# bdaiinstitute/judo

Hardware: AMD Instinct MI355X
Metric: rollouts/sec + plan-step ms, leap_cube MPPI 65536xH64 (higher is better)
Workload: dtype f32

## Files before the change

### include/judo_amd.h

```cpp
#ifndef JUDO_AMD_H
#define JUDO_AMD_H

#include <stddef.h>
#include <stdint.h>

#ifdef __cplusplus
extern "C" {
#endif

typedef struct jh_model jh_model;

enum jh_status {
  JH_OK = 0,
  JH_ERR_INVALID = -1,
  JH_ERR_HIP = -2,
  JH_ERR_UNSUPPORTED = -3,
  JH_ERR_BLOB = -4
};

enum jh_task_kind { JH_TASK_CARTPOLE = 0, JH_TASK_CYLINDER_PUSH = 1, JH_TASK_LEAP_CUBE = 2, JH_TASK_FR3_PICK = 3 };
enum jh_spline_kind { JH_SPLINE_ZERO = 0, JH_SPLINE_LINEAR = 1, JH_SPLINE_CUBIC = 3 };

#define JH_MAX_TASK_PARAMS 32
#define JH_MAX_KNOT_DIM 512
// ... 1 lines not shown

const char* jh_last_error(void);
int jh_version(void);

int jh_model_create(const void* blob, size_t nbytes, int device, jh_model** out);
void jh_model_destroy(jh_model* m);
int jh_model_dims(const jh_model* m, int* dims );

int jh_model_stats(jh_model* m, int* out , int reset);


int jh_model_set_self_collision(jh_model* m, int on);

int jh_model_set_contact_capacity(jh_model* m, int contacts);

int jh_model_build(const jh_model* m, int* out );

int jh_model_fr3_build(const jh_model* m, int* out );

int jh_model_trace_layout(const jh_model* m, int* out );
int jh_trace_gather(const float* rec_in , int k, int stride_in, int n_offset, int n_local, const float* trace , int row_floats,
                    int colmajor, float* rec_out , void* stream);

int jh_model_limits(const jh_model* m, int* out );
int jh_model_max_fused_knots(const jh_model* m, int H);
int jh_model_one_launch_max_knots(const jh_model* m, int H);
int jh_model_set_plan_step_launches(jh_model* m, int launches);
int jh_model_set_rollout_schedule(jh_model* m, int mode);

int jh_upload_async(void* dst_device, const void* src_host, size_t nbytes, void* stream);
int jh_download_wait(void* dst_host, const void* src_device, size_t nbytes, void* stream);
int jh_download_begin(void* dst_host, const void* src_device, size_t nbytes, void* stream);
int jh_download_end(void);

int jh_rollout_cost(const jh_model* m, const float* x0, const float* nominal, const float* noise, int ldn, const float* sigma,
                    const float* W, const float* ctrl_lo_hi, const float* task_params, int phase, int N, int n_offset, int H, int K,
                    float* costs, float* knots_out, void* stream);
int jh_rollout_cost_traced(const jh_model* m, const float* x0, const float* nominal, const float* noise, int ldn, const float* sigma,
                    const float* W, const float* ctrl_lo_hi, const float* task_params, int phase, int N, int n_offset, int H, int K,
                    float* costs, float* knots_out, float* trace , void* stream);

int jh_rollout_materialize(const jh_model* m, const float* x0, int x0_batched, const float* controls, int N, int H, float* states,
                           float* sensors, void* stream);

int jh_task_reward(const jh_model* m, const float* states, const float* sensors, const float* controls, const float* task_params,
                   int phase, int N, int H, float* rewards, void* stream);

int jh_noise_normal(unsigned long long seed, unsigned int draw, int rows, int n_offset, int n_local, float* out, int ldn, void* stream);

int jh_sample_knots(const float* nominal, const float* noise, int ldn, const float* sigma, const float* ctrl_lo_hi ,
                    int N, int n_offset, int K, int nu, float* knots_nku, void* stream);

int jh_spline_controls(const float* W, const float* knots_nku, const float* nominal, const float* noise, int ldn, const float* sigma,
                       const float* ctrl_lo_hi, int N, int n_offset, int H, int K, int nu, float* controls, void* stream);

int jh_knot_moments(const float* knots_nku, const float* nominal, const float* noise, int ldn, const float* sigma, const float* ctrl_lo_hi,
                    const float* center, int N, int n_offset, int K, int nu, float* out, void* stream);

size_t jh_update_scratch_floats(int N, int K, int nu);
int jh_mppi_partial(const float* costs, const float* knots_nku, const float* nominal, const float* noise, int ldn, const float* sigma,
                    const float* ctrl_lo_hi, int N, int n_offset, int K, int nu, float lambda, float* scratch, float* rec, void* stream);
int jh_mppi_merge(const float* recs, int G, int K, int nu, float lambda, float* nominal_out, void* stream);

int jh_topk_partial(const float* costs, const float* knots_nku, const float* nominal, const float* noise, int ldn, const float* sigma,
                    const float* ctrl_lo_hi, int N, int n_offset, int K, int nu, int k, int tie_high, float* scratch, float* rec,
                    void* stream);
size_t jh_update_fused_scratch_floats(int N, int K, int nu);
int jh_update_fused(const float* costs, const float* knots_nku, const float* nominal, const float* noise, int ldn, const float* sigma, const float* ctrl_lo_hi, int N,
                    int n_offset, int K, int nu, int mode, float lambda, int k, int tie_high, int E, const float* trace, int row_floats, int colmajor, float* scratch,
                    float* nominal_out, float* sigma_out, float* trace_out, void* stream);
int jh_plan_step(const jh_model* m, void* blk_dev, const void* blk_host, size_t blk_bytes, int o_nominal, int o_sigma, int o_tp, int o_lohi, const float* noise, int ldn,
                 const float* W, int phase, int N, int n_offset, int H, int K, float* costs, float* knots_out, float* trace, int mode, float lambda, int k, int tie_high, int E,
                 int row_floats, int colmajor, float* scratch, float* out, void* out_host_mark, void* const* timing, void* stream);
size_t jh_plan_batch_scratch_floats(int B, int N, int K, int nu);
int jh_plan_step_batch(const jh_model* m, int B, void* blk_dev, const void* blk_host, size_t blk_bytes, size_t blk_stride_bytes, int o_nominal, int o_sigma, int o_tp, int o_lohi,
                       const float* noise, int ldn, size_t noise_stride_floats, const float* W, int N, int H, int K, float* costs, float* trace, int mode, float lambda, int k,
                       int tie_high, int E, int row_floats, int colmajor, float* scratch, float* out, size_t out_stride_floats, void* out_host_mark, void* const* timing,
                       void* stream);
typedef struct jh_model_set jh_model_set;
int jh_model_set_create(const jh_model* const* models , int B, jh_model_set** out);
int jh_model_set_update(jh_model_set* set, int b, const jh_model* model);
int jh_model_set_info(const jh_model_set* set, int* out );
void jh_model_set_destroy(jh_model_set* set);
int jh_plan_step_batch_models(const jh_model_set* set, void* blk_dev, const void* blk_host, size_t blk_bytes, size_t blk_stride_bytes, int o_nominal, int o_sigma, int o_tp, int o_lohi,
                              const float* noise, int ldn, size_t noise_stride_floats, const float* W, int N, int H, int K, float* costs, float* trace, int mode, float lambda, int k,
                              int tie_high, int E, int row_floats, int colmajor, float* scratch, float* out, size_t out_stride_floats, void* out_host_mark, void* const* timing,
                              void* stream);
int jh_noise_normal_batch(int B, const unsigned long long* seeds , const unsigned int* draws , int rows, int n_local, float* out, int ldn, void* stream);
int jh_spline_controls_batch(const float* W, int B, const float* blk, size_t blk_stride_floats, int o_nominal, int o_sigma, int o_lohi, const float* noise, int ldn,
                             size_t noise_stride_floats, int N, int H, int K, int nu, float* controls, void* stream);
int jh_update_fused_batch(int B, const float* costs, const float* blk, size_t blk_stride_floats, int o_nominal, int o_sigma, int o_lohi, const float* noise, int ldn,
                          size_t noise_stride_floats, int N, int K, int nu, int mode, float lambda, int k, int tie_high, int E, const float* trace, int row_floats, int colmajor,
                          float* scratch, float* out, size_t out_stride_floats, void* out_host_mark, void* stream);
size_t jh_shard_record_floats(int K, int nu, int mode, int k, int E, int row_floats);
int jh_update_shard(const float* costs, const float* knots_nku, const float* nominal, const float* noise, int ldn, const float* sigma, const float* ctrl_lo_hi, int N,
                    int n_offset, int K, int nu, int mode, float lambda, int k, int tie_high, int E, const float* trace, int row_floats, int colmajor, float* scratch,
                    float* rec_out, void* stream);
int jh_shard_merge(const float* recs, int G, int K, int nu, int mode, float lambda, int k, int tie_high, int E, int row_floats, float* nominal_out, float* sigma_out,
                   float* trace_out, void* stream);
int jh_plan_step_shard(const jh_model* m, void* blk_dev, const void* blk_host, size_t blk_bytes, int o_nominal, int o_sigma, int o_tp, int o_lohi, const float* noise, int ldn,
                       const float* W, int phase, int N, int n_offset, int H, int K, float* costs, float* knots_out, float* trace, int mode, float lambda, int k, int tie_high,
                       int E, int row_floats, int colmajor, float* scratch, float* rec_out, void* const* timing, void* stream);
int jh_plan_merge(const float* recs, int G, int K, int nu, int mode, float lambda, int k, int tie_high, int E, int row_floats, float* out, void* out_host_mark,
                  void* timing_done, void* stream);
int jh_event_create(void** out);
void jh_event_destroy(void* ev);
int jh_event_record(void* ev, void* stream);
int jh_stream_wait_event(void* stream, void* ev);
int jh_event_elapsed_ms(void* a, void* b, float* ms);
int jh_elite_merge(const float* recs, int G, int k, int K, int nu, int tie_high, float sigma_min, float sigma_max, float* nominal_out,
                   float* sigma_out, void* stream);

typedef struct jh_policy jh_policy;
int jh_policy_create(const float* const* weights, const float* const* biases, jh_policy** out);
void jh_policy_destroy(jh_policy* p);
size_t jh_policy_scratch_floats(int N);
int jh_policy_step(const jh_policy* p, const float* states, int ld, int nq, int base_qpos, int base_qvel, int leg_qpos, int leg_qvel,
                   const float* command, float* policy_out, float* control, float* scratch, int N, void* stream);

typedef struct jh_tree jh_tree;
int jh_tree_create(const void* blob, size_t nbytes, jh_tree** out);
void jh_tree_destroy(jh_tree* t);
int jh_tree_stats(jh_tree* t, int* out4, int reset);
int jh_tree_set_self_collision(jh_tree* t, int on);
int jh_tree_dims(const jh_tree* t, int* out4 );
int jh_tree_substeps(const jh_tree* t, const float* state_in, const float* ctrl, float* warmstart, int N, int substeps, float* state_out, float* sensors_out,
                     void* stream);

size_t jh_policy_rollout_scratch_floats(int N);
int jh_policy_rollout(const jh_policy* p, jh_tree* t, const float* x0, int x0_batched, const float* commands, float* policy_out, float* warmstart, int reset_warmstart,
                      int N, int T, int substeps, double cutoff_seconds, float* states, float* sensors, float* scratch, int* steps_done, void* stream);
int jh_policy_rollout_batch(const jh_policy* p, jh_tree* t, int B, const float* x0, size_t x0_stride_floats, const float* commands, float* policy_out, float* warmstart,
                            int reset_warmstart, int n, int T, int substeps, double cutoff_seconds, float* states, float* sensors, float* scratch, int* steps_done, void* stream);

#ifdef __cplusplus
}
#endif
#endif
```

### judo_amd/_lib.py

```python

from __future__ import annotations

import ctypes as C
import os

_HERE = os.path.dirname(os.path.abspath(__file__))
LIB_PATH = os.environ.get("JUDO_AMD_LIB") or os.path.join(_HERE, "libjudo_amd.so")

_lib: C.CDLL | None = None

f32p = C.c_void_p

_SIGNATURES = {
    "jh_last_error": (C.c_char_p, []),
    "jh_version": (C.c_int, []),
    "jh_model_create": (C.c_int, [C.c_void_p, C.c_size_t, C.c_int, C.POINTER(C.c_void_p)]),
    "jh_model_destroy": (None, [C.c_void_p]),
    "jh_model_dims": (C.c_int, [C.c_void_p, C.POINTER(C.c_int)]),
    "jh_model_stats": (C.c_int, [C.c_void_p, C.POINTER(C.c_int), C.c_int]),
    "jh_model_set_kernel": (C.c_int, [C.c_void_p, C.c_int]),
    "jh_model_limits": (C.c_int, [C.c_void_p, C.POINTER(C.c_int)]),
    "jh_register_xcheck": (C.c_int, [C.c_void_p]),
    "jh_model_max_fused_knots": (C.c_int, [C.c_void_p, C.c_int]),
    "jh_model_one_launch_max_knots": (C.c_int, [C.c_void_p, C.c_int]),
    "jh_model_set_plan_step_launches": (C.c_int, [C.c_void_p, C.c_int]),
    "jh_model_set_rollout_schedule": (C.c_int, [C.c_void_p, C.c_int]),
    "jh_model_set_self_collision": (C.c_int, [C.c_void_p, C.c_int]),
    "jh_model_set_contact_capacity": (C.c_int, [C.c_void_p, C.c_int]),
    "jh_model_build": (C.c_int, [C.c_void_p, C.POINTER(C.c_int)]),
    "jh_model_fr3_build": (C.c_int, [C.c_void_p, C.POINTER(C.c_int)]),
    "jh_model_trace_layout": (C.c_int, [C.c_void_p, C.POINTER(C.c_int)]),
    "jh_trace_gather": (C.c_int, [C.c_void_p, C.c_int, C.c_int, C.c_int, C.c_int, C.c_void_p, C.c_int, C.c_int, C.c_void_p, C.c_void_p]),
    "jh_upload_async": (C.c_int, [C.c_void_p, C.c_void_p, C.c_size_t, C.c_void_p]),
    "jh_download_wait": (C.c_int, [C.c_void_p, C.c_void_p, C.c_size_t, C.c_void_p]),
    "jh_download_begin": (C.c_int, [C.c_void_p, C.c_void_p, C.c_size_t, C.c_void_p]),
    "jh_download_end": (C.c_int, []),
    "jh_rollout_cost": (C.c_int, [C.c_void_p, f32p, f32p, f32p, C.c_int, f32p, f32p, f32p, f32p, C.c_int, C.c_int, C.c_int, C.c_int, C.c_int, f32p, f32p, C.c_void_p]),
    "jh_rollout_cost_traced": (C.c_int, [C.c_void_p, f32p, f32p, f32p, C.c_int, f32p, f32p, f32p, f32p, C.c_int, C.c_int, C.c_int, C.c_int, C.c_int, f32p, f32p, f32p, C.c_void_p]),
    "jh_rollout_materialize": (C.c_int, [C.c_void_p, f32p, C.c_int, f32p, C.c_int, C.c_int, f32p, f32p, C.c_void_p]),
    "jh_task_reward": (C.c_int, [C.c_void_p, f32p, f32p, f32p, f32p, C.c_int, C.c_int, C.c_int, f32p, C.c_void_p]),
    "jh_noise_normal": (C.c_int, [C.c_ulonglong, C.c_uint, C.c_int, C.c_int, C.c_int, f32p, C.c_int, C.c_void_p]),
    "jh_sample_knots": (C.c_int, [f32p, f32p, C.c_int, f32p, f32p, C.c_int, C.c_int, C.c_int, C.c_int, f32p, C.c_void_p]),
    "jh_spline_controls": (C.c_int, [f32p, f32p, f32p, f32p, C.c_int, f32p, f32p, C.c_int, C.c_int, C.c_int, C.c_int, C.c_int, f32p, C.c_void_p]),
    "jh_spline_controls_batch": (C.c_int, [f32p, C.c_int, f32p, C.c_size_t, C.c_int, C.c_int, C.c_int, f32p, C.c_int, C.c_size_t, C.c_int, C.c_int, C.c_int, C.c_int, f32p, C.c_void_p]),
    "jh_knot_moments": (C.c_int, [f32p, f32p, f32p, C.c_int, f32p, f32p, f32p, C.c_int, C.c_int, C.c_int, C.c_int, f32p, C.c_void_p]),
    "jh_policy_create": (C.c_int, [C.POINTER(C.c_void_p), C.POINTER(C.c_void_p), C.POINTER(C.c_void_p)]),
    "jh_policy_destroy": (None, [C.c_void_p]),
    "jh_policy_scratch_floats": (C.c_size_t, [C.c_int]),
    "jh_policy_step": (C.c_int, [C.c_void_p, f32p, C.c_int, C.c_int, C.c_int, C.c_int, C.c_int, C.c_int, f32p, f32p, f32p, f32p, C.c_int, C.c_void_p]),
    "jh_tree_create": (C.c_int, [C.c_void_p, C.c_size_t, C.POINTER(C.c_void_p)]),
    "jh_tree_destroy": (None, [C.c_void_p]),
    "jh_tree_stats": (C.c_int, [C.c_void_p, C.POINTER(C.c_int), C.c_int]),
    "jh_tree_dims": (C.c_int, [C.c_void_p, C.POINTER(C.c_int)]),
    "jh_tree_set_self_collision": (C.c_int, [C.c_void_p, C.c_int]),
    "jh_tree_substeps": (C.c_int, [C.c_void_p, f32p, f32p, f32p, C.c_int, C.c_int, f32p, f32p, C.c_void_p]),
    "jh_policy_rollout_scratch_floats": (C.c_size_t, [C.c_int]),
    "jh_policy_rollout": (C.c_int, [C.c_void_p, C.c_void_p, f32p, C.c_int, f32p, f32p, f32p, C.c_int, C.c_int, C.c_int, C.c_int, C.c_double, f32p, f32p, f32p, C.POINTER(C.c_int), C.c_void_p]),
    "jh_policy_rollout_batch": (C.c_int, [C.c_void_p, C.c_void_p, C.c_int, f32p, C.c_size_t, f32p, f32p, f32p, C.c_int, C.c_int, C.c_int, C.c_int, C.c_double, f32p, f32p, f32p, C.POINTER(C.c_int),
                                          C.c_void_p]),
    "jh_update_scratch_floats": (C.c_size_t, [C.c_int, C.c_int, C.c_int]),
    "jh_mppi_partial": (C.c_int, [f32p, f32p, f32p, f32p, C.c_int, f32p, f32p, C.c_int, C.c_int, C.c_int, C.c_int, C.c_float, f32p, f32p, C.c_void_p]),
    "jh_mppi_merge": (C.c_int, [f32p, C.c_int, C.c_int, C.c_int, C.c_float, f32p, C.c_void_p]),
    "jh_topk_partial": (C.c_int, [f32p, f32p, f32p, f32p, C.c_int, f32p, f32p, C.c_int, C.c_int, C.c_int, C.c_int, C.c_int, C.c_int, f32p, f32p, C.c_void_p]),
    "jh_update_fused_scratch_floats": (C.c_size_t, [C.c_int, C.c_int, C.c_int]),
    "jh_update_fused": (C.c_int, [f32p, f32p, f32p, f32p, C.c_int, f32p, f32p, C.c_int, C.c_int, C.c_int, C.c_int, C.c_int, C.c_float, C.c_int, C.c_int, C.c_int, f32p, C.c_int, C.c_int,
                                  f32p, f32p, f32p, f32p, C.c_void_p]),
    "jh_plan_step": (C.c_int, [C.c_void_p, C.c_void_p, C.c_void_p, C.c_size_t, C.c_int, C.c_int, C.c_int, C.c_int, f32p, C.c_int, f32p, C.c_int, C.c_int, C.c_int, C.c_int, C.c_int, f32p, f32p, f32p,
                               C.c_int, C.c_float, C.c_int, C.c_int, C.c_int, C.c_int, C.c_int, f32p, f32p, C.c_void_p, C.c_void_p, C.c_void_p]),
    "jh_plan_batch_scratch_floats": (C.c_size_t, [C.c_int, C.c_int, C.c_int, C.c_int]),
    "jh_plan_step_batch": (C.c_int, [C.c_void_p, C.c_int, C.c_void_p, C.c_void_p, C.c_size_t, C.c_size_t, C.c_int, C.c_int, C.c_int, C.c_int, f32p, C.c_int, C.c_size_t, f32p, C.c_int, C.c_int, C.c_int,
                                     f32p, f32p, C.c_int, C.c_float, C.c_int, C.c_int, C.c_int, C.c_int, C.c_int, f32p, f32p, C.c_size_t, C.c_void_p, C.c_void_p, C.c_void_p]),
    "jh_model_set_create": (C.c_int, [C.POINTER(C.c_void_p), C.c_int, C.POINTER(C.c_void_p)]),
    "jh_model_set_update": (C.c_int, [C.c_void_p, C.c_int, C.c_void_p]),
    "jh_model_set_info": (C.c_int, [C.c_void_p, C.POINTER(C.c_int)]),
    "jh_model_set_destroy": (None, [C.c_void_p]),
    "jh_plan_step_batch_models": (C.c_int, [C.c_void_p, C.c_void_p, C.c_void_p, C.c_size_t, C.c_size_t, C.c_int, C.c_int, C.c_int, C.c_int, f32p, C.c_int, C.c_size_t, f32p, C.c_int, C.c_int, C.c_int,
                                            f32p, f32p, C.c_int, C.c_float, C.c_int, C.c_int, C.c_int, C.c_int, C.c_int, f32p, f32p, C.c_size_t, C.c_void_p, C.c_void_p, C.c_void_p]),
    "jh_update_fused_batch": (C.c_int, [C.c_int, f32p, f32p, C.c_size_t, C.c_int, C.c_int, C.c_int, f32p, C.c_int, C.c_size_t, C.c_int, C.c_int, C.c_int, C.c_int, C.c_float, C.c_int, C.c_int, C.c_int,
                                        f32p, C.c_int, C.c_int, f32p, f32p, C.c_size_t, C.c_void_p, C.c_void_p]),
    "jh_noise_normal_batch": (C.c_int, [C.c_int, C.POINTER(C.c_ulonglong), C.POINTER(C.c_uint), C.c_int, C.c_int, f32p, C.c_int, C.c_void_p]),
    "jh_shard_record_floats": (C.c_size_t, [C.c_int, C.c_int, C.c_int, C.c_int, C.c_int, C.c_int]),
    "jh_update_shard": (C.c_int, [f32p, f32p, f32p, f32p, C.c_int, f32p, f32p, C.c_int, C.c_int, C.c_int, C.c_int, C.c_int, C.c_float, C.c_int, C.c_int, C.c_int, f32p, C.c_int, C.c_int,
                                  f32p, f32p, C.c_void_p]),
    "jh_shard_merge": (C.c_int, [f32p, C.c_int, C.c_int, C.c_int, C.c_int, C.c_float, C.c_int, C.c_int, C.c_int, C.c_int, f32p, f32p, f32p, C.c_void_p]),
    "jh_plan_step_shard": (C.c_int, [C.c_void_p, C.c_void_p, C.c_void_p, C.c_size_t, C.c_int, C.c_int, C.c_int, C.c_int, f32p, C.c_int, f32p, C.c_int, C.c_int, C.c_int, C.c_int, C.c_int, f32p, f32p, f32p,
                                     C.c_int, C.c_float, C.c_int, C.c_int, C.c_int, C.c_int, C.c_int, f32p, f32p, C.c_void_p, C.c_void_p]),
    "jh_plan_merge": (C.c_int, [f32p, C.c_int, C.c_int, C.c_int, C.c_int, C.c_float, C.c_int, C.c_int, C.c_int, C.c_int, f32p, C.c_void_p, C.c_void_p, C.c_void_p]),
    "jh_event_create": (C.c_int, [C.POINTER(C.c_void_p)]),
    "jh_event_destroy": (None, [C.c_void_p]),
    "jh_event_record": (C.c_int, [C.c_void_p, C.c_void_p]),
    "jh_stream_wait_event": (C.c_int, [C.c_void_p, C.c_void_p]),
    "jh_event_elapsed_ms": (C.c_int, [C.c_void_p, C.c_void_p, C.POINTER(C.c_float)]),
    "jh_elite_merge": (C.c_int, [f32p, C.c_int, C.c_int, C.c_int, C.c_int, C.c_int, C.c_float, C.c_float, f32p, f32p, C.c_void_p]),
}

EXPORTED_SYMBOLS = tuple(_SIGNATURES)

MAX_KNOT_DIM = 512
MAX_ELITES = 32
MAX_TASK_PARAMS = 32


class JudoAmdError(RuntimeError):
    """A HIP/runtime failure reported by libjudo_amd.so."""


def lib() -> C.CDLL:
    global _lib
    if _lib is None:
        if not os.path.exists(LIB_PATH):
            raise ImportError(
                f"{LIB_PATH} is missing: the MI355X engine has no CPU fallback. "
                "Build it with `python -c 'import __graft_entry__ as g; g.build()'` (needs hipcc)."
            )
        L = C.CDLL(LIB_PATH)
        for name, (res, args) in _SIGNATURES.items():
            fn = getattr(L, name)
            fn.restype = res
            fn.argtypes = args
        _lib = L
    return _lib


def check(status: int, what: str) -> None:
    if status == 0:
        return
    msg = lib().jh_last_error().decode("utf-8", "replace")
    if status == -1:
        raise ValueError(f"{what}: {msg}")
    raise JudoAmdError(f"{what} failed (status {status}): {msg}")


def ptr(t) -> int | None:
    if t is None or isinstance(t, int):
        return t
    return t.data_ptr()
```

### judo_amd/csrc/jh_api.hip

```cpp
#include <algorithm>
#include <cmath>
#include <cstdlib>
#include <cstring>

#include "jh_internal.h"
#include "jh_update_dev.h"

static thread_local char g_err[512] = "";

void jh_set_error(const char* fmt, ...) {
  va_list ap;
  va_start(ap, fmt);
  vsnprintf(g_err, sizeof(g_err), fmt, ap);
  va_end(ap);
}

extern "C" const char* jh_last_error(void) { return g_err; }
extern "C" int jh_version(void) { return 100; }

static int image_cylinders(const jh_blob_header& h, const float* F, const int* I) {
  constexpr int HEADER = 24, BODY_I = 6, BODY_F = 32, BLOCK_I = 4, DOF_F = 20, ACT_I = 2, ACT_F = 8, GEOM_I = 2, GEOM_F = 20, GF_RBOUND = 15;
  if (h.nint < (uint32_t)HEADER || h.nfloat < (uint32_t)HEADER) return 0;
  const long NM = I[0], NBLK = I[1], nv = I[2], nu = I[4], NG = I[5];
  if (NM < 0 || NBLK < 0 || nv < 0 || nu < 0 || NG < 0) return 0;
  const long oI = HEADER + NM * BODY_I + NBLK * BLOCK_I + nu * ACT_I, oF = HEADER + NM * BODY_F + nv * DOF_F + nu * ACT_F;
  if (oI + NG * GEOM_I > (long)h.nint || oF + NG * GEOM_F > (long)h.nfloat) return 0;
  int n = 0;
  for (long g = 0; g < NG; g++) {
    if (I[oI + g * GEOM_I + 1] != 5) continue;
    const float* f = F + oF + g * GEOM_F;
    const float r = f[0], L = f[1], rb = f[GF_RBOUND], want = sqrtf(r * r + L * L);
    if (!(r > 0.f) || !(L > 0.f) || f[2] != 0.f) { jh_set_error("model_create: cylinder geom %ld: sizes must be (radius > 0, half length > 0, 0), got (%g, %g, %g)", g, r, L, f[2]); return -1; }
    if (!(fabsf(rb - want) <= 1e-5f * want)) { jh_set_error("model_create: cylinder geom %ld: bounding radius %g is not sqrt(r^2 + L^2) = %g", g, rb, want); return -1; }
    n++;
  }
  return n;
}

static int image_arm_pairs(const jh_blob_header& h, const int* I) {
  constexpr int HEADER = 24, GEOM_I = 2, GBOX = 6, GCAPSULE = 3, LF = 8, RF = 9;
  if (h.nint < (uint32_t)HEADER) return 0;
  const long gi = I[13];
  if (gi < HEADER || gi + 8 > (long)h.nint) return 0;
  const long nag = I[gi], npair = I[gi + 1];
  if (nag < 0 || npair < 0 || gi + 8 + nag * GEOM_I + npair * 2 > (long)h.nint) return 0;
  int n = 0;
  for (long p = 0; p < npair; p++) {
    const long g1 = I[gi + 8 + nag * GEOM_I + 2 * p], g2 = I[gi + 8 + nag * GEOM_I + 2 * p + 1];
    if (g1 < 0 || g1 >= nag || g2 < 0 || g2 >= nag || g1 == g2) { jh_set_error("model_create: candidate pair %ld names geoms (%ld, %ld) of %ld", p, g1, g2, nag); return -1; }
    const int b1 = I[gi + 8 + g1 * GEOM_I], t1 = I[gi + 8 + g1 * GEOM_I + 1], b2 = I[gi + 8 + g2 * GEOM_I], t2 = I[gi + 8 + g2 * GEOM_I + 1];
    const bool arm_arm = b1 >= 1 && b2 >= 1 && !((b1 == LF && b2 == RF) || (b1 == RF && b2 == LF));
    const bool arm_capsule = t1 == GCAPSULE || (t1 == GBOX && t2 == GCAPSULE && b1 >= 1);
    if (!arm_arm && !arm_capsule) continue;
    if (b1 == b2) { jh_set_error("model_create: candidate pair %ld collides two geoms of arm body %d with each other", p, b1); return -1; }
    if (t1 == GCAPSULE && t2 != GCAPSULE) { jh_set_error("model_create: candidate pair %ld between arm bodies has its capsule first; the kernel takes (box, capsule)", p); return -1; }
    n++;
  }
  return n;
}

extern "C" int jh_model_create(const void* blob, size_t nbytes, int device, jh_model** out) {
  JH_REQUIRE(blob && out, "model_create: null pointer");
  if (nbytes < sizeof(jh_blob_header)) { jh_set_error("model_create: blob too small (%zu bytes)", nbytes); return JH_ERR_BLOB; }
  jh_blob_header h;
  memcpy(&h, blob, sizeof(h));
  if (h.magic != JH_BLOB_MAGIC || h.version != JH_BLOB_VERSION) { jh_set_error("model_create: bad magic/version (%08x, %u)", h.magic, h.version); return JH_ERR_BLOB; }
  size_t need = sizeof(h) + 4 * ((size_t)h.nfloat + h.nint);
  if (nbytes != need) { jh_set_error("model_create: blob size %zu != expected %zu", nbytes, need); return JH_ERR_BLOB; }
  if (h.kind > JH_TASK_FR3_PICK) { jh_set_error("model_create: unknown task kind %u", h.kind); return JH_ERR_BLOB; }
  if (h.kind == JH_TASK_CARTPOLE && h.nfloat < CP_NPARAM) { jh_set_error("model_create: cartpole blob has %u floats, need %d", h.nfloat, CP_NPARAM); return JH_ERR_BLOB; }
  if (h.kind == JH_TASK_CYLINDER_PUSH && h.nfloat < CY_NPARAM) { jh_set_error("model_create: cylinder blob has %u floats, need %d", h.nfloat, CY_NPARAM); return JH_ERR_BLOB; }
  if (h.ntaskparam > JH_MAX_TASK_PARAMS) { jh_set_error("model_create: too many task params"); return JH_ERR_BLOB; }
  int cylinders = 0, arm_pairs = 0;
  if (h.kind == JH_TASK_LEAP_CUBE || h.kind == JH_TASK_FR3_PICK) {
    const char* q = (const char*)blob + sizeof(h);
    std::vector<float> F((const float*)q, (const float*)q + h.nfloat);
    std::vector<int> I((const int*)(q + 4 * (size_t)h.nfloat), (const int*)(q + 4 * (size_t)h.nfloat) + h.nint);
    cylinders = image_cylinders(h, F.data(), I.data());
    if (cylinders < 0) return JH_ERR_BLOB;
    if (cylinders > 0 && h.kind != JH_TASK_LEAP_CUBE) { jh_set_error("model_create: %d cylinder geoms, and only the leap kernel has a cylinder build", cylinders); return JH_ERR_BLOB; }
    if (h.kind == JH_TASK_FR3_PICK) {
      arm_pairs = image_arm_pairs(h, I.data());
      if (arm_pairs < 0) return JH_ERR_BLOB;
    }
  }
  JH_HIP(hipSetDevice(device));
  jh_model* m = new jh_model();
  m->device = device; m->kind = (int)h.kind; m->nq = h.nq; m->nv = h.nv; m->nu = h.nu; m->ns = h.ns; m->ntaskparam = h.ntaskparam;
  m->nf = h.nfloat; m->ni = h.nint; m->d_f = nullptr; m->d_i = nullptr; m->d_stats = nullptr; m->kernel_gen = (h.kind == JH_TASK_LEAP_CUBE || h.kind == JH_TASK_FR3_PICK) ? 3 : 2; m->self_collision = 1; m->contact_capacity = cylinders > 0 ? 64 : 48; m->cylinders = cylinders; m->arm_pairs = arm_pairs;
  { const char* e = getenv("JUDO_AMD_ROLLOUT_SCHEDULE"); m->rollout_schedule = (e && (e[0] == '1' || e[0] == '2')) ? e[0] - '0' : 0; }
  { const char* e = getenv("JUDO_AMD_PLAN_STEP_LAUNCHES"); m->plan_step_launches = (e && e[0] == '2') ? 2 : 0; }
  const char* p = (const char*)blob + sizeof(h);
  m->h_f.assign((const float*)p, (const float*)p + h.nfloat);
  m->h_i.assign((const int*)(p + 4 * (size_t)h.nfloat), (const int*)(p + 4 * (size_t)h.nfloat) + h.nint);
  {
    hipMemPool_t pool = nullptr; int dev = 0;
    if (hipGetDevice(&dev) == hipSuccess && hipDeviceGetDefaultMemPool(&pool, dev) == hipSuccess && pool) {
      unsigned long long keep = ~0ull;
      (void)hipMemPoolSetAttribute(pool, hipMemPoolAttrReleaseThreshold, &keep);
    }
  }
  hipError_t e = hipMalloc(&m->d_f, 4 * (m->nf ? m->nf : 1));
  if (e == hipSuccess) e = hipMalloc(&m->d_i, 4 * (m->ni ? m->ni : 1));
  if (e == hipSuccess) e = hipMalloc(&m->d_stats, JH_NSTATS * sizeof(int));
  if (e == hipSuccess) e = hipMemset(m->d_stats, 0, JH_NSTATS * sizeof(int));
  if (e == hipSuccess && m->nf) e = hipMemcpy(m->d_f, m->h_f.data(), 4 * m->nf, hipMemcpyHostToDevice);
  if (e == hipSuccess && m->ni) e = hipMemcpy(m->d_i, m->h_i.data(), 4 * m->ni, hipMemcpyHostToDevice);
  if (e != hipSuccess) {
    jh_set_error("model_create: device upload failed: %s", hipGetErrorString(e));
    if (m->d_f) (void)hipFree(m->d_f);
    if (m->d_i) (void)hipFree(m->d_i);
    if (m->d_stats) (void)hipFree(m->d_stats);
    delete m;
    return JH_ERR_HIP;
  }
  *out = m;
  return JH_OK;
}

extern "C" void jh_model_destroy(jh_model* m) {
  if (!m) return;
  if (m->d_f) (void)hipFree(m->d_f);
  if (m->d_i) (void)hipFree(m->d_i);
  if (m->d_stats) (void)hipFree(m->d_stats);
  delete m;
}

extern "C" int jh_model_dims(const jh_model* m, int* dims) {
  JH_REQUIRE(m && dims, "model_dims: null pointer");
  dims[0] = m->nq; dims[1] = m->nv; dims[2] = m->nu; dims[3] = m->ns; dims[4] = m->kind; dims[5] = m->ntaskparam;
  return JH_OK;
}

extern "C" int jh_model_stats(jh_model* m, int* out, int reset) {
  JH_REQUIRE(m && out, "model_stats: null pointer");
  JH_HIP(hipMemcpy(out, m->d_stats, 4 * sizeof(int), hipMemcpyDeviceToHost));
  JH_HIP(hipMemcpy(out + 4, m->d_stats + 20, 2 * sizeof(int), hipMemcpyDeviceToHost));
  out[6] = reset ? __atomic_exchange_n(&m->ovf_fallbacks, 0, __ATOMIC_RELAXED) : __atomic_load_n(&m->ovf_fallbacks, __ATOMIC_RELAXED);
  out[7] = reset ? __atomic_exchange_n(&m->one_launch_steps, 0, __ATOMIC_RELAXED) : __atomic_load_n(&m->one_launch_steps, __ATOMIC_RELAXED);
  if (reset) JH_HIP(hipMemset(m->d_stats, 0, JH_NSTATS * sizeof(int)));
  return JH_OK;
}

extern "C" int jh_model_hist(jh_model* m, int* out ) {
  JH_REQUIRE(m && out, "model_hist: null pointer");
  JH_HIP(hipMemcpy(out, m->d_stats + 24, 40 * sizeof(int), hipMemcpyDeviceToHost));
  return JH_OK;
}

extern "C" int jh_model_counters(jh_model* m, int* out, int first, int count) {
  JH_REQUIRE(m && out && first >= 0 && count >= 0 && first + count <= JH_NSTATS, "model_counters: bad range");
  JH_HIP(hipMemcpy(out, m->d_stats + first, count * sizeof(int), hipMemcpyDeviceToHost));
  return JH_OK;
}

static jh_xcheck_launchers g_xcheck = {nullptr, nullptr, nullptr};

extern "C" int jh_register_xcheck(const jh_xcheck_launchers* launchers) {
  JH_REQUIRE(launchers && launchers->rollout_cost && launchers->rollout_materialize && launchers->max_knots, "register_xcheck: incomplete launcher table");
  g_xcheck = *launchers;
  return JH_OK;
}
// ... 185 lines not shown
  JH_HIP(hipMemcpy(out, m->d_stats + 4, 10 * sizeof(long long), hipMemcpyDeviceToHost));
  return JH_OK;
}

extern "C" int jh_rollout_cost(const jh_model* m, const float* x0, const float* nominal, const float* noise, int ldn, const float* sigma,
                               const float* W, const float* lohi, const float* tp, int phase, int N, int n_offset, int H, int K, float* costs,
                               float* knots_out, void* stream) {
  return jh_rollout_cost_traced(m, x0, nominal, noise, ldn, sigma, W, lohi, tp, phase, N, n_offset, H, K, costs, knots_out, nullptr, stream);
}

extern "C" int jh_rollout_cost_traced(const jh_model* m, const float* x0, const float* nominal, const float* noise, int ldn, const float* sigma,
                                      const float* W, const float* lohi, const float* tp, int phase, int N, int n_offset, int H, int K, float* costs,
                                      float* knots_out, float* trace, void* stream) {
  JH_REQUIRE(m && x0 && nominal && noise && sigma && W && lohi && tp && costs, "rollout_cost: null pointer");
  if (trace) { int adr, nfl, cm; trace_layout(m, &adr, &nfl, &cm); JH_REQUIRE(nfl > 0, "rollout_cost_traced: this model's fused kernel writes no trace sensors (jh_model_trace_layout)"); }
  JH_REQUIRE(N > 0 && H > 0 && K >= 1, "rollout_cost: N, H, K must be positive (N=%d H=%d K=%d)", N, H, K);
  JH_REQUIRE(ldn >= N, "rollout_cost: ldn (%d) < N (%d)", ldn, N);
  JH_REQUIRE(K * m->nu <= JH_MAX_KNOT_DIM, "rollout_cost: K*nu = %d exceeds %d", K * m->nu, JH_MAX_KNOT_DIM);
  JH_REQUIRE(n_offset >= 0, "rollout_cost: negative n_offset");
  hipStream_t st = (hipStream_t)stream;
  if (m->kind == JH_TASK_CARTPOLE || m->kind == JH_TASK_CYLINDER_PUSH)
    return jh_simple_rollout_cost(m, x0, nominal, noise, ldn, sigma, W, lohi, tp, N, n_offset, H, K, costs, knots_out, trace, st);
  if (m->kind == JH_TASK_LEAP_CUBE && m->kernel_gen == 3)
    return m->cylinders > 0         ? jh_engine5_rollout_cost_cyl(m, x0, nominal, noise, ldn, sigma, W, lohi, tp, N, n_offset, H, K, costs, knots_out, trace, st)
           : m->contact_capacity > 48 ? jh_engine5_rollout_cost_cap64(m, x0, nominal, noise, ldn, sigma, W, lohi, tp, N, n_offset, H, K, costs, knots_out, trace, st)
                                    : jh_engine5_rollout_cost(m, x0, nominal, noise, ldn, sigma, W, lohi, tp, N, n_offset, H, K, costs, knots_out, trace, st);
  if (m->kind == JH_TASK_FR3_PICK && m->kernel_gen == 3)
    return m->arm_pairs > 0 ? jh_engine6_rollout_cost_self(m, x0, nominal, noise, ldn, sigma, W, lohi, tp, phase, N, n_offset, H, K, costs, knots_out, trace, st)
                            : jh_engine6_rollout_cost(m, x0, nominal, noise, ldn, sigma, W, lohi, tp, phase, N, n_offset, H, K, costs, knots_out, trace, st);
  JH_REQUIRE(trace == nullptr, "rollout_cost_traced: only the product kernels (generation 3, cartpole, cylinder_push) write trace sensors");
  if (!g_xcheck.rollout_cost) { jh_set_error("rollout_cost: no kernel for this model / generation in this library"); return JH_ERR_UNSUPPORTED; }
  return g_xcheck.rollout_cost(m, m->kernel_gen, x0, nominal, noise, ldn, sigma, W, lohi, tp, phase, N, n_offset, H, K, costs, knots_out, stream);
}

static int plan_step_launches(const jh_model* m, int N, int H, int K, const float* costs, const float* knots_out, const float* W, const float* noise, int ldn, bool* one) {
  *one = false;
  if (m->plan_step_launches == 2 || !(m->kind == JH_TASK_CARTPOLE || m->kind == JH_TASK_CYLINDER_PUSH)) return JH_OK;
  const bool fits = costs && W && noise && N > 0 && H > 0 && K >= 1 && ldn >= N && K * m->nu <= JH_MAX_KNOT_DIM && jh_simple_plan_step_fits(m, H, K);
  if (m->plan_step_launches == 1) {
    JH_REQUIRE(!knots_out, "plan_step: the one-launch plan step writes no candidate knots (knots_out), and one launch is forced (jh_model_set_plan_step_launches)");
    JH_REQUIRE(fits, "plan_step: one launch is forced but K = %d exceeds its LDS staging at H = %d (jh_model_one_launch_max_knots)", K, H);
  }
  *one = fits && !knots_out;
  if (*one) __atomic_fetch_add(&m->one_launch_steps, 1, __ATOMIC_RELAXED);
  return JH_OK;
}

static int plan_step(const char* who, const jh_model* m, void* blk_dev, const void* blk_host, size_t blk_bytes, int o_nominal, int o_sigma, int o_tp, int o_lohi,
                     const float* noise, int ldn, const float* W, int phase, int N, int n_offset, int H, int K, float* costs, float* knots_out, float* trace, int mode,
                     float lambda, int k, int tie_high, int E, int row_floats, int colmajor, float* scratch, float* out, unsigned* flag, float* rec_out,
                     void* const* timing, void* stream) {
  JH_REQUIRE(m && blk_dev && blk_host && (out || rec_out) && scratch, "%s: null pointer", who);
  const float* b = (const float*)blk_dev;
  hipStream_t st = (hipStream_t)stream;
  int rc = blk_dev == blk_host ? JH_OK : jh_upload_async(blk_dev, blk_host, blk_bytes, stream);
  if (rc == JH_OK && timing) JH_HIP(hipEventRecord((hipEvent_t)timing[0], st));
  const int KU = K * m->nu;
  const unsigned expect = flag ? __atomic_load_n(flag, __ATOMIC_RELAXED) + 1u : 0u;
  bool one = false;
  if (rc == JH_OK) rc = plan_step_launches(m, N, H, K, costs, knots_out, W, noise, ldn, &one);
  if (rc == JH_OK && !one) rc = jh_rollout_cost_traced(m, b, b + o_nominal, noise, ldn, b + o_sigma, W, b + o_lohi, b + o_tp, phase, N, n_offset, H, K, costs, knots_out, trace, stream);
  if (rc == JH_OK && !one && timing) JH_HIP(hipEventRecord((hipEvent_t)timing[1], st));
  jh_upd::TailArgs a;
  if (rc == JH_OK)
    rc = jh_update_tail_args(who, costs, nullptr, b + o_nominal, noise, ldn, b + o_sigma, b + o_lohi, N, n_offset, K, m->nu, mode, lambda, k, tie_high, trace ? E : 0, trace, row_floats,
                             colmajor, scratch, out, out ? out + KU : nullptr, (out && trace && E > 0) ? out + 2 * KU : nullptr, rec_out, &a);
  a.done_flag = flag; a.done_value = expect;
  if (rc == JH_OK) rc = one ? jh_simple_plan_step(m, b, W, b + o_tp, H, K, a, st) : jh_update_tail_launch(a, st);
  if (rc == JH_OK && one && timing) JH_HIP(hipEventRecord((hipEvent_t)timing[1], st));
  if (rc == JH_OK && timing) JH_HIP(hipEventRecord((hipEvent_t)timing[2], st));
  if (rc == JH_OK && out) rc = download_begin(out, out, 0, stream, flag, expect);
  return rc;
}

extern "C" int jh_plan_step(const jh_model* m, void* blk_dev, const void* blk_host, size_t blk_bytes, int o_nominal, int o_sigma, int o_tp, int o_lohi, const float* noise, int ldn,
                            const float* W, int phase, int N, int n_offset, int H, int K, float* costs, float* knots_out, float* trace, int mode, float lambda, int k, int tie_high, int E,
                            int row_floats, int colmajor, float* scratch, float* out, void* out_host_mark, void* const* timing , void* stream) {
  JH_REQUIRE(out, "plan_step: null pointer");
  unsigned* flag = (out_host_mark && out_host_mark != (void*)out) ? (unsigned*)out_host_mark : nullptr;
  return plan_step("plan_step", m, blk_dev, blk_host, blk_bytes, o_nominal, o_sigma, o_tp, o_lohi, noise, ldn, W, phase, N, n_offset, H, K, costs, knots_out, trace, mode, lambda, k,
                   tie_high, E, row_floats, colmajor, scratch, out, flag, nullptr, timing, stream);
}

static int plan_step_batch(const char* who, const jh_model* m, const float* images, long long image_stride, int B, void* blk_dev, const void* blk_host, size_t blk_bytes, size_t blk_stride_bytes,
                           int o_nominal, int o_sigma, int o_tp, int o_lohi, const float* noise, int ldn, size_t noise_stride_floats, const float* W, int N, int H, int K, float* costs,
                           float* trace, int mode, float lambda, int k, int tie_high, int E, int row_floats, int colmajor, float* scratch, float* out, size_t out_stride_floats,
                           void* out_host_mark, void* const* timing, void* stream) {
  JH_REQUIRE(m && blk_dev && blk_host && out && scratch && noise && W && costs, "%s: null pointer", who);
  if (m->kind == JH_TASK_FR3_PICK) { jh_set_error("%s: fr3_pick has no batched plan step (its phase is chosen per problem on the host)", who); return JH_ERR_UNSUPPORTED; }
  if (m->kind == JH_TASK_LEAP_CUBE && m->kernel_gen != 3) { jh_set_error("%s: only kernel generation 3 of the leap family has a batched launch (this model runs %d)", who, m->kernel_gen); return JH_ERR_UNSUPPORTED; }
  JH_REQUIRE(B >= 1, "%s: B must be at least 1 (B=%d)", who, B);
  JH_REQUIRE(B <= 65535, "%s: B = %d exceeds the 65535 problems of a launch (the grid's second dimension)", who, B);
  JH_REQUIRE(N > 0 && H > 0 && K >= 1, "%s: N, H, K must be positive (N=%d H=%d K=%d)", who, N, H, K);
  JH_REQUIRE(ldn >= N, "%s: ldn (%d) < N (%d)", who, ldn, N);
  const int KU = K * m->nu;
  JH_REQUIRE(KU <= JH_MAX_KNOT_DIM, "%s: K*nu = %d exceeds %d", who, KU, JH_MAX_KNOT_DIM);
  const int nx = m->nq + m->nv;
  JH_REQUIRE(o_nominal >= 0 && o_sigma >= 0 && o_tp >= 0 && o_lohi >= 0, "%s: negative block offset", who);
  const size_t need = sizeof(float) * (size_t)std::max(std::max(nx, o_nominal + KU), std::max(std::max(o_sigma + KU, o_tp + m->ntaskparam), o_lohi + 2 * m->nu));
  JH_REQUIRE(blk_bytes >= need, "%s: a block of %zu bytes does not hold x0 | nominal | sigma | task params | bounds at the given offsets (%zu bytes)", who, blk_bytes, need);
  JH_REQUIRE(blk_stride_bytes >= blk_bytes && blk_stride_bytes % sizeof(float) == 0, "%s: blk_stride_bytes = %zu is smaller than a block (%zu bytes) or no multiple of 4", who, blk_stride_bytes, blk_bytes);
  JH_REQUIRE(noise_stride_floats >= (size_t)KU * (size_t)ldn, "%s: noise_stride_floats = %zu is smaller than a problem's noise (K*nu*ldn = %zu)", who, noise_stride_floats, (size_t)KU * (size_t)ldn);
  int t_adr = 0, t_nfl = 0, t_cm = 0;
  if (trace) { trace_layout(m, &t_adr, &t_nfl, &t_cm); JH_REQUIRE(t_nfl > 0 && row_floats == H * t_nfl, "%s: row_floats = %d is not H x the model's %d trace floats per step (jh_model_trace_layout)", who, row_floats, t_nfl); }
  const int E_t = trace ? E : 0;
  JH_REQUIRE(E_t >= 0 && E_t <= JH_MAX_ELITES, "%s: bad trace arguments (E=%d)", who, E);
  const size_t rec = 2 * (size_t)KU + (size_t)E_t * (2 + (size_t)(E_t > 0 ? row_floats : 0));
  JH_REQUIRE(out_stride_floats >= rec, "%s: out_stride_floats = %zu is smaller than an output record (nominal | sigma | E trace records = %zu floats)", who, out_stride_floats, rec);
  const bool closed = m->kind == JH_TASK_CARTPOLE || m->kind == JH_TASK_CYLINDER_PUSH;
  if (!closed && m->kind != JH_TASK_LEAP_CUBE) { jh_set_error("%s: no batched kernel for this model", who); return JH_ERR_UNSUPPORTED; }
  hipStream_t st = (hipStream_t)stream;
  const float* b = (const float*)blk_dev;
  if (blk_dev != blk_host) { const int rc = jh_upload_async(blk_dev, blk_host, (size_t)(B - 1) * blk_stride_bytes + blk_bytes, stream); if (rc != JH_OK) return rc; }
  if (timing) JH_HIP(hipEventRecord((hipEvent_t)timing[0], st));
  unsigned* flag = (out_host_mark && out_host_mark != (void*)out) ? (unsigned*)out_host_mark : nullptr;
  const unsigned expect = flag ? __atomic_load_n(flag, __ATOMIC_RELAXED) + 1u : 0u;
  bool one = false;
  if (int rc = plan_step_launches(m, N, H, K, costs, nullptr, W, noise, ldn, &one)) return rc;
  jh_upd::TailArgs a;
  if (int rc = jh_update_tail_args(who, costs, nullptr, b + o_nominal, noise, ldn, b + o_sigma, b + o_lohi, N, 0, K, m->nu, mode, lambda, k, tie_high, E_t, trace, row_floats, colmajor,
                                   scratch, out, out + KU, E_t > 0 ? out + 2 * KU : nullptr, nullptr, &a)) return rc;
  jh_upd::BatchArgs s;
  s.B = B; s.blk = (long long)(blk_stride_bytes / sizeof(float)); s.noise = (long long)noise_stride_floats; s.costs = N; s.trace = (long long)N * row_floats;
  s.scratch = (long long)jh_update_fused_scratch_floats(N, K, m->nu); s.out = (long long)out_stride_floats;
  s.counter = reinterpret_cast<unsigned*>(scratch) + 1; s.done_flag = flag; s.done_value = expect; s.image = image_stride;
  int rc = JH_OK;
  if (one) rc = jh_simple_plan_step_batch(m, images, b, W, b + o_tp, H, K, a, s, st);
  else {
    if (closed) rc = jh_simple_rollout_cost_batch(m, images, b, b + o_tp, W, H, K, a, s, st);
    else
      rc = m->cylinders > 0           ? jh_engine5_rollout_cost_batch_cyl(m, images, image_stride, B, b, b + o_nominal, b + o_sigma, b + o_lohi, b + o_tp, s.blk, noise, ldn, s.noise, W, N, H, K, costs, trace, st)
           : m->contact_capacity > 48 ? jh_engine5_rollout_cost_batch_cap64(m, images, image_stride, B, b, b + o_nominal, b + o_sigma, b + o_lohi, b + o_tp, s.blk, noise, ldn, s.noise, W, N, H, K, costs, trace, st)
                                      : jh_engine5_rollout_cost_batch(m, images, image_stride, B, b, b + o_nominal, b + o_sigma, b + o_lohi, b + o_tp, s.blk, noise, ldn, s.noise, W, N, H, K, costs, trace, st);
    if (rc == JH_OK && timing) JH_HIP(hipEventRecord((hipEvent_t)timing[1], st));
    if (rc == JH_OK) rc = jh_update_tail_batch_launch(a, s, st);
  }
  if (rc == JH_OK && one && timing) JH_HIP(hipEventRecord((hipEvent_t)timing[1], st));
  if (rc == JH_OK && timing) JH_HIP(hipEventRecord((hipEvent_t)timing[2], st));
  if (rc == JH_OK) rc = download_begin(out, out, 0, stream, flag, expect);
  return rc;
}

extern "C" int jh_plan_step_batch(const jh_model* m, int B, void* blk_dev, const void* blk_host, size_t blk_bytes, size_t blk_stride_bytes, int o_nominal, int o_sigma, int o_tp, int o_lohi,
                                  const float* noise, int ldn, size_t noise_stride_floats, const float* W, int N, int H, int K, float* costs, float* trace, int mode, float lambda, int k,
                                  int tie_high, int E, int row_floats, int colmajor, float* scratch, float* out, size_t out_stride_floats, void* out_host_mark, void* const* timing,
                                  void* stream) {
  JH_REQUIRE(m != nullptr, "plan_step_batch: null pointer");
  return plan_step_batch("plan_step_batch", m, m->d_f, 0, B, blk_dev, blk_host, blk_bytes, blk_stride_bytes, o_nominal, o_sigma, o_tp, o_lohi, noise, ldn, noise_stride_floats, W, N, H, K, costs, trace,
                         mode, lambda, k, tie_high, E, row_floats, colmajor, scratch, out, out_stride_floats, out_host_mark, timing, stream);
}

struct jh_model_set {
  int B;
  size_t nf, stride;
  float* d_images;
  const jh_model* m0;
  std::vector<std::vector<float>> hf;
};

static int model_set_member(const char* who, const jh_model* m0, const jh_model* m, int b) {
  JH_REQUIRE(m != nullptr, "%s: member %d is a null pointer", who, b);
  if (m->kind == JH_TASK_FR3_PICK) { jh_set_error("%s: member %d is an fr3_pick model, which has no batched plan step (its phase is chosen per problem on the host)", who, b); return JH_ERR_UNSUPPORTED; }
  if (m->kind == JH_TASK_LEAP_CUBE && m->kernel_gen != 3) { jh_set_error("%s: member %d runs kernel_gen %d: only kernel generation 3 of the leap family has a batched launch", who, b, m->kernel_gen); return JH_ERR_UNSUPPORTED; }
  if (m->kind != JH_TASK_CARTPOLE && m->kind != JH_TASK_CYLINDER_PUSH && m->kind != JH_TASK_LEAP_CUBE) { jh_set_error("%s: member %d: no batched kernel for this model (kind %d)", who, b, m->kind); return JH_ERR_UNSUPPORTED; }
  if (m != m0) {
#define JH_SET_SAME(field, fmt)                                                                                                                                    \
  JH_REQUIRE(m->field == m0->field, "%s: member %d differs from the set's member 0 in " #field " (" fmt " against " fmt ")", who, b, m->field, m0->field)
    JH_SET_SAME(device, "%d"); JH_SET_SAME(kind, "%d"); JH_SET_SAME(nq, "%d"); JH_SET_SAME(nv, "%d"); JH_SET_SAME(nu, "%d"); JH_SET_SAME(ns, "%d"); JH_SET_SAME(ntaskparam, "%d");
    JH_SET_SAME(nf, "%zu"); JH_SET_SAME(ni, "%zu");
    if (m->h_i != m0->h_i) {
      size_t w = 0;
      while (w < m->h_i.size() && m->h_i[w] == m0->h_i[w]) w++;
      jh_set_error("%s: member %d differs from the set's member 0 in the int section h_i (word %zu: %d against %d): topology, pair lists and lane lists are one for the launch", who, b, w, m->h_i[w], m0->h_i[w]);
      return JH_ERR_INVALID;
    }
    JH_SET_SAME(kernel_gen, "%d"); JH_SET_SAME(contact_capacity, "%d"); JH_SET_SAME(cylinders, "%d"); JH_SET_SAME(self_collision, "%d"); JH_SET_SAME(rollout_schedule, "%d");
    JH_SET_SAME(plan_step_launches, "%d");
#undef JH_SET_SAME
  }
  JH_REQUIRE(m->h_f.size() == m->nf && m->d_f, "%s: member %d has no float section of nf = %zu floats", who, b, m->nf);
  if (m->kind == JH_TASK_LEAP_CUBE) {
    const bool ok = m->cylinders > 0 ? jh_engine5_accepts_cyl(m) : m->contact_capacity > 48 ? jh_engine5_accepts_cap64(m) : jh_engine5_accepts(m);
    if (!ok) {
      jh_set_error("%s: member %d: the leap kernel does not accept this image (dimensions, table sizes, or h_f: the cube's inertia must be isotropic)", who, b);
      return JH_ERR_UNSUPPORTED;
    }
  }
  return JH_OK;
}

static int model_set_upload(jh_model_set* s, int b, const jh_model* m) {
  if (s->nf) JH_HIP(hipMemcpy(s->d_images + (size_t)b * s->stride, m->d_f, 4 * s->nf, hipMemcpyDeviceToDevice));
  s->hf[b] = m->h_f;
  return JH_OK;
}

extern "C" int jh_model_set_create(const jh_model* const* models, int B, jh_model_set** out) {
  JH_REQUIRE(models && out, "model_set_create: null pointer");
  JH_REQUIRE(B >= 1, "model_set_create: B must be at least 1 (B=%d)", B);
  JH_REQUIRE(B <= 65535, "model_set_create: B = %d exceeds the 65535 problems of a launch (the grid's second dimension)", B);
  for (int b = 0; b < B; b++) if (int rc = model_set_member("model_set_create", models[0], models[b], b)) return rc;
  const jh_model* m0 = models[0];
  JH_HIP(hipSetDevice(m0->device));
  jh_model_set* s = new jh_model_set();
  s->B = B; s->nf = m0->nf; s->stride = (m0->nf + 63) / 64 * 64; s->d_images = nullptr; s->m0 = m0; s->hf.resize(B);
  if (s->stride == 0) s->stride = 64;
  hipError_t e = hipMalloc(&s->d_images, 4 * s->stride * (size_t)B);
  if (e == hipSuccess) e = hipMemset(s->d_images, 0, 4 * s->stride * (size_t)B);
  int rc = JH_OK;
  if (e != hipSuccess) { jh_set_error("model_set_create: device allocation failed: %s", hipGetErrorString(e)); rc = JH_ERR_HIP; }
  for (int b = 0; b < B && rc == JH_OK; b++) rc = model_set_upload(s, b, models[b]);
  if (rc != JH_OK) { if (s->d_images) (void)hipFree(s->d_images); delete s; return rc; }
  *out = s;
  return JH_OK;
}

extern "C" int jh_model_set_update(jh_model_set* s, int b, const jh_model* model) {
  JH_REQUIRE(s && model, "model_set_update: null pointer");
  JH_REQUIRE(b >= 0 && b < s->B, "model_set_update: member %d of a set of %d", b, s->B);
  if (int rc = model_set_member("model_set_update", s->m0, model, b)) return rc;
  JH_HIP(hipSetDevice(s->m0->device));
  if (int rc = model_set_upload(s, b, model)) return rc;
  if (b == 0) s->m0 = model;
  return JH_OK;
}

extern "C" int jh_model_set_info(const jh_model_set* s, int* out) {
  JH_REQUIRE(s && out, "model_set_info: null pointer");
  int differ = 0;
  for (int b = 1; b < s->B; b++) differ += s->hf[b].size() != s->hf[0].size() || memcmp(s->hf[b].data(), s->hf[0].data(), 4 * s->hf[0].size()) != 0;
  out[0] = s->B; out[1] = (int)s->nf; out[2] = (int)s->stride; out[3] = differ;
  return JH_OK;
}

extern "C" void jh_model_set_destroy(jh_model_set* s) {
  if (!s) return;
  if (s->d_images) (void)hipFree(s->d_images);
  delete s;
}

extern "C" int jh_plan_step_batch_models(const jh_model_set* set, void* blk_dev, const void* blk_host, size_t blk_bytes, size_t blk_stride_bytes, int o_nominal, int o_sigma, int o_tp, int o_lohi,
                                         const float* noise, int ldn, size_t noise_stride_floats, const float* W, int N, int H, int K, float* costs, float* trace, int mode, float lambda,
                                         int k, int tie_high, int E, int row_floats, int colmajor, float* scratch, float* out, size_t out_stride_floats, void* out_host_mark,
                                         void* const* timing, void* stream) {
  JH_REQUIRE(set != nullptr, "plan_step_batch_models: null pointer");
  return plan_step_batch("plan_step_batch_models", set->m0, set->d_images, (long long)set->stride, set->B, blk_dev, blk_host, blk_bytes, blk_stride_bytes, o_nominal, o_sigma, o_tp, o_lohi, noise, ldn,
                         noise_stride_floats, W, N, H, K, costs, trace, mode, lambda, k, tie_high, E, row_floats, colmajor, scratch, out, out_stride_floats, out_host_mark, timing, stream);
}

extern "C" int jh_update_fused_batch(int B, const float* costs, const float* blk, size_t blk_stride_floats, int o_nominal, int o_sigma, int o_lohi, const float* noise, int ldn,
                                     size_t noise_stride_floats, int N, int K, int nu, int mode, float lambda, int k, int tie_high, int E, const float* trace, int row_floats,
                                     int colmajor, float* scratch, float* out, size_t out_stride_floats, void* out_host_mark, void* stream) {
  JH_REQUIRE(costs && blk && noise && scratch && out, "update_fused_batch: null pointer");
  JH_REQUIRE(B >= 1, "update_fused_batch: B must be at least 1 (B=%d)", B);
  JH_REQUIRE(B <= 65535, "update_fused_batch: B = %d exceeds the 65535 problems of a launch (the grid's second dimension)", B);
  JH_REQUIRE(N > 0 && K > 0 && nu > 0 && K * nu <= JH_MAX_KNOT_DIM, "update_fused_batch: N, K, nu must be positive and K*nu <= %d (N=%d K=%d nu=%d)", JH_MAX_KNOT_DIM, N, K, nu);
  JH_REQUIRE(o_nominal >= 0 && o_sigma >= 0 && o_lohi >= 0, "update_fused_batch: negative block offset");
  const int KU = K * nu;
  const size_t need = (size_t)std::max(std::max(o_nominal + KU, o_sigma + KU), o_lohi + 2 * nu);
  JH_REQUIRE(blk_stride_floats >= need, "update_fused_batch: blk_stride_floats = %zu is smaller than a block (nominal | sigma | bounds at the given offsets end at %zu floats)", blk_stride_floats, need);
  JH_REQUIRE(ldn >= N && noise_stride_floats >= (size_t)KU * (size_t)ldn, "update_fused_batch: ldn (%d) < N (%d), or noise_stride_floats = %zu is smaller than a problem's noise (K*nu*ldn = %zu)", ldn, N,
             noise_stride_floats, (size_t)KU * (size_t)ldn);
  const int E_t = trace ? E : 0;
  JH_REQUIRE(E_t >= 0 && E_t <= JH_MAX_ELITES && (E_t == 0 || row_floats >= 1), "update_fused_batch: bad trace arguments (E=%d row_floats=%d)", E, row_floats);
  const size_t rec = 2 * (size_t)KU + (size_t)E_t * (2 + (size_t)(E_t > 0 ? row_floats : 0));
  JH_REQUIRE(out_stride_floats >= rec, "update_fused_batch: out_stride_floats = %zu is smaller than an output record (nominal | sigma | E trace records = %zu floats)", out_stride_floats, rec);
  unsigned* flag = (out_host_mark && out_host_mark != (void*)out) ? (unsigned*)out_host_mark : nullptr;
  const unsigned expect = flag ? __atomic_load_n(flag, __ATOMIC_RELAXED) + 1u : 0u;
  jh_upd::TailArgs a;
  if (int rc = jh_update_tail_args("update_fused_batch", costs, nullptr, blk + o_nominal, noise, ldn, blk + o_sigma, blk + o_lohi, N, 0, K, nu, mode, lambda, k, tie_high, E_t, trace, row_floats,
                                   colmajor, scratch, out, out + KU, E_t > 0 ? out + 2 * KU : nullptr, nullptr, &a)) return rc;
  jh_upd::BatchArgs s;
  s.B = B; s.blk = (long long)blk_stride_floats; s.noise = (long long)noise_stride_floats; s.costs = N; s.trace = (long long)N * row_floats;
  s.scratch = (long long)jh_update_fused_scratch_floats(N, K, nu); s.out = (long long)out_stride_floats;
  s.counter = reinterpret_cast<unsigned*>(scratch) + 1; s.done_flag = flag; s.done_value = expect;
  if (int rc = jh_update_tail_batch_launch(a, s, (hipStream_t)stream)) return rc;
  return download_begin(out, out, 0, stream, flag, expect);
}

extern "C" int jh_plan_step_shard(const jh_model* m, void* blk_dev, const void* blk_host, size_t blk_bytes, int o_nominal, int o_sigma, int o_tp, int o_lohi, const float* noise,
                                  int ldn, const float* W, int phase, int N, int n_offset, int H, int K, float* costs, float* knots_out, float* trace, int mode, float lambda, int k,
                                  int tie_high, int E, int row_floats, int colmajor, float* scratch, float* rec_out, void* const* timing , void* stream) {
  JH_REQUIRE(rec_out, "plan_step_shard: null pointer");
  return plan_step("plan_step_shard", m, blk_dev, blk_host, blk_bytes, o_nominal, o_sigma, o_tp, o_lohi, noise, ldn, W, phase, N, n_offset, H, K, costs, knots_out, trace, mode,
                   lambda, k, tie_high, E, row_floats, colmajor, scratch, nullptr, nullptr, rec_out, timing, stream);
}

extern "C" int jh_plan_merge(const float* recs, int G, int K, int nu, int mode, float lambda, int k, int tie_high, int E, int row_floats, float* out, void* out_host_mark,
                             void* timing_done , void* stream) {
  JH_REQUIRE(recs && out, "plan_merge: null pointer");
  const int KU = K * nu;
  int rc = jh_shard_merge(recs, G, K, nu, mode, lambda, k, tie_high, E, row_floats, out, out + KU, E > 0 ? out + 2 * KU : nullptr, stream);
  if (rc == JH_OK && timing_done) JH_HIP(hipEventRecord((hipEvent_t)timing_done, (hipStream_t)stream));
  if (rc == JH_OK) rc = jh_download_begin(out_host_mark, out, 0, stream);
  return rc;
}

extern "C" int jh_event_create(void** out) { JH_REQUIRE(out, "event_create: null pointer"); hipEvent_t e; JH_HIP(hipEventCreate(&e)); *out = e; return JH_OK; }
extern "C" void jh_event_destroy(void* ev) { if (ev) (void)hipEventDestroy((hipEvent_t)ev); }
extern "C" int jh_event_record(void* ev, void* stream) { JH_REQUIRE(ev, "event_record: null pointer"); JH_HIP(hipEventRecord((hipEvent_t)ev, (hipStream_t)stream)); return JH_OK; }
extern "C" int jh_stream_wait_event(void* stream, void* ev) {
  JH_REQUIRE(ev, "stream_wait_event: null pointer");
  JH_HIP(hipStreamWaitEvent((hipStream_t)stream, (hipEvent_t)ev, 0));
  return JH_OK;
}
extern "C" int jh_event_elapsed_ms(void* a, void* b, float* ms) {
  JH_REQUIRE(a && b && ms, "event_elapsed_ms: null pointer");
  JH_HIP(hipEventSynchronize((hipEvent_t)b));
  JH_HIP(hipEventElapsedTime(ms, (hipEvent_t)a, (hipEvent_t)b));
  return JH_OK;
}

extern "C" int jh_rollout_materialize(const jh_model* m, const float* x0, int x0_batched, const float* controls, int N, int H, float* states,
                                      float* sensors, void* stream) {
  JH_REQUIRE(m && x0 && controls, "rollout_materialize: null pointer");
  JH_REQUIRE(states || sensors, "rollout_materialize: both outputs are null");
  JH_REQUIRE(N > 0 && H > 0, "rollout_materialize: N and H must be positive (N=%d H=%d)", N, H);
  hipStream_t st = (hipStream_t)stream;
  if (m->kind == JH_TASK_CARTPOLE || m->kind == JH_TASK_CYLINDER_PUSH) return jh_simple_materialize(m, x0, x0_batched, controls, N, H, states, sensors, st);
  if (m->kind == JH_TASK_LEAP_CUBE && m->kernel_gen == 3)
    return m->cylinders > 0 ? jh_engine5_materialize_cyl(m, x0, x0_batched, controls, N, H, states, sensors, st) : m->contact_capacity > 48 ? jh_engine5_materialize_cap64(m, x0, x0_batched, controls, N, H, states, sensors, st) : jh_engine5_materialize(m, x0, x0_batched, controls, N, H, states, sensors, st);
  if (m->kind == JH_TASK_FR3_PICK && m->kernel_gen == 3)
    return m->arm_pairs > 0 ? jh_engine6_materialize_self(m, x0, x0_batched, controls, N, H, states, sensors, st) : jh_engine6_materialize(m, x0, x0_batched, controls, N, H, states, sensors, st);
  if (!g_xcheck.rollout_materialize) { jh_set_error("rollout_materialize: no kernel for this model / generation in this library"); return JH_ERR_UNSUPPORTED; }
  return g_xcheck.rollout_materialize(m, m->kernel_gen, x0, x0_batched, controls, N, H, states, sensors, stream);
}

extern "C" int jh_task_reward(const jh_model* m, const float* states, const float* sensors, const float* controls, const float* tp, int phase, int N,
                              int H, float* rewards, void* stream) {
// ... 10 lines not shown
```

### judo_amd/csrc/jh_engine_v5.hip

```cpp
#include <cstddef>
#include <type_traits>

#include "jh_coop.h"

using namespace jh_eng;
using namespace jh_coop;

namespace {

#ifdef JH_V5_WAVESTAMP
__device__ unsigned long long* g_wavestamp = nullptr;
__device__ int g_wavestamp_cap = 0;
#endif

constexpr int G = 16, RPW = 4, WAVE = 64;
constexpr int NCH = 4, NLK = 4;

constexpr int LSMAX = 16;
constexpr int WAVES_PER_EU = 2;
constexpr int WAVES_PER_BLOCK = 4;
constexpr int BFS = 33;
constexpr int PAS = 9;
constexpr int RSPAD = 4;
constexpr int C3PAD = 278;
constexpr int NSLDS = 3;
constexpr double BIGPROB = 0.999999;
constexpr int CVX_STOP_NM = 1000;
#define OPAQUE(x) asm volatile("" : "+v"(x))
#define WSYNC() do { __builtin_amdgcn_fence(__ATOMIC_RELEASE, "wavefront"); __builtin_amdgcn_wave_barrier(); __builtin_amdgcn_fence(__ATOMIC_ACQUIRE, "wavefront"); } while (0)
#ifndef JH_V5_NSLOT
#define JH_V5_NSLOT 2
#endif
#ifndef JH_V5_NSBIG
#define JH_V5_NSBIG 3
#endif
#ifndef JH_V5_CYL
#define JH_V5_CYL 0
#endif
constexpr int GCYL = 5;
constexpr int NSLOT = JH_V5_NSLOT;
constexpr int NSBIG = JH_V5_NSBIG;
constexpr int NCP = 16 * (NSBIG < NSLDS ? NSBIG : NSLDS);
constexpr int NCAP = 16 * NSBIG;
constexpr int NOVF = NCAP - NCP;
constexpr int MAXHIT = 64;
constexpr int POOL_F = 10;
constexpr int MAXG = 80, MAXLG = 8;
constexpr int CUBE = 17;
constexpr int HITPAIR = 1 << 15;
static_assert(MAXG <= 128, "hand geom pairs are packed into 14 bits");
constexpr int MAXBP = 128;
constexpr int MAXBPL = 96;
constexpr int NDH = 22 * 23 / 2;
constexpr int NV = 22, NQ = 23, NU = 16, NS = 31, NS_CALTECH = 23, NX = 45, NMB = 17;
constexpr int NBC = 20;
__device__ __forceinline__ bool static_code(int b) { return b == 0 || b >= NMB; }

enum { LC_DAMP = 0, LC_KVD, LC_KP, LC_KV, LC_CLO, LC_CHI, LC_CLIM, LC_FL, LC_FB, LC_FD, LC_INVW, LC_LIMITED, LC_LO, LC_HI, LC_LK, LC_LB, LC_SI, LC_IMCK = LC_SI + 5, LC_N = 25 };

struct __attribute__((aligned(16))) RS {
  float pa[NMB][PAS];
  float xR[NMB][9];
  float qv[NV], g[NV], p[NV], ws[NV];
  float acn[6];
  float Mbb[NCH][10];
  float rhs6[6];
  float cmd[4];
  union {
    struct {
      float bs[NBC][4];
      unsigned short hits[MAXHIT];
      unsigned char bpl[MAXBPL];
    };
    struct { float pk_q[G], pk_fs[G], pk_cq[4], pk_acc; };
  };
  union {
    float pool[NCP][POOL_F];
    struct { float Hcc[21], Hbb[NCH][10], Hcb[NCH][24], Hx[6][16]; };
    struct { float Hd[NDH], dinv[NV]; };
    struct { float c3pad_[C3PAD]; float c3s[G][12]; };
  };
  int ncon, nhit;
  float pad_[RSPAD];
};

static_assert(offsetof(RS, c3s) % 16 == 0 && C3PAD >= NDH + NV && sizeof(((RS*)nullptr)->c3pad_) + sizeof(((RS*)nullptr)->c3s) <= sizeof(((RS*)nullptr)->pool), "c3 cache: aligned rows behind the Newton matrices, inside the pool's storage");
struct PoolCtx { RS* S; int* overflow; float* ovf; };

__device__ __forceinline__ void push_contact(const PoolCtx& pc, const float* pos, const float* n, float dist, int body, float mu, float tran) {
  int i = atomicAdd(&pc.S->ncon, 1);
  float* e;
  if (i < NCP) e = pc.S->pool[i];
  else if (NOVF > 0 && pc.ovf && i < NCAP) e = pc.ovf + (i - NCP) * POOL_F;
  else { if (pc.overflow) atomicAdd(pc.overflow, 1); return; }
  e[0] = pos[0]; e[1] = pos[1]; e[2] = pos[2]; e[3] = n[0]; e[4] = n[1]; e[5] = n[2]; e[6] = dist; e[7] = mu; e[8] = __int_as_float(body); e[9] = tran;
}

struct LeapSink {
  PoolCtx pc; int sides; float mu, tran; bool flip;
  __device__ __forceinline__ void push(const float* pos, const float* n, float dist) {
    const float nn[3] = {flip ? -n[0] : n[0], flip ? -n[1] : n[1], flip ? -n[2] : n[2]};
    push_contact(pc, pos, nn, dist, sides, mu, tran);
  }
};

#if JH_V5_CYL
struct CvxOne {
  float pos[3], n[3], dist; bool hit;
  __device__ __forceinline__ void push(const float* p, const float* nn, float d) { for (int k = 0; k < 3; k++) { pos[k] = p[k]; n[k] = nn[k]; } dist = d; hit = true; }
};
#endif

struct Slot {
  int la, lb;
  float fr[9];
  float rc[3];
  float aref[3], D0, D1, Dm, mu, fri;
  float jar[3], jp[3];
};

__device__ __forceinline__ bool obb_face_overlap(const float* ca, const float* Ra, const float* ha, const float* cb, const float* Rb, const float* hb) {
  const float d[3] = {cb[0] - ca[0], cb[1] - ca[1], cb[2] - ca[2]};
  float C[9];
#pragma unroll
  for (int i = 0; i < 3; i++)
#pragma unroll
    for (int j = 0; j < 3; j++) C[3 * i + j] = fabsf(Ra[i] * Rb[j] + Ra[3 + i] * Rb[3 + j] + Ra[6 + i] * Rb[6 + j]);
  bool ok = true;
#pragma unroll
  for (int i = 0; i < 3; i++) {
    const float da = fabsf(d[0] * Ra[i] + d[1] * Ra[3 + i] + d[2] * Ra[6 + i]);
    ok = ok && da <= ha[i] + hb[0] * C[3 * i] + hb[1] * C[3 * i + 1] + hb[2] * C[3 * i + 2];
    const float db = fabsf(d[0] * Rb[i] + d[1] * Rb[3 + i] + d[2] * Rb[6 + i]);
    ok = ok && db <= hb[i] + ha[0] * C[i] + ha[1] * C[3 + i] + ha[2] * C[6 + i];
// ... 225 lines not shown
#ifdef JH_V5_WAVESTAMP
  const unsigned long long ws_entry = wall_clock64(); unsigned long long ws_staged = ws_entry;
#endif
  const int tid = threadIdx.x, wv = tid >> 6, lane = tid & 63, r = lane >> 4;
  int l = lane & 15, c = l >> 2, s = l & 3;
  RS& S = sRS[wv * RPW + r];
  const int nmI = gI[0], nblkI = gI[1], nuI = gI[4], ngI = gI[5], nsiteI = gI[6], nsI = gI[7], oRef = gI[18];
  const int oBodyF = HEADER_F, oDofF = oBodyF + nmI * BODY_F, oActF = oDofF + gI[2] * DOF_F, oGeomF = oActF + nuI * ACT_F, oSiteF = oGeomF + ngI * GEOM_F;
  const int oGeomI = HEADER_I + nmI * BODY_I + nblkI * BLOCK_I + nuI * ACT_I, oSiteI = oGeomI + ngI * GEOM_I;
  const int oLane = gI[11], lgm = gI[12];
  const int oBP = gI[15], oBS = gI[16], nBP = gI[17], oBG = oBP + 2 * nBP;
  for (int i = tid; i < 16 * BODY_F; i += WAVE * WPB) sBody[(i / BODY_F) * BFS + i % BODY_F] = gF[oBodyF + BODY_F + i];
  for (int i = tid; i < ngI * GEOM_F; i += WAVE * WPB) sGeomF[i] = gF[oGeomF + i];
  for (int i = tid; i < ngI * GEOM_I; i += WAVE * WPB) sGeomI[i] = gI[oGeomI + i];
  for (int i = tid; i < 16 * lgm; i += WAVE * WPB) sLaneG[i] = gI[oLane + i];
  if (!MATERIALIZE && tid < 9) sTp[tid] = tp[tid];
  if constexpr (SELF) {
    for (int i = tid; i < 2 * nBP && i < 2 * MAXBP; i += WAVE * WPB) sBP[i] = gI[oBP + i];
    for (int i = tid; i < 2 * NBC; i += WAVE * WPB) sBG[i] = gI[oBG + i];
    for (int i = tid; i < NBC * 8; i += WAVE * WPB) sBB[i] = gF[oBS + i];
  }
  if (tid < 16) {
    const float* df = gF + oDofF + (6 + l) * DOF_F; const float* af = gF + oActF + l * ACT_F;
    float* lc = sLane + l * LC_N;
    lc[LC_DAMP] = df[DF_DAMP]; lc[LC_KVD] = df[DF_KV]; lc[LC_FL] = df[DF_FL]; lc[LC_FB] = df[DF_FB]; lc[LC_FD] = df[DF_FD]; lc[LC_INVW] = df[DF_INVW];
    lc[LC_LIMITED] = df[DF_LIMITED]; lc[LC_LO] = df[DF_LO]; lc[LC_HI] = df[DF_HI]; lc[LC_LK] = df[DF_LK]; lc[LC_LB] = df[DF_LB];
    for (int k = 0; k < 5; k++) lc[LC_SI + k] = df[DF_SOLIMP + k];
    lc[LC_KP] = af[AF_KP]; lc[LC_KV] = af[AF_KV]; lc[LC_CLIM] = af[AF_CLIM]; lc[LC_CLO] = af[AF_CLO]; lc[LC_CHI] = af[AF_CHI];
    lc[LC_IMCK] = l < 6 ? 1.f / (l < 3 ? gF[HF_CMASS] : gF[HF_CINERTIA + (l < 3 ? 0 : l - 3)]) : 0.f;
  }
  const float* lc = sLane + l * LC_N;
  int grp = blockIdx.x * WPB + wv;
  const int ngroups = (N + RPW - 1) / RPW;
  if constexpr (PERSIST) {
    __syncthreads();
#ifdef JH_V5_WAVESTAMP
    ws_staged = wall_clock64();
#endif
  }
  for (; !PERSIST || grp < ngroups;) {
  if constexpr (PERSIST) { if (lane == 0) sGrp[wv] = grp; }
#ifdef JH_V5_WAVESTAMP
  const unsigned long long ws_start = wall_clock64();
#endif
  const int n = (grp << (2 - dshift)) + (r >> dshift);
  const bool live = n < N && (r & ((1 << dshift) - 1)) == 0;
  const int nc = n < N ? n : N - 1;
  const float h = gF[HF_DT], impratio = gF[HF_IMPRATIO], tol = gF[HF_TOL], lstol = gF[HF_LSTOL]; const int cap = (int)gF[HF_MAXITER];
  const float grav[3] = {gF[HF_GRAV], gF[HF_GRAV + 1], gF[HF_GRAV + 2]};
  const float cmass = gF[HF_CMASS], cI[3] = {gF[HF_CINERTIA], gF[HF_CINERTIA + 1], gF[HF_CINERTIA + 2]};
  const float chs[3] = {gF[HF_CSIZE], gF[HF_CSIZE + 1], gF[HF_CSIZE + 2]}, crb = gF[HF_CRBOUND], ctran = gF[HF_CTRAN];
  const float cK = gF[HF_CK], cB = gF[HF_CB];
  float csi[5]; for (int k = 0; k < 5; k++) csi[k] = gF[HF_SOLIMP + k];
  const float mck = (l < 3 ? cmass : (l == 3 ? cI[0] : (l == 4 ? cI[1] : (l == 5 ? cI[2] : 0.f))));
  float q, qd, qc[7], vc[6];
  {
    const float* xi = x0 + ((MATERIALIZE && x0_batched) ? (size_t)nc * NX : 0);
    for (int k = 0; k < 7; k++) qc[k] = xi[k];
    for (int k = 0; k < 6; k++) vc[k] = xi[NQ + k];
    q = xi[7 + l]; qd = xi[NQ + 6 + l];
  }
  auto knot_at = [&](int k, int ll, int ncc) -> float {
    const int i = k * NU + ll;
    float v = nominal[i];
    if (n_offset + ncc != 0) v = fmaf(sigma[i], noise[(size_t)i * ldn + ncc], v);
    return jh_clampf(v, lohi[ll], lohi[NU + ll]);
  };
  if (!MATERIALIZE) {
    if (knots_out && live) for (int k = 0; k < K; k++) knots_out[(size_t)(k * NU + l) * ldn + n] = knot_at(k, l, nc);
  }
  S.ws[6 + l] = 0.f; if (l < 6) S.ws[l] = 0.f;
  if (l < 4) S.cmd[l] = l == 0 ? cmass : (l == 1 ? cI[0] : (l == 2 ? cI[1] : cI[2]));
  int n_iters = 0, n_maxed = 0, n_wave_iters = 0;
  float acc = 0.f;
#ifdef JH_V5_TICKS
  long long cyc[16] = {0, 0, 0, 0, 0, 0, 0, 0, 0, 0, 0, 0, 0, 0, 0, 0}, t0 = clock64();
#define V5_TICK(slot) { long long t__ = clock64(); cyc[slot] += t__ - t0; t0 = t__; }
#else
#define V5_TICK(slot)
#endif
#ifdef JH_V5_COUNT
  int cnt_dense = 0, cnt_it = 0, cnt_l2 = 0, cnt_bp = 0, cnt_hh = 0, cnt_cls[4] = {0, 0, 0, 0};
  enum { CB_SPH = 34, CB_SPHMAX, CB_BOXMAX, CB_L1PAIRPASS, CB_L1LISTPASS, CB_TRIPS, CB_BPAIRS, CB_T, CB_COMBOPASS, CB_CUBEBOX, CB_CUBEBOXLANES, CB_MSPH, CB_MBOX, CB_MT, CB_NOSPH, CB_ONEA, CB_ONEB,
         CB_OWNTRIPS, CB_SPHOVER, CB_FEWSPH };
#define V5_CADD(k, v) do { if (stats) atomicAdd(stats + (k), (int)(v)); } while (0)
#define V5_CMAX(k, v) do { if (stats) atomicMax(stats + (k), (int)(v)); } while (0)
#endif
  if constexpr (PERSIST) WSYNC();
  else {
    __syncthreads();
#ifdef JH_V5_WAVESTAMP
    ws_staged = wall_clock64();
#endif
  }

  for (int hh = 0; hh < H; hh++) {
    OPAQUE(l); c = l >> 2; s = l & 3;
    const float* lc = sLane + l * LC_N;
    float u;
    if (MATERIALIZE) u = controls[((size_t)nc * H + hh) * NU + l];
    else {
      u = 0.f;
      {
        int lo_ = lane; OPAQUE(lo_);
        const int g_ = PERSIST ? sGrp[wv] : (int)(blockIdx.x * WPB + wv);
        const int n_ = (g_ << (2 - dshift)) + ((lo_ >> 4) >> dshift), nc_ = n_ < N ? n_ : N - 1;
        for (int k = 0; k < K; k++) u = fmaf(W[hh * K + k], knot_at(k, l, nc_), u);
      }
    }
    float Mrow[NLK], fs_own, a0_own;
    {
      float ax[NLK][3], og[NLK][3], Rown[9], pown[3];
      {
        float nn = rsqrtf(qc[3] * qc[3] + qc[4] * qc[4] + qc[5] * qc[5] + qc[6] * qc[6]);
        qc[3] *= nn; qc[4] *= nn; qc[5] *= nn; qc[6] *= nn;
        float Rc[9]; quat2mat(Rc, qc + 3);
        float P[3] = {0, 0, 0}, R[9] = {1, 0, 0, 0, 1, 0, 0, 0, 1};
        float sn_own, cs_own; sincosf(q, &sn_own, &cs_own);
#pragma unroll
        for (int j = 0; j < NLK; j++) {
          const float* bf = sBody + (4 * c + j) * BFS;
          float P2[3], R0[9];
          if (j == 0) { for (int k = 0; k < 3; k++) P2[k] = bf[BF_LPOS + k]; for (int k = 0; k < 9; k++) R0[k] = bf[BF_LR + k]; }
          else { mulMV(P2, R, bf + BF_LPOS); for (int k = 0; k < 3; k++) P2[k] += P[k]; mulMM(R0, R, bf + BF_LR); }
          const float* al = bf + BF_AXIS;
          mulMV(ax[j], R0, al);
          for (int k = 0; k < 3; k++) { og[j][k] = P2[k]; P[k] = P2[k]; }
          const float sn = quad_get(sn_own, j), cs = quad_get(cs_own, j), t = 1.f - cs, x = al[0], y = al[1], z = al[2];
          float Rq[9] = {t * x * x + cs, t * x * y - sn * z, t * x * z + sn * y, t * x * y + sn * z, t * y * y + cs, t * y * z - sn * x, t * x * z - sn * y, t * y * z + sn * x, t * z * z + cs};
          mulMM(R, R0, Rq);
          if (j == s) { for (int k = 0; k < 3; k++) pown[k] = P2[k]; for (int k = 0; k < 9; k++) Rown[k] = R[k]; }
        }
        for (int k = 0; k < 3; k++) { S.pa[1 + l][k] = pown[k]; S.pa[1 + l][4 + k] = s == 0 ? ax[0][k] : (s == 1 ? ax[1][k] : (s == 2 ? ax[2][k] : ax[3][k])); }
        for (int k = 0; k < 9; k++) S.xR[1 + l][k] = Rown[k];
        if (l == 0) { for (int k = 0; k < 3; k++) S.pa[0][k] = qc[k]; for (int k = 0; k < 9; k++) S.xR[0][k] = Rc[k]; S.ncon = 0; S.nhit = 0; }
        S.qv[6 + l] = qd;
        if (l < 6) S.qv[l] = vc[l];
      }
      if (!MATERIALIZE && trace && nsI == NS) {
        WSYNC();
        if (live && l < nsiteI && l < 5) {
          int b = gI[oSiteI + l]; float p3[3]; mulMV(p3, S.xR[b], gF + oSiteF + l * SITE_F);
          float* tr = trace + ((size_t)n * H + hh) * 15 + 3 * l;
          for (int k = 0; k < 3; k++) tr[k] = p3[k] + S.pa[b][k];
        }
      }
      if (MATERIALIZE && sensors) {
        float* y = sensors + ((size_t)nc * H + hh) * nsI;
        if (live) y[l] = q;
        WSYNC();
        if (nsI == NS) {
          if (live && l < nsiteI && l < 5) {
            int b = gI[oSiteI + l]; float p3[3]; mulMV(p3, S.xR[b], gF + oSiteF + l * SITE_F);
            for (int k = 0; k < 3; k++) y[16 + 3 * l + k] = p3[k] + S.pa[b][k];
          }
        } else if (live && l < 7) {
          const float* rf = gF + oRef;
          if (l < 3) y[16 + l] = rf[3 + l] * (qc[0] - rf[0]) + rf[6 + l] * (qc[1] - rf[1]) + rf[9 + l] * (qc[2] - rf[2]);
          else {
            const float a0 = rf[12], a1 = -rf[13], a2 = -rf[14], a3 = -rf[15], b0 = qc[3], b1 = qc[4], b2 = qc[5], b3 = qc[6];
            const float qo[4] = {a0 * b0 - a1 * b1 - a2 * b2 - a3 * b3, a0 * b1 + a1 * b0 + a2 * b3 - a3 * b2, a0 * b2 - a1 * b3 + a2 * b0 + a3 * b1, a0 * b3 + a1 * b2 - a2 * b1 + a3 * b0};
            y[16 + l] = l == 3 ? qo[0] : (l == 4 ? qo[1] : (l == 5 ? qo[2] : qo[3]));
          }
        }
      }
      {
        const float* bf = sBody + (4 * c + s) * BFS;
// ... 61 lines not shown
      float Icw[3] = {cI[0] * vc[3], cI[1] * vc[4], cI[2] * vc[5]}, gc[3]; cross3(gc, vc + 3, Icw);
      (void)gc;
      a0c_own = l < 3 ? (l == 0 ? grav[0] : (l == 1 ? grav[1] : grav[2])) : 0.f;
    }
    WSYNC();
    V5_TICK(0)
    bool hand_hits = false;
    {
      int nh = 0;
      float Rc[9]; for (int k = 0; k < 9; k++) Rc[k] = S.xR[0][k];
      const float* pw = S.pa[1 + l]; const float* Rw = S.xR[1 + l];
      if constexpr (SELF) {
        const float* b8 = sBB + 8 * (1 + l); float cw[3]; mulMV(cw, Rw, b8);
        S.bs[1 + l][0] = cw[0] + pw[0]; S.bs[1 + l][1] = cw[1] + pw[1]; S.bs[1 + l][2] = cw[2] + pw[2]; S.bs[1 + l][3] = b8[3];
        if (l < 4) { S.bs[0][l] = sBB[l]; for (int b = NMB; b < NBC; b++) S.bs[b][l] = sBB[8 * b + l]; }
      }
      float pwr[3], Rwr[9];
      for (int k = 0; k < 3; k++) pwr[k] = pw[k];
      for (int k = 0; k < 9; k++) Rwr[k] = Rw[k];
      int gids[MAXLG];
#pragma unroll
      for (int i = 0; i < MAXLG; i++) gids[i] = i < lgm ? sLaneG[l * lgm + i] : -1;
#pragma unroll
      for (int i = 0; i < MAXLG; i++) {
        if (i >= lgm) break;
        const int gid = gids[i], g0 = gid < 0 ? 0 : gid;
        const float* gf = sGeomF + g0 * GEOM_F;
        const int gbody = sGeomI[g0 * GEOM_I], gtype = sGeomI[g0 * GEOM_I + 1];
        const float lp[3] = {gf[GF_POS], gf[GF_POS + 1], gf[GF_POS + 2]}, rb = gf[GF_RBOUND];
        float gp[3]; mulMV(gp, Rwr, lp); gp[0] += pwr[0]; gp[1] += pwr[1]; gp[2] += pwr[2];
        if (gbody < 0) { gp[0] = lp[0]; gp[1] = lp[1]; gp[2] = lp[2]; }
        const float dc[3] = {gp[0] - qc[0], gp[1] - qc[1], gp[2] - qc[2]}, rs = rb + crb;
        float cl[3]; mulMTV(cl, Rc, dc);
        bool hit = (gid >= 0) & (dot3(dc, dc) <= rs * rs) & (fabsf(cl[0]) <= chs[0] + rb) & (fabsf(cl[1]) <= chs[1] + rb) & (fabsf(cl[2]) <= chs[2] + rb);
#if JH_V5_CYL
        if (hit && gtype != GSPHERE) {
          const bool cyl = gtype == GCYL;
          const float gh[3] = {gf[GF_SIZE], cyl ? gf[GF_SIZE] : gf[GF_SIZE + 1], cyl ? gf[GF_SIZE + 1] : gf[GF_SIZE + 2]};
          float gR[9], gl[3];
          if (gbody < 0) { for (int k = 0; k < 9; k++) gR[k] = gf[GF_R + k]; } else mulMM(gR, Rwr, gf + GF_R);
          mulMTV(gl, gR, dc);
          hit = fabsf(gl[0]) <= gh[0] + crb && fabsf(gl[1]) <= gh[1] + crb && fabsf(gl[2]) <= gh[2] + crb;
        }
#else
#ifdef JH_V5_COUNT
        if constexpr (SELF) { const unsigned long long bx = __ballot(hit && gtype == GBOX); if (lane == 0 && bx != 0) { V5_CADD(CB_CUBEBOX, 1); V5_CADD(CB_CUBEBOXLANES, __popcll(bx)); } }
#endif
        if (hit && gtype == GBOX) {
          float gR[9], gl[3];
          if (gbody < 0) { for (int k = 0; k < 9; k++) gR[k] = gf[GF_R + k]; } else mulMM(gR, Rwr, gf + GF_R);
          mulMTV(gl, gR, dc);
          hit = fabsf(gl[0]) <= gf[GF_SIZE] + crb && fabsf(gl[1]) <= gf[GF_SIZE + 1] + crb && fabsf(gl[2]) <= gf[GF_SIZE + 2] + crb;
        }
#endif
        unsigned m16 = (unsigned)((__ballot(hit) >> (16 * r)) & 0xFFFFull);
        int pos = nh + __popc(m16 & ((1u << l) - 1u));
        if (hit && pos < MAXHIT) S.hits[pos] = (unsigned short)gid;
        nh += __popc(m16);
      }
      WSYNC();
      V5_TICK(13)
      if constexpr (SELF) {
      int nbl = 0;
      {
        constexpr int NPASS = MAXBP / G;
        int pab[NPASS]; unsigned sph = 0;
#pragma unroll
        for (int i = 0; i < NPASS; i++) { const int pi = i * G + l, pj = pi < nBP ? pi : 0; pab[i] = sBP[2 * pj] | sBP[2 * pj + 1] << 8; }
#pragma unroll
        for (int i = 0; i < NPASS; i++) {
          const float* sa = S.bs[pab[i] & 0xFF]; const float* sb = S.bs[pab[i] >> 8];
          const float d[3] = {sa[0] - sb[0], sa[1] - sb[1], sa[2] - sb[2]}, rs = sa[3] + sb[3];
          sph |= ((i * G + l < nBP) & (dot3(d, d) <= rs * rs)) ? 1u << i : 0u;
        }
#ifdef JH_V5_COUNT
        {
          int ns = 0, npass = 0;
          for (int i = 0; i < NPASS; i++) { const unsigned long long b = __ballot((sph >> i) & 1u); ns += __popc((unsigned)((b >> (16 * r)) & 0xFFFFull)); npass += b != 0; }
          const int nsm = wave_rowmax(ns);
          if (l == 0 && live) { V5_CADD(CB_SPH, ns); V5_CMAX(CB_MSPH, ns); V5_CADD(CB_NOSPH, ns == 0); V5_CADD(CB_SPHOVER, ns > MAXBPL); V5_CMAX(CB_FEWSPH, MAXBP - ns); }
          if (lane == 0) { V5_CADD(CB_SPHMAX, nsm); V5_CADD(CB_L1PAIRPASS, npass); V5_CADD(CB_L1LISTPASS, (nsm + G - 1) / G); }
        }
#endif
        unsigned char* const tail = reinterpret_cast<unsigned char*>(&S.pool[0][0]);
        static_assert(sizeof(((RS*)nullptr)->pool) >= MAXBP - MAXBPL, "the tail of the sphere survivors fits the contact pool's storage");
        int nsl = 0;
#pragma unroll
        for (int i = 0; i < NPASS; i++) {
          if (i * G >= nBP) break;
          const bool hit = (sph >> i) & 1u;
          const unsigned m16 = (unsigned)((__ballot(hit) >> (16 * r)) & 0xFFFFull);
          const int pos = nsl + __popc(m16 & ((1u << l) - 1u));
          if (hit) { if (pos < MAXBPL) S.bpl[pos] = (unsigned char)(i * G + l); else tail[pos - MAXBPL] = (unsigned char)(i * G + l); }
          nsl += __popc(m16);
        }
        WSYNC();
        for (int base = 0; __any(base < nsl); base += G) {
          const int idx = base + l;
          bool hit = idx < nsl; int pi = 0;
          if (hit) {
            pi = idx < MAXBPL ? S.bpl[idx] : tail[idx - MAXBPL];
            const int ba = sBP[2 * pi], bb = sBP[2 * pi + 1];
            const float* sa = S.bs[ba]; const float* sb = S.bs[bb];
            const float I9[9] = {1, 0, 0, 0, 1, 0, 0, 0, 1};
            float Ra[9]; for (int k = 0; k < 9; k++) Ra[k] = static_code(ba) ? I9[k] : S.xR[ba][k];
            hit = obb_face_overlap(sa, Ra, sBB + 8 * ba + 4, sb, S.xR[bb], sBB + 8 * bb + 4);
          }
          unsigned m16 = (unsigned)((__ballot(hit) >> (16 * r)) & 0xFFFFull);
          int pos = nbl + __popc(m16 & ((1u << l) - 1u));
          if (hit && pos < MAXBPL) S.bpl[pos] = (unsigned char)pi;
          nbl += __popc(m16);
          WSYNC();
        }
      }
#ifdef JH_V5_COUNT
      { const int nbm = wave_rowmax(nbl); if (lane == 0) V5_CADD(CB_BOXMAX, nbm); if (l == 0 && live) V5_CMAX(CB_MBOX, nbl); }
#endif
      if (nbl > MAXBPL) { if (l == 0 && live && stats) atomicAdd(stats, nbl - MAXBPL); nbl = MAXBPL; }
#ifdef JH_V5_COUNT
      if (l == 0 && live) cnt_bp += nbl;
#endif
      const int nh_cube = nh;
      WSYNC();
      V5_TICK(14)
      for (int i = 0; __any(i < nbl); i++) {
#ifdef JH_V5_COUNT
        if (lane == 0) cnt_l2++;
#endif
        int ba = 0, bb = 0, ga0 = 0, na = 0, gb0 = 0, nb = 0;
        if (i < nbl) { const int pi = S.bpl[i]; ba = sBP[2 * pi]; bb = sBP[2 * pi + 1]; ga0 = sBG[2 * ba]; na = sBG[2 * ba + 1]; gb0 = sBG[2 * bb]; nb = sBG[2 * bb + 1]; }
        bool near = false;
        if (l < na + nb) {
          const bool isA = l < na;
          const int g = isA ? ga0 + l : gb0 + (l - na), own = isA ? ba : bb, oth = isA ? bb : ba;
          const float* gf = sGeomF + g * GEOM_F;
          float cw[3];
          if (static_code(own)) { cw[0] = gf[GF_POS]; cw[1] = gf[GF_POS + 1]; cw[2] = gf[GF_POS + 2]; }
          else { mulMV(cw, S.xR[own], gf + GF_POS); cw[0] += S.pa[own][0]; cw[1] += S.pa[own][1]; cw[2] += S.pa[own][2]; }
          const float dw[3] = {cw[0] - S.bs[oth][0], cw[1] - S.bs[oth][1], cw[2] - S.bs[oth][2]};
          float dl[3];
          if (static_code(oth)) { dl[0] = dw[0]; dl[1] = dw[1]; dl[2] = dw[2]; } else mulMTV(dl, S.xR[oth], dw);
          const float* hb = sBB + 8 * oth + 4;
          const float ex = fmaxf(fabsf(dl[0]) - hb[0], 0.f), ey = fmaxf(fabsf(dl[1]) - hb[1], 0.f), ez = fmaxf(fabsf(dl[2]) - hb[2], 0.f);
          near = ex * ex + ey * ey + ez * ez <= gf[GF_RBOUND] * gf[GF_RBOUND];
        }
        const unsigned m16 = (unsigned)((__ballot(near) >> (16 * r)) & 0xFFFFull);
        const unsigned mB = (m16 >> na) & ((1u << nb) - 1u);
        const unsigned mA = mB != 0 ? (m16 & ((1u << na) - 1u)) : 0u;
        const int nB = __popc(mB), T = __popc(mA) * nB;
#ifdef JH_V5_COUNT
        {
          const int tm = wave_rowmax((T + G - 1) / G);
          if (lane == 0) V5_CADD(CB_COMBOPASS, tm);
          if (l == 0 && live && T != 0) { V5_CADD(CB_BPAIRS, 1); V5_CADD(CB_T, T); V5_CMAX(CB_MT, T); V5_CADD(CB_ONEA, __popc(mA) == 1); V5_CADD(CB_ONEB, nB == 1); V5_CADD(CB_OWNTRIPS, __popc(mA)); }
        }
#endif
        const float rnB = __builtin_amdgcn_rcpf((float)nB);
        for (int t = l; __any(t - l < T); t += G) {
          bool hit = false;
          int ga = 0, gb = 0;
          if (t < T) {
            const int ra = (int)(((float)t + 0.5f) * rnB), rb = t - ra * nB;
            ga = ga0 + nth_bit16(mA, ra); gb = gb0 + nth_bit16(mB, rb);
            const float* fa = sGeomF + ga * GEOM_F; const float* fb = sGeomF + gb * GEOM_F;
            float ca[3], cb[3];
            if (static_code(ba)) { ca[0] = fa[GF_POS]; ca[1] = fa[GF_POS + 1]; ca[2] = fa[GF_POS + 2]; }
// ... 780 lines not shown
  if (stats && lane == 0 && live) { atomicAdd(stats + 20, n_wave_iters); atomicAdd(stats + 21, H); }
#ifdef JH_V5_WAVESTAMP
  if (lane == 0 && g_wavestamp && grp < g_wavestamp_cap) {
    unsigned long long* w = g_wavestamp + (size_t)grp * 6;
    w[0] = ((unsigned long long)blockIdx.x << 32) | ((unsigned long long)wv << 8) | (__smid() & 0xff); w[1] = ws_entry; w[2] = ws_staged; w[3] = ws_start; w[4] = wall_clock64(); w[5] = 1;
  }
#endif
  if constexpr (!PERSIST) break;
  else {
    int t = 0;
    if (lane == 0) t = (int)atomicAdd(head, 1u);
    grp = (int)(gridDim.x * WPB) + __builtin_amdgcn_readfirstlane(t);
  }
  }
}

bool model_is_leap(const jh_model* m) {
  return m->kind == JH_TASK_LEAP_CUBE && m->nq == 23 && m->nv == 22 && m->nu == 16 && (m->ns == NS || (m->ns == NS_CALTECH && m->h_i.size() > 18 && m->h_i[18] > 0)) && m->h_i.size() > 17 &&
         m->h_i[0] == 17 && m->h_i[1] == 4 && m->h_i[11] > 0 && m->h_i[5] <= MAXG && m->h_i[12] <= MAXLG && m->h_i[17] <= MAXBP
         && m->h_f.size() > (size_t)HF_CINERTIA + 2 && m->h_f[HF_CINERTIA] == m->h_f[HF_CINERTIA + 1] && m->h_f[HF_CINERTIA] == m->h_f[HF_CINERTIA + 2]
         ;
}

int device_cus(const jh_model* m) {
  int v = 0;
  return (hipDeviceGetAttribute(&v, hipDeviceAttributeMultiprocessorCount, m->device) == hipSuccess && v > 0) ? v : 256;
}

}

#ifndef JH_V5_NAME
#define JH_V5_NAME(f) f
#endif
#ifdef JH_V5_WAVESTAMP
extern "C" int JH_V5_NAME(jh_v5_wavestamp_buffer)(unsigned long long* buf, int groups) {
  JH_HIP(hipMemcpyToSymbol(HIP_SYMBOL(g_wavestamp), &buf, sizeof(buf)));
  JH_HIP(hipMemcpyToSymbol(HIP_SYMBOL(g_wavestamp_cap), &groups, sizeof(groups)));
  return JH_OK;
}
#endif
int JH_V5_NAME(jh_engine5_rollout_cost)(const jh_model* m, const float* x0, const float* nominal, const float* noise, int ldn, const float* sigma, const float* W,
                            const float* lohi, const float* tp, int N, int n_offset, int H, int K, float* costs, float* knots_out, float* trace, hipStream_t st) {
  if (!model_is_leap(m)) { jh_set_error("rollout_cost: the cooperative engine kernel is instantiated for leap_cube only"); return JH_ERR_UNSUPPORTED; }
  if ((m->cylinders > 0) != (JH_V5_CYL != 0)) { jh_set_error("rollout_cost: an image with cylinder geoms runs on the cylinder build of the leap kernel and no other image does (%d cylinders)", m->cylinders); return JH_ERR_UNSUPPORTED; }
  const int dshift = jh_latency_shift(N, RPW); const int per_block = (RPW >> dshift) * WAVES_PER_BLOCK;
  int grid = (N + per_block - 1) / per_block;
  bool persist = dshift == 0 && m->rollout_schedule != 1; int slots = 0;
  if (persist) { slots = 2 * device_cus(m); persist = m->rollout_schedule == 2 || grid > slots; }
  const size_t ovf_bytes = NOVF > 0 ? (size_t)N * NOVF * POOL_F * sizeof(float) : 0;
  float* scratch = nullptr; float* ovf = nullptr; unsigned* head = nullptr;
  if (ovf_bytes > 0 || persist) scratch = jh_launch_scratch(m, ovf_bytes + (persist ? 16 : 0), st, ovf_bytes > 0);
  if (scratch && persist && hipMemsetAsync(scratch, 0, 16, st) != hipSuccess) { (void)hipGetLastError(); persist = false; }
  if (!scratch) persist = false;
  if (persist) { head = (unsigned*)scratch; if (grid > slots) grid = slots; }
  if (scratch && ovf_bytes > 0) ovf = scratch + (head ? 4 : 0);
#define JH_V5_LAUNCH_COST(SELF_, PERSIST_)                                                                                                                                        \
  hipLaunchKernelGGL((k_leap_v5<false, WAVES_PER_BLOCK, SELF_, PERSIST_>), dim3(grid), dim3(WAVE * WAVES_PER_BLOCK), 0, st, m->d_f, m->d_i, x0, 0, nominal, noise, ldn, sigma, W, \
                     lohi, tp, N, n_offset, H, K, costs, knots_out, (const float*)nullptr, (float*)nullptr, (float*)nullptr, m->d_stats, dshift, trace, ovf, head, 0ll, 0ll, 0ll)
  if (m->self_collision && m->h_i[17] > 0) { if (persist) JH_V5_LAUNCH_COST(true, true); else JH_V5_LAUNCH_COST(true, false); }
  else { if (persist) JH_V5_LAUNCH_COST(false, true); else JH_V5_LAUNCH_COST(false, false); }
#undef JH_V5_LAUNCH_COST
  return jh_launch_done(scratch, st);
}

int JH_V5_NAME(jh_engine5_materialize)(const jh_model* m, const float* x0, int x0_batched, const float* controls, int N, int H, float* states, float* sensors,
                           hipStream_t st) {
  if (!model_is_leap(m)) { jh_set_error("rollout_materialize: the cooperative engine kernel is instantiated for leap_cube only"); return JH_ERR_UNSUPPORTED; }
  if ((m->cylinders > 0) != (JH_V5_CYL != 0)) { jh_set_error("rollout_materialize: an image with cylinder geoms runs on the cylinder build of the leap kernel and no other image does (%d cylinders)", m->cylinders); return JH_ERR_UNSUPPORTED; }
  const int dshift = jh_latency_shift(N, RPW); const int per_block = (RPW >> dshift) * WAVES_PER_BLOCK;
  int grid = (N + per_block - 1) / per_block;
  float* ovf = nullptr;
  if (NOVF > 0) ovf = jh_launch_scratch(m, (size_t)N * NOVF * POOL_F * sizeof(float), st);
  if (m->self_collision && m->h_i[17] > 0)
    hipLaunchKernelGGL((k_leap_v5<true, WAVES_PER_BLOCK, true>), dim3(grid), dim3(WAVE * WAVES_PER_BLOCK), 0, st, m->d_f, m->d_i, x0, x0_batched, (const float*)nullptr, (const float*)nullptr, 0,
                       (const float*)nullptr, (const float*)nullptr, (const float*)nullptr, (const float*)nullptr, N, 0, H, 0, (float*)nullptr, (float*)nullptr,
                       controls, states, sensors, m->d_stats, dshift, (float*)nullptr, ovf, (unsigned*)nullptr, 0ll, 0ll, 0ll);
  else
    hipLaunchKernelGGL((k_leap_v5<true, WAVES_PER_BLOCK, false>), dim3(grid), dim3(WAVE * WAVES_PER_BLOCK), 0, st, m->d_f, m->d_i, x0, x0_batched, (const float*)nullptr, (const float*)nullptr, 0,
                       (const float*)nullptr, (const float*)nullptr, (const float*)nullptr, (const float*)nullptr, N, 0, H, 0, (float*)nullptr, (float*)nullptr,
                       controls, states, sensors, m->d_stats, dshift, (float*)nullptr, ovf, (unsigned*)nullptr, 0ll, 0ll, 0ll);
  return jh_launch_done(ovf, st);
}

int JH_V5_NAME(jh_engine5_rollout_cost_batch)(const jh_model* m, const float* images, long long image_stride, int B, const float* x0, const float* nominal, const float* sigma, const float* lohi, const float* tp, long long blk_stride,
                                  const float* noise, int ldn, long long noise_stride, const float* W, int N, int H, int K, float* costs, float* trace, hipStream_t st) {
  if (!model_is_leap(m)) { jh_set_error("plan_step_batch: the cooperative engine kernel is instantiated for leap_cube only"); return JH_ERR_UNSUPPORTED; }
  if ((m->cylinders > 0) != (JH_V5_CYL != 0)) { jh_set_error("plan_step_batch: an image with cylinder geoms runs on the cylinder build of the leap kernel and no other image does (%d cylinders)", m->cylinders); return JH_ERR_UNSUPPORTED; }
  JH_REQUIRE((long long)B * N <= 0x7fffffffll, "plan_step_batch: B * N = %lld rollouts exceed one launch", (long long)B * N);
  const int dshift = jh_latency_shift(B * N, RPW); const int per_block = (RPW >> dshift) * WAVES_PER_BLOCK;
  const int grid = (N + per_block - 1) / per_block;
  const size_t ovf_bytes = NOVF > 0 ? (size_t)B * N * NOVF * POOL_F * sizeof(float) : 0;
  float* ovf = ovf_bytes > 0 ? jh_launch_scratch(m, ovf_bytes, st) : nullptr;
#define JH_V5_LAUNCH_BATCH(SELF_)                                                                                                                                                  \
  hipLaunchKernelGGL((k_leap_v5<false, WAVES_PER_BLOCK, SELF_, false, true>), dim3(grid, B), dim3(WAVE * WAVES_PER_BLOCK), 0, st, images, m->d_i, x0, 0, nominal, noise, ldn, sigma, W, \
                     lohi, tp, N, 0, H, K, costs, (float*)nullptr, (const float*)nullptr, (float*)nullptr, (float*)nullptr, m->d_stats, dshift, trace, ovf, (unsigned*)nullptr, blk_stride, noise_stride, image_stride)
  if (m->self_collision && m->h_i[17] > 0) JH_V5_LAUNCH_BATCH(true); else JH_V5_LAUNCH_BATCH(false);
#undef JH_V5_LAUNCH_BATCH
  return jh_launch_done(ovf, st);
}

bool JH_V5_NAME(jh_engine5_accepts)(const jh_model* m) { return model_is_leap(m) && (m->cylinders > 0) == (JH_V5_CYL != 0); }
```

### judo_amd/csrc/jh_internal.h

```cpp
#pragma once

#include <hip/hip_runtime.h>

#include <cstdarg>
#include <cstdint>
#include <cstdio>
#include <vector>

#include "judo_amd.h"
#include "judo_amd_xcheck.h"

#define JH_BLOB_MAGIC 0x314D484Au
#define JH_BLOB_VERSION 1u
#define JH_NSTATS 512

struct jh_blob_header {
  uint32_t magic, version, kind, nq, nv, nu, ns, ntaskparam, nfloat, nint;
  uint32_t reserved[6];
};

struct jh_model {
  int device, kind, nq, nv, nu, ns, ntaskparam;
  size_t nf, ni;
  float* d_f;
  int* d_i;
  int kernel_gen;
  int contact_capacity;
  int cylinders;
  int arm_pairs;
  int self_collision;
  int rollout_schedule;
  int plan_step_launches;
  mutable int one_launch_steps = 0;
  mutable int ovf_fallbacks = 0;
  int* d_stats;
  std::vector<float> h_f;
  std::vector<int> h_i;
};

void jh_set_error(const char* fmt, ...);

inline float* jh_launch_scratch(const jh_model* m, size_t bytes, hipStream_t st, bool overflow_rows = true) {
  hipMemPool_t pool = nullptr; void* p = nullptr;
  if (hipDeviceGetDefaultMemPool(&pool, m->device) == hipSuccess && pool && hipMallocFromPoolAsync(&p, bytes, pool, st) == hipSuccess) return (float*)p;
  (void)hipGetLastError();
  if (!overflow_rows) return nullptr;
  if (__atomic_fetch_add(&m->ovf_fallbacks, 1, __ATOMIC_RELAXED) == 0)
    fprintf(stderr, "judo_amd: no stream-ordered scratch for the contacts above the LDS pool (%zu bytes): this launch runs with the LDS capacity alone; see jh_model_stats out[6]\n", bytes);
  return nullptr;
}

#define JH_HIP(call)                                                                      \
  do {                                                                                    \
    hipError_t e__ = (call);                                                              \
    if (e__ != hipSuccess) {                                                              \
      jh_set_error("%s failed: %s (%s:%d)", #call, hipGetErrorString(e__), __FILE__, __LINE__); \
      return JH_ERR_HIP;                                                                  \
    }                                                                                     \
  } while (0)

inline int jh_launch_done(float* ovf, hipStream_t st) {
  const hipError_t e = hipGetLastError();
  const hipError_t f = ovf ? hipFreeAsync(ovf, st) : hipSuccess;
  if (e != hipSuccess) { jh_set_error("kernel launch failed: %s", hipGetErrorString(e)); return JH_ERR_HIP; }
  if (f != hipSuccess) { jh_set_error("hipFreeAsync failed: %s", hipGetErrorString(f)); return JH_ERR_HIP; }
  return JH_OK;
}

#define JH_REQUIRE(cond, ...)    \
  do {                           \
    if (!(cond)) {               \
      jh_set_error(__VA_ARGS__); \
      return JH_ERR_INVALID;     \
    }                            \
  } while (0)

enum {
  CP_DT = 0, CP_G, CP_MCART, CP_MPOLE, CP_L, CP_IPOLE, CP_DAMP_X, CP_DAMP_TH, CP_KP, CP_KV, CP_CTRL_LO, CP_CTRL_HI, CP_CTRL_LIMITED,
  CP_FRC_LO, CP_FRC_HI, CP_FRC_LIMITED, CP_X_LO, CP_X_HI, CP_X_LIMITED, CP_LIM_K, CP_LIM_B, CP_SOLIMP0, CP_SOLIMP1, CP_SOLIMP2,
  CP_SOLIMP3, CP_SOLIMP4, CP_INVW_X, CP_TIP, CP_NPARAM
};
enum {
  CY_DT = 0, CY_MP, CY_MC, CY_DAMP_P, CY_DAMP_C, CY_KP, CY_KV, CY_CTRL_LO, CY_CTRL_HI, CY_CTRL_LIMITED, CY_FRC_LO, CY_FRC_HI,
  CY_FRC_LIMITED, CY_RSUM, CY_CON_K, CY_CON_B, CY_SOLIMP0, CY_SOLIMP1, CY_SOLIMP2, CY_SOLIMP3, CY_SOLIMP4, CY_TRAN, CY_MU, CY_SITE_Z,
  CY_MARGIN, CY_NPARAM
};

int jh_simple_rollout_cost(const jh_model* m, const float* x0, const float* nominal, const float* noise, int ldn, const float* sigma,
                           const float* W, const float* lohi, const float* tp, int N, int n_offset, int H, int K, float* costs,
                           float* knots_out, float* trace, hipStream_t st);
int jh_latency_shift(int N, int rpw);
int jh_simple_max_knots(const jh_model* m, int H);
int jh_simple_one_launch_max_knots(const jh_model* m, int H);
int jh_engine_max_knots(const jh_model* m, int H);
int jh_simple_materialize(const jh_model* m, const float* x0, int x0_batched, const float* controls, int N, int H, float* states,
                          float* sensors, hipStream_t st);
int jh_simple_reward(const jh_model* m, const float* states, const float* controls, const float* tp, int N, int H, float* rewards, hipStream_t st);

int jh_engine_rollout_cost(const jh_model* m, const float* x0, const float* nominal, const float* noise, int ldn, const float* sigma,
                           const float* W, const float* lohi, const float* tp, int phase, int N, int n_offset, int H, int K, float* costs,
                           float* knots_out, hipStream_t st);
int jh_engine_materialize(const jh_model* m, const float* x0, int x0_batched, const float* controls, int N, int H, float* states,
                          float* sensors, hipStream_t st);
int jh_engine_reward(const jh_model* m, const float* states, const float* sensors, const float* controls, const float* tp, int phase, int N,
                     int H, float* rewards, hipStream_t st);

int jh_engine2_rollout_cost(const jh_model* m, const float* x0, const float* nominal, const float* noise, int ldn, const float* sigma,
                            const float* W, const float* lohi, const float* tp, int N, int n_offset, int H, int K, float* costs, float* knots_out,
                            hipStream_t st);
int jh_engine2_materialize(const jh_model* m, const float* x0, int x0_batched, const float* controls, int N, int H, float* states, float* sensors,
                           hipStream_t st);

int jh_engine5_rollout_cost(const jh_model* m, const float* x0, const float* nominal, const float* noise, int ldn, const float* sigma, const float* W,
                            const float* lohi, const float* tp, int N, int n_offset, int H, int K, float* costs, float* knots_out, float* trace, hipStream_t st);
int jh_engine5_materialize(const jh_model* m, const float* x0, int x0_batched, const float* controls, int N, int H, float* states, float* sensors,
                           hipStream_t st);
int jh_engine5_rollout_cost_cap64(const jh_model* m, const float* x0, const float* nominal, const float* noise, int ldn, const float* sigma, const float* W,
                                  const float* lohi, const float* tp, int N, int n_offset, int H, int K, float* costs, float* knots_out, float* trace, hipStream_t st);
int jh_engine5_materialize_cap64(const jh_model* m, const float* x0, int x0_batched, const float* controls, int N, int H, float* states, float* sensors,
                                 hipStream_t st);
int jh_engine5_rollout_cost_cyl(const jh_model* m, const float* x0, const float* nominal, const float* noise, int ldn, const float* sigma, const float* W,
                                const float* lohi, const float* tp, int N, int n_offset, int H, int K, float* costs, float* knots_out, float* trace, hipStream_t st);
int jh_engine5_materialize_cyl(const jh_model* m, const float* x0, int x0_batched, const float* controls, int N, int H, float* states, float* sensors,
                               hipStream_t st);

int jh_engine5_rollout_cost_batch(const jh_model* m, const float* images, long long image_stride, int B, const float* x0, const float* nominal, const float* sigma, const float* lohi, const float* tp, long long blk_stride,
                                  const float* noise, int ldn, long long noise_stride, const float* W, int N, int H, int K, float* costs, float* trace, hipStream_t st);
int jh_engine5_rollout_cost_batch_cap64(const jh_model* m, const float* images, long long image_stride, int B, const float* x0, const float* nominal, const float* sigma, const float* lohi, const float* tp, long long blk_stride,
                                        const float* noise, int ldn, long long noise_stride, const float* W, int N, int H, int K, float* costs, float* trace, hipStream_t st);
int jh_engine5_rollout_cost_batch_cyl(const jh_model* m, const float* images, long long image_stride, int B, const float* x0, const float* nominal, const float* sigma, const float* lohi, const float* tp, long long blk_stride,
                                      const float* noise, int ldn, long long noise_stride, const float* W, int N, int H, int K, float* costs, float* trace, hipStream_t st);

bool jh_engine5_accepts(const jh_model* m);
bool jh_engine5_accepts_cap64(const jh_model* m);
bool jh_engine5_accepts_cyl(const jh_model* m);

bool jh_model_is_fr3(const jh_model* m);
int jh_engine3_rollout_cost(const jh_model* m, const float* x0, const float* nominal, const float* noise, int ldn, const float* sigma, const float* W,
                            const float* lohi, const float* tp, int phase, int N, int n_offset, int H, int K, float* costs, float* knots_out, hipStream_t st);
int jh_engine3_materialize(const jh_model* m, const float* x0, int x0_batched, const float* controls, int N, int H, float* states, float* sensors,
                           hipStream_t st);

int jh_engine6_rollout_cost(const jh_model* m, const float* x0, const float* nominal, const float* noise, int ldn, const float* sigma, const float* W,
                            const float* lohi, const float* tp, int phase, int N, int n_offset, int H, int K, float* costs, float* knots_out, float* trace, hipStream_t st);
int jh_engine6_materialize(const jh_model* m, const float* x0, int x0_batched, const float* controls, int N, int H, float* states, float* sensors,
                           hipStream_t st);
bool jh_model_is_fr3_self(const jh_model* m);
int jh_engine6_rollout_cost_self(const jh_model* m, const float* x0, const float* nominal, const float* noise, int ldn, const float* sigma, const float* W,
                                 const float* lohi, const float* tp, int phase, int N, int n_offset, int H, int K, float* costs, float* knots_out, float* trace, hipStream_t st);
int jh_engine6_materialize_self(const jh_model* m, const float* x0, int x0_batched, const float* controls, int N, int H, float* states, float* sensors,
                                hipStream_t st);

__device__ __forceinline__ float jh_impedance(float s0, float s1, float s2, float s3, float s4, float dist) {
  if (s0 == s1 || s2 <= 1e-15f) return 0.5f * (s0 + s1);
  float x = fabsf(dist / s2);
  if (x >= 1.f) return s1;
  if (x <= 0.f) return s0;
  float y;
  if (s4 == 1.f) y = x;
  else if (x <= s3) y = __powf(x, s4) / __powf(s3, s4 - 1.f);
  else y = 1.f - __powf(1.f - x, s4) / __powf(1.f - s3, s4 - 1.f);
  return s0 + y * (s1 - s0);
}

__device__ __forceinline__ float jh_clampf(float v, float lo, float hi) { return fminf(hi, fmaxf(lo, v)); }

struct jh_policy;
int jh_policy_step_strided(const jh_policy* p, const float* states, int ld, int nq, int base_qpos, int base_qvel, int leg_qpos, int leg_qvel, const float* command, int ldc,
                           float* policy_out, float* control, float* scratch, int N, hipStream_t st);
```

### judo_amd/device.py

```python

from __future__ import annotations

import ctypes as C
import os

import numpy as np
import torch

from judo_amd import _lib
from judo_amd.models import layout, load_description, pack_model


def require_gpu() -> torch.device:
    if not torch.cuda.is_available():
        raise RuntimeError("judo_amd needs an MI355X (HIP device): torch.cuda.is_available() is False and there is no CPU fallback")
    return torch.device("cuda", torch.cuda.current_device())


_raw_stream = getattr(torch._C, "_cuda_getCurrentRawStream", None)


def current_stream_ptr() -> int:
    if _raw_stream is not None:
        return int(_raw_stream(torch.cuda.current_device()))
# ... 79 lines not shown

    def set_contact_capacity(self, contacts: int) -> None:
        _lib.check(_lib.lib().jh_model_set_contact_capacity(self.handle, int(contacts)), "jh_model_set_contact_capacity")
        self._max_knots_cache.clear()
        self.contact_capacity = int(contacts)

    def set_self_collision(self, on: bool) -> None:
        _lib.check(_lib.lib().jh_model_set_self_collision(self.handle, int(bool(on))), "jh_model_set_self_collision")
        self._self_collision_requested = bool(on)
        self.self_collision = bool(on) and self.kernel_generation == 3 and self.desc.get("family", self.task) == "leap_cube"

    def trace_layout(self) -> tuple[int, int, bool]:
        out = (C.c_int * 3)()
        _lib.check(_lib.lib().jh_model_trace_layout(self.handle, out), "jh_model_trace_layout")
        return int(out[0]), int(out[1]), bool(out[2])

    def limits(self) -> tuple[int, int, int, int]:
        out = (C.c_int * 4)()
        _lib.check(_lib.lib().jh_model_limits(self.handle, out), "jh_model_limits")
        return tuple(int(v) for v in out)

    @property
    def max_fused_knots(self) -> int:
        out = (C.c_int * 4)()
        _lib.check(_lib.lib().jh_model_limits(self.handle, out), "jh_model_limits")
        return int(out[0])

    def max_fused_knots_at(self, H: int) -> int:
        H = int(H)
        k = self._max_knots_cache.get(H)
        if k is None:
            k = int(_lib.lib().jh_model_max_fused_knots(self.handle, H))
            if k < 0:
                _lib.check(k, "jh_model_max_fused_knots")
            self._max_knots_cache[H] = k
        return k

    def one_launch_max_knots_at(self, H: int) -> int:
        k = int(_lib.lib().jh_model_one_launch_max_knots(self.handle, int(H)))
        if k < 0:
            _lib.check(k, "jh_model_one_launch_max_knots")
        return k

    def set_plan_step_launches(self, launches: int) -> None:
        _lib.check(_lib.lib().jh_model_set_plan_step_launches(self.handle, int(launches)), "jh_model_set_plan_step_launches")

    def set_rollout_schedule(self, mode: int) -> None:
        _lib.check(_lib.lib().jh_model_set_rollout_schedule(self.handle, int(mode)), "jh_model_set_rollout_schedule")

    def stats(self, reset: bool = True) -> dict:
        out = (C.c_int * 8)()
        _lib.check(_lib.lib().jh_model_stats(self.handle, out, int(reset)), "jh_model_stats")
        u = [v & 0xFFFFFFFF for v in out]
        return {"contact_overflow": u[0], "newton_cap_hits": u[1], "newton_iters": u[2], "steps": u[3], "wave_newton_iters": u[4], "wave_steps": u[5], "overflow_pool_fallbacks": u[6], "one_launch_plan_steps": u[7]}

    def __del__(self) -> None:
        try:
            if getattr(self, "handle", None):
                _lib.lib().jh_model_destroy(self.handle)
                self.handle = None
        except Exception:
            pass


class GpuModelSet:

    def __init__(self, models) -> None:
        self.models = list(models)
        if not self.models:
            raise ValueError("a model set needs at least one model")
        handles = (C.c_void_p * len(self.models))(*[m.handle.value for m in self.models])
        handle = C.c_void_p()
        _lib.check(_lib.lib().jh_model_set_create(handles, len(self.models), C.byref(handle)), "jh_model_set_create")
        self.handle = handle

    def __len__(self) -> int:
        return len(self.models)

    def info(self) -> dict:
        out = (C.c_int * 4)()
        _lib.check(_lib.lib().jh_model_set_info(self.handle, out), "jh_model_set_info")
        return {"B": int(out[0]), "image_floats": int(out[1]), "stride_floats": int(out[2]), "distinct_from_first": int(out[3])}

    def update(self, b: int, model: GpuModel) -> None:
        _lib.check(_lib.lib().jh_model_set_update(self.handle, int(b), model.handle), "jh_model_set_update")
        self.models[int(b)] = model

    def close(self) -> None:
        if getattr(self, "handle", None):
            _lib.lib().jh_model_set_destroy(self.handle)
            self.handle = None

    def __del__(self) -> None:
        try:
            self.close()
        except Exception:
            pass
```

### judo_amd/engine_model.py

```python

from __future__ import annotations

import numpy as np

from judo_amd.models import (
    MINMU,
    MINVAL,
    TASK_KIND,
    _pack,
    clamp_solimp,
    inverse_weights,
    layout,
    quat_mul,
    quat_to_mat,
    solref_to_kb,
)

JFREE, JSLIDE, JHINGE = 0, 2, 3
GBOX, GSPHERE, GCAPSULE, GCYLINDER = 6, 2, 3, 5
GTYPE = {"box": GBOX, "sphere": GSPHERE, "capsule": GCAPSULE, "cylinder": GCYLINDER}
MAX_MOVING, MAX_DOF, MAX_BLOCKS, MAX_BLOCK_DOF, MAX_GEOM, MAX_SITE = 20, 24, 4, 9, 80, 8

BODY_I, GEOM_I, ACT_I, BLOCK_I = 6, 2, 2, 4
BODY_F, DOF_F, ACT_F, GEOM_F, SITE_F = 32, 20, 8, 20, 3
HEADER_I, HEADER_F = 24, 24
SOLVER_TOL, SOLVER_MAX_ITER, SOLVER_LS_TOL = 1e-5, 50, 1e-2
ABLATE = (0, 1)


def _static_world_pose(desc: dict, b: int) -> tuple[np.ndarray, np.ndarray]:
    chain = []
    while b > 0:
        chain.append(b)
        b = desc["bodies"][b]["parent"]
    pos, quat = np.zeros(3), np.array([1.0, 0, 0, 0])
    for bb in reversed(chain):
        body = desc["bodies"][bb]
        pos = pos + quat_to_mat(quat) @ np.array(body["pos"])
        quat = quat_mul(quat, body["quat"])
    return pos, quat / np.linalg.norm(quat)


def engine_structure(desc: dict) -> dict:
    lay = layout(desc)
    nb = len(desc["bodies"])
    joints_of = lay.body_joints
    is_static = [False] * nb
    is_static[0] = True
    for b in range(1, nb):
        is_static[b] = (len(joints_of[b]) == 0) and is_static[desc["bodies"][b]["parent"]]
    moving = [b for b in range(1, nb) if not is_static[b]]
    for b in moving:
        if len(joints_of[b]) != 1:
            raise NotImplementedError(f"body {desc['bodies'][b]['name']}: the engine needs exactly one joint per moving body")
    free = [b for b in moving if desc["joints"][joints_of[b][0]]["type"] == "free"]
    if len(free) != 1 or moving[0] != free[0]:
        raise NotImplementedError("the engine needs exactly one free body, listed before the articulated bodies")
    fb = desc["bodies"][free[0]]
    if desc["bodies"][fb["parent"]]["parent"] != -1 and fb["parent"] != 0:
        raise NotImplementedError("free body must hang off the world")
    if np.abs(fb["ipos"]).max() > 0 or abs(abs(fb["iquat"][0]) - 1) > 1e-12:
        raise NotImplementedError("free body: centre of mass must be the body origin and the inertia axis-aligned")
    midx = {b: i for i, b in enumerate(moving)}
    block_of, blocks = {}, []
    for b in moving[1:]:
        p = desc["bodies"][b]["parent"]
        if is_static[p]:
            block_of[b] = len(blocks)
            blocks.append([b])
        else:
            if p not in block_of:
                raise NotImplementedError("articulated body attached to the free body is not supported")
            block_of[b] = block_of[p]
            blocks[block_of[b]].append(b)
    for blk in blocks:
        if blk != list(range(blk[0], blk[0] + len(blk))):
            raise NotImplementedError("bodies of a block must be contiguous (depth-first MJCF order)")
    return dict(layout=lay, is_static=is_static, moving=moving, midx=midx, blocks=blocks, block_of=block_of, free=free[0])


def _mat_to_quat(R: np.ndarray) -> np.ndarray:
    t = np.trace(R)
    if t > 0:
        s = np.sqrt(t + 1.0) * 2
# ... 83 lines not shown
                raise NotImplementedError("framepos relative to a moving site")
            bp, bq = _static_world_pose(desc, site["body"])
            p_ref = bp + quat_to_mat(bq) @ np.array(site["pos"])
            R_ref = quat_to_mat(quat_mul(bq, site.get("quat", [1, 0, 0, 0])))
            found = True
        elif sn["type"] == "framequat":
            if sn.get("reftype") == "body":
                if not weld(sn["ref"]):
                    raise NotImplementedError("framequat relative to a moving body")
                q_ref = np.array(_static_world_pose(desc, sn["ref"])[1], dtype=np.float64)
            found = True
    return [*p_ref, *R_ref.reshape(-1), *q_ref] if found else None


def generic_pairs(desc: dict, fused: dict, st: dict, cube_only: bool | None = None) -> list[tuple[int, int]]:
    arm_pairs = bool(desc.get("self_collision", False))
    bodies = desc["bodies"]
    njnt = [0] * len(bodies)
    for j in desc["joints"]:
        njnt[j["body"]] += 1

    def weld(b):
        while b > 0 and njnt[b] == 0:
            b = bodies[b]["parent"]
        return b

    def weld_parent(b):
        w = weld(b)
        return weld(bodies[w]["parent"]) if w > 0 else 0

    excl = {tuple(sorted(e)) for e in desc["excludes"]}
    geoms = fused["geoms"]
    free_fused = st["free"]
    out, extra = [], []
    for a in range(len(geoms)):
        for b in range(a + 1, len(geoms)):
            ia, ib = a, b
            if geoms[a]["type"] == "capsule" and geoms[b]["type"] == "box":
                ia, ib = b, a
            ga, gb = geoms[ia], geoms[ib]
            ta, tb = ga["type"], gb["type"]
            round_ = ("sphere", "cylinder")
            if not ((ta == "box" and tb in ("box", "sphere", "capsule", "cylinder")) or (ta in round_ and tb == "box") or (ta in round_ and tb in round_ and cube_only is False)
                    or (arm_pairs and ta == tb == "capsule")):
                continue
            ba, bb = ga["orig_body"], gb["orig_body"]
            wa, wb = weld(ba), weld(bb)
            new = ta == "capsule" or (tb == "capsule" and not (wa == 0 or ga["body"] == free_fused))
            if new and not arm_pairs:
                continue
            if wa == wb or tuple(sorted((ba, bb))) in excl:
                continue
            if (weld_parent(ba) == wb and wb != 0) or (weld_parent(bb) == wa and wa != 0):
                continue
            leap = desc.get("family", desc["task"]) == "leap_cube"
            if (leap if cube_only is None else cube_only) and free_fused not in (ga["body"], gb["body"]):
                continue
            (extra if new else out).append((ia, ib))
    def rank(pr):
        ba, bb = geoms[pr[0]]["body"], geoms[pr[1]]["body"]
        if free_fused in (ba, bb):
            return 0
        return 1 if (st["is_static"][ba] or st["is_static"][bb]) else 2
    out.sort(key=rank)
    return out + extra


def kernel_stand_ins(desc: dict) -> dict:
    if not any(g["type"] == "cylinder" for g in desc["geoms"]) or desc.get("family", desc["task"]) != "leap_cube":
        return desc
    out = dict(desc)
    out["geoms"] = [dict(g, type="sphere", size=[g["size"][0]], substitute_for_cylinder=list(g["size"])) if g["type"] == "cylinder" else g for g in desc["geoms"]]
    return out


def bounding_box_half(g: dict) -> np.ndarray:
    if g["type"] == "sphere":
        return np.array([g["size"][0]] * 3)
    if g["type"] == "cylinder":
        return np.array([g["size"][0], g["size"][0], g["size"][1]])
    return np.array(g["size"][:3])


def pack_engine_model(desc: dict, fingertips: str | None = None) -> bytes:
    fingertips = desc.get("fingertips", "sphere") if fingertips is None else fingertips
    if fingertips not in ("sphere", "cylinder"):
        raise ValueError(f"fingertips must be 'sphere' or 'cylinder', got {fingertips!r}")
    keep_cyl = fingertips == "cylinder" and desc.get("family", desc["task"]) == "leap_cube"
    if not isinstance(desc.get("self_collision", False), bool):
        raise ValueError(f"self_collision must be a bool, got {desc['self_collision']!r}")
    if desc.get("self_collision", False) and desc.get("family", desc["task"]) != "fr3_pick":
        raise NotImplementedError("self_collision: only the fr3 kernel has a build selected by this entry (the leap kernel models the hand's own contacts by default)")
    if fingertips == "cylinder" and not keep_cyl:
        raise NotImplementedError("fingertips='cylinder': only the leap kernel has a cylinder build")
    for g in desc["geoms"]:
        if keep_cyl and g["type"] == "cylinder" and (len(g["size"]) != 2 or min(g["size"]) <= 0):
            raise NotImplementedError(f"geom {g.get('name')}: a cylinder's size is (radius, half length), both positive")
    kinds = ("box", "sphere", "cylinder") if keep_cyl else ("box", "sphere")
    if not keep_cyl:
        desc = kernel_stand_ins(desc)
    orig = desc
    ref_frames = sensor_reference_frames(orig)
    dofw_o, bodyw_o = inverse_weights(orig)
    desc = fuse_fixed_bodies(orig)
    st = engine_structure(desc)
    lay, moving, midx, blocks = st["layout"], st["moving"], st["midx"], st["blocks"]
    o = desc["option"]
    dofw = dofw_o
    bodyw_geom = lambda g: bodyw_o[g.get("orig_body", g["body"])][0]
    _, bodyw = inverse_weights(desc)
    NM, NBLK = len(moving), len(blocks)
    if NM > MAX_MOVING or lay.nv > MAX_DOF or NBLK > MAX_BLOCKS or max(len(b) for b in blocks) > MAX_BLOCK_DOF:
        raise NotImplementedError("model exceeds the engine's compile-time limits")

    cube_geoms = [g for g in desc["geoms"] if g["body"] == st["free"]]
    if len(cube_geoms) != 1 or cube_geoms[0]["type"] != "box" or np.abs(cube_geoms[0]["pos"]).max() > 0:
        raise NotImplementedError("free body must carry exactly one box geom centred on the body origin")
    cube = cube_geoms[0]
    others = [g for g in desc["geoms"] if g["body"] != st["free"] and g["type"] in kinds]
    others.sort(key=lambda g: (-1 if st["is_static"][g["body"]] else midx[g["body"]]))
    if len(others) > MAX_GEOM:
        raise NotImplementedError("too many collision geoms")

    I: list[int] = [0] * HEADER_I
    F: list[float] = [0.0] * HEADER_F
    integ = {"euler": 0, "implicitfast": 3}[o["integrator"]]
    cone = {"pyramidal": 0, "elliptic": 1}[o["cone"]]
    if integ != 3:
        raise NotImplementedError("engine kernels implement the implicitfast integrator (leap_cube / fr3_pick)")
    sites = desc["sites"]
    sens = desc["sensors"]
    I[0:12] = [NM, NBLK, lay.nv, lay.nq, lay.nu, len(others), len(sites), lay.ns, integ, cone, len(sens), 0]
    uniform = all(g["solref"] == cube["solref"] and g["solimp"] == cube["solimp"] for g in others)
    for g in others:
        if g["condim"] != 3 or g["margin"] != 0 or g["gap"] != 0:
            raise NotImplementedError("engine assumes condim 3 and zero margin/gap")
    cK, cB = solref_to_kb(cube["solref"], cube["solimp"], o["timestep"])
    F[0:3] = [o["timestep"], o["impratio"], SOLVER_TOL]
    F[3:6] = o["gravity"]
    F[6:8] = [cK, cB]
    F[8:13] = clamp_solimp(cube["solimp"])
    fbody = desc["bodies"][st["free"]]
    F[13:17] = [fbody["mass"], *fbody["inertia"]]
    F[17:20] = cube["size"]
    F[20] = float(np.linalg.norm(cube["size"]))
    F[21] = bodyw_geom(cube)
    F[22] = float(SOLVER_MAX_ITER)
    F[23] = float(SOLVER_LS_TOL)

    for i, b in enumerate(moving):
        body = desc["bodies"][b]
        j = lay.body_joints[b][0]
        jn = desc["joints"][j]
        jt = {"free": JFREE, "slide": JSLIDE, "hinge": JHINGE}[jn["type"]]
        p = body["parent"]
        if st["is_static"][p]:
            ppos, pquat = _static_world_pose(desc, p)
            lpos = ppos + quat_to_mat(pquat) @ np.array(body["pos"])
            lquat = quat_mul(pquat, body["quat"])
            par = -1
        else:
            lpos, lquat, par = np.array(body["pos"]), np.array(body["quat"]), midx[p]
        if jt != JFREE and np.abs(jn["pos"]).max() > 0:
            raise NotImplementedError("engine assumes joint anchors at the body origin")
        blk = st["block_of"].get(b, -1)
        I += [par, jt, lay.jnt_dofadr[j], lay.jnt_qposadr[j], blk, (b - blocks[blk][0]) if blk >= 0 else 0]
        lR = quat_to_mat(lquat / np.linalg.norm(lquat))
# ... 62 lines not shown
            I += [2, lay.jnt_qposadr[s["obj"]], s["adr"]]
        elif s["type"] == "framezaxis" and s.get("objtype") == "body":
            I += [3, midx[s["obj"]], s["adr"]]
        elif s["type"] == "framezaxis":
            I += [5, s["obj"], s["adr"]]
        else:
            I += [4, 0, s["adr"]]
    if NM - 1 == 16 and NBLK == 4 and uniform:
        lists: list[list[int]] = [[] for _ in range(16)]
        for gi, g in enumerate(others):
            b = g["body"]
            if not st["is_static"][b]:
                lists[midx[b] - 1].append(gi)
        for gi, g in enumerate(others):
            if st["is_static"][g["body"]]:
                min(lists, key=len).append(gi)
        lgm = max(len(x) for x in lists)
        I[11], I[12] = len(I), lgm
        for x in lists:
            I += x + [-1] * (lgm - len(x))
        oidx = {id(g): i for i, g in enumerate(others)}
        og = [g for g in desc["geoms"] if g["type"] in kinds]
        hh = [(a, b) for a, b in generic_pairs(orig, dict(desc, geoms=og), st, cube_only=False) if st["free"] not in (og[a]["body"], og[b]["body"])]
        link_code = lambda g: midx[g["body"]]
        partners: dict[int, set] = {}
        for a, b in hh:
            for x, y in ((og[a], og[b]), (og[b], og[a])):
                if st["is_static"][x["body"]] and not st["is_static"][y["body"]]:
                    partners.setdefault(x["body"], set()).add(link_code(y))
        sgroups: list[frozenset] = []
        for g in others:
            if st["is_static"][g["body"]]:
                key = frozenset(partners.get(g["body"], ()))
                if key not in sgroups:
                    sgroups.append(key)
        if len(sgroups) > 4:
            raise NotImplementedError("more than four groups of static collision geometry")
        SCODES = [0, 17, 18, 19]
        NBC = 20
        code = lambda g: SCODES[sgroups.index(frozenset(partners.get(g["body"], ())))] if st["is_static"][g["body"]] else link_code(g)
        is_static_code = lambda c: c == 0 or c > 16
        groups: dict[tuple[int, int], list[tuple[int, int]]] = {}
        for a, b in hh:
            ga, gb = og[a], og[b]
            if is_static_code(code(gb)) or (not is_static_code(code(ga)) and code(ga) > code(gb)):
                ga, gb = gb, ga
            if is_static_code(code(gb)):
                continue
            groups.setdefault((code(ga), code(gb)), []).append((oidx[id(ga)], oidx[id(gb)]))
        rng = {}
        for c in range(NBC):
            idxs = [i for i, g in enumerate(others) if code(g) == c]
            assert not idxs or idxs == list(range(idxs[0], idxs[0] + len(idxs))), "geoms of a body must be contiguous"
            rng[c] = (idxs[0], len(idxs)) if idxs else (0, 0)
        for (ca, cb), lst in groups.items():
            assert len(lst) == rng[ca][1] * rng[cb][1] and rng[ca][1] + rng[cb][1] <= 16, (ca, cb, len(lst))
        I[15], I[17] = len(I), len(groups)
        for (ca, cb) in groups:
            I += [ca, cb]
        for c in range(NBC):
            I += list(rng[c])
        I[16] = len(F)
        for c in range(NBC):
            gs = [g for g in others if code(g) == c]
            if not gs:
                F += [0.0] * 8
                continue
            corners = []
            for g in gs:
                if is_static_code(c):
                    bpos, bquat = _static_world_pose(desc, g["body"])
                    gp, gR = bpos + quat_to_mat(bquat) @ np.array(g["pos"]), quat_to_mat(quat_mul(bquat, g["quat"]))
                else:
                    gp, gR = np.array(g["pos"]), quat_to_mat(g["quat"])
                hs = bounding_box_half(g)
                for sx in (-1, 1):
                    for sy in (-1, 1):
                        for sz in (-1, 1):
                            corners.append(gp + gR @ (hs * np.array([sx, sy, sz])))
            corners = np.array(corners)
            lo, hi = corners.min(0), corners.max(0)
            ctr, half = 0.5 * (lo + hi), 0.5 * (hi - lo)
            F += [*ctr, float(np.linalg.norm(half)), *half, 0.0]
    allg = [g for g in desc["geoms"] if g["type"] in kinds + ("capsule",)]
    gidx = {id(g): i for i, g in enumerate(allg)}
    pairs_all = generic_pairs(orig, dict(desc, geoms=allg), st)
    frames = []
    for sx in sites:
        if st["is_static"][sx["body"]]:
            bp, bq = _static_world_pose(desc, sx["body"])
            frames.append(dict(body=-1, pos=list(bp + quat_to_mat(bq) @ np.array(sx["pos"])), quat=list(quat_mul(bq, sx.get("quat", [1, 0, 0, 0])))))
        else:
            frames.append(dict(body=midx[sx["body"]], pos=sx["pos"], quat=sx.get("quat", [1, 0, 0, 0])))
    dists = [sx for sx in sens if sx["type"] == "distance"]
    eqs = desc["equalities"]
    I[13], I[14] = len(I), len(F)
    I[20], I[21] = ABLATE
    I += [len(allg), len(pairs_all), len(eqs), len(frames), len(dists), len(sens), 0, 0]
    for g in allg:
        b = g["body"]
        if st["is_static"][b]:
            bpos, bquat = _static_world_pose(desc, b)
            pos = bpos + quat_to_mat(bquat) @ np.array(g["pos"])
            R = quat_to_mat(quat_mul(bquat, g["quat"]))
            mb = -1
        else:
            pos, R, mb = np.array(g["pos"]), quat_to_mat(g["quat"]), midx[b]
        size = (list(g["size"]) + [0, 0, 0])[:3]
        rb = size[0] if g["type"] == "sphere" else (size[0] + size[1] if g["type"] == "capsule" else float(np.linalg.norm(size)))
        I += [mb, GTYPE[g["type"]]]
        F += [*size, *pos, *R.reshape(-1), rb, max(MINMU, g["friction"][0]), bodyw_geom(g), 0, 0]
    for g in allg:
        F += [*g["solref"], *clamp_solimp(g["solimp"]), 0.0]
    for a, b in pairs_all:
        I += [a, b]
    for e in eqs:
        j1, j2 = e["joint1"], e["joint2"]
        d1, d2 = lay.jnt_dofadr[j1], lay.jnt_dofadr[j2]
        if any(abs(x) > 0 for x in e["polycoef"][2:]):
            raise NotImplementedError("joint equality: only linear coupling")
        eK, eB = solref_to_kb(e["solref"], e["solimp"], o["timestep"])
        blk1 = st["block_of"][desc["joints"][j1]["body"]]
        if blk1 != st["block_of"][desc["joints"][j2]["body"]]:
            raise NotImplementedError("joint equality across blocks")
        d0 = lay.jnt_dofadr[lay.body_joints[blocks[blk1][0]][0]]
        I += [d1, d2, blk1, d1 - d0, d2 - d0]
        F += [e["polycoef"][0], e["polycoef"][1], eK, eB, *clamp_solimp(e["solimp"]), dofw[d1] + dofw[d2], 0, 0]
    for fr in frames:
        I += [fr["body"]]
        F += [*fr["pos"], *quat_to_mat(fr["quat"]).reshape(-1)]
    glists: list[int] = []
    for sx in dists:
        la = [gidx[id(g)] for g in allg if g["orig_body"] == sx["body1"] and g["type"] == "box"]
        lb = [gidx[id(g)] for g in allg if g["orig_body"] == sx["body2"] and g["type"] == "box"]
        I += [len(glists), len(la), len(glists) + len(la), len(lb)]
        glists += la + lb
        F += [sx["cutoff"]]
    idist = 0
    for sx in sens:
        if sx["type"] == "framepos" and sx.get("reftype") is not None and sx["objtype"] == "body":
            I += [6, midx[sx["obj"]], 0, sx["adr"]]
        elif sx["type"] == "framequat":
            I += [7, midx[sx["obj"]], 0, sx["adr"]]
        elif sx["type"] == "framepos" and sx.get("objtype") == "site":
            I += [0, sx["obj"], 0, sx["adr"]]
        elif sx["type"] == "framepos":
            I += [1, midx[sx["obj"]], 0, sx["adr"]]
        elif sx["type"] == "jointpos":
            I += [2, lay.jnt_qposadr[sx["obj"]], 0, sx["adr"]]
        elif sx["type"] == "framezaxis" and sx.get("objtype") == "site":
            I += [5, sx["obj"], 0, sx["adr"]]
        elif sx["type"] == "framezaxis":
            I += [3, midx[sx["obj"]], 0, sx["adr"]]
        else:
            I += [4, idist, 0, sx["adr"]]
            idist += 1
    I += glists
    if ref_frames is not None:
        I[18] = len(F)
        F += ref_frames
    ntp = 9 if desc.get("family", desc["task"]) == "leap_cube" else 22
    return _pack(TASK_KIND[desc.get("family", desc["task"])], lay, ntp, F, I)


def geom_order(desc: dict) -> list[str]:
    st = engine_structure(desc)
    others = [g for g in desc["geoms"] if g["body"] != st["free"] and g["type"] in ("box", "sphere")]
    others.sort(key=lambda g: (-1 if st["is_static"][g["body"]] else st["midx"][g["body"]]))
    return [g["name"] for g in others]
```

### judo_amd/models.py

```python

from __future__ import annotations

import copy
import json
import os
import struct
from dataclasses import dataclass

import numpy as np

MODEL_DIR = os.path.join(os.path.dirname(os.path.abspath(__file__)), "models")
TASK_KIND = {"cartpole": 0, "cylinder_push": 1, "leap_cube": 2, "fr3_pick": 3}
BLOB_MAGIC = 0x314D484A
MINVAL = 1e-15
MINMU = 1e-5


def load_description(task: str) -> dict:
    if task in DERIVED_DESCRIPTIONS:
        return DERIVED_DESCRIPTIONS[task]()
    path = os.path.join(MODEL_DIR, task + ".json")
    if not os.path.exists(path):
        raise ValueError(f"unknown task {task!r}: no model description at {path}")
    with open(path) as f:
# ... 229 lines not shown
        Jr = Sb[:, :3].T
        Jp = np.cross(Sb[:, :3], aux["coms"][b]).T + Sb[:, 3:].T
        Mi = Minv[np.ix_(dofs, dofs)]
        bodyw[b] = (np.trace(Jp @ Mi @ Jp.T) / 3, np.trace(Jr @ Mi @ Jr.T) / 3)
    return dofw, bodyw


def solref_to_kb(solref, solimp, timestep: float) -> tuple[float, float]:
    dmax = min(0.9999, max(0.0001, solimp[1]))
    if solref[0] > 0:
        tc = max(solref[0], 2 * timestep)
        return 1 / max(MINVAL, dmax * dmax * tc * tc * solref[1] * solref[1]), 2 / max(MINVAL, dmax * tc)
    return -solref[0] / max(MINVAL, dmax * dmax), -solref[1] / max(MINVAL, dmax)


def clamp_solimp(solimp) -> list[float]:
    return [min(0.9999, max(0.0001, solimp[0])), min(0.9999, max(0.0001, solimp[1])), max(0.0, solimp[2]),
            min(0.9999, max(0.0001, solimp[3])), max(1.0, solimp[4])]


def actuator_ctrlrange(desc: dict) -> np.ndarray:
    out = np.zeros((len(desc["actuators"]), 2))
    for i, a in enumerate(desc["actuators"]):
        out[i] = a["ctrlrange"] if a["ctrlrange"] is not None else (-np.inf, np.inf)
    return out


def _pack(kind: int, lay: Layout, ntaskparam: int, floats, ints) -> bytes:
    f = np.asarray(floats, dtype=np.float32)
    i = np.asarray(ints, dtype=np.int32)
    head = struct.pack("<16I", BLOB_MAGIC, 1, kind, lay.nq, lay.nv, lay.nu, lay.ns, ntaskparam, f.size, i.size, 0, 0, 0, 0, 0, 0)
    return head + f.tobytes() + i.tobytes()


def _pack_cartpole(desc: dict) -> bytes:
    lay = layout(desc)
    o = desc["option"]
    cart, pole = desc["bodies"][1], desc["bodies"][2]
    jx, jth = desc["joints"]
    act = desc["actuators"][0]
    dofw, _ = inverse_weights(desc)
    K, B = solref_to_kb(jx["solreflimit"], jx["solimplimit"], o["timestep"])
    site_tip = next(s for s in desc["sites"] if s["name"] == "trace_pole")
    P = [
        o["timestep"], -o["gravity"][2], cart["mass"], pole["mass"], pole["ipos"][2], pole["inertia"][0], jx["damping"], jth["damping"],
        act["kp"], act["kv"], *(act["ctrlrange"] or (0, 0)), float(act["ctrlrange"] is not None),
        *(act["forcerange"] or (0, 0)), float(act["forcerange"] is not None),
        *(jx["range"] or (0, 0)), float(jx["range"] is not None), K, B, *clamp_solimp(jx["solimplimit"]), dofw[0], site_tip["pos"][2],
    ]
    return _pack(TASK_KIND["cartpole"], lay, 6, P, [])


def _pack_cylinder(desc: dict) -> bytes:
    lay = layout(desc)
    o = desc["option"]
    pusher, cart = desc["bodies"][2], desc["bodies"][3]
    jp, jc = desc["joints"][0], desc["joints"][2]
    act = desc["actuators"][0]
    gp = next(g for g in desc["geoms"] if g["name"] == "pusher")
    gc = next(g for g in desc["geoms"] if g["name"] == "cart")
    _, bodyw = inverse_weights(desc)
    solref = [0.5 * (a + b) for a, b in zip(gp["solref"], gc["solref"])]
    solimp = [0.5 * (a + b) for a, b in zip(gp["solimp"], gc["solimp"])]
    K, B = solref_to_kb(solref, solimp, o["timestep"])
    mu = max(MINMU, max(gp["friction"][0], gc["friction"][0]))
    margin = max(gp["margin"], gc["margin"]) - max(gp["gap"], gc["gap"])
    site = next(s for s in desc["sites"] if s["name"] == "pusher_site")
    P = [
        o["timestep"], pusher["mass"], cart["mass"], jp["damping"], jc["damping"], act["kp"], act["kv"],
        *(act["ctrlrange"] or (0, 0)), float(act["ctrlrange"] is not None), *(act["forcerange"] or (0, 0)), float(act["forcerange"] is not None),
        gp["size"][0] + gc["size"][0], K, B, *clamp_solimp(solimp), bodyw[2][0] + bodyw[3][0], mu, site["pos"][2], margin,
    ]
    return _pack(TASK_KIND["cylinder_push"], lay, 6, P, [])


def pack_model(desc: dict) -> bytes:
    task = desc.get("family", desc["task"])
    if task == "cartpole":
        return _pack_cartpole(desc)
    if task == "cylinder_push":
        return _pack_cylinder(desc)
    from judo_amd.engine_model import pack_engine_model

    return pack_engine_model(desc)


def _scale_named(items: list[dict], factors: dict | None, what: str, apply) -> None:
    if not factors:
        return
    names = {it["name"] for it in items}
    for name, factor in factors.items():
        if name is not None and name not in names:
            raise ValueError(f"scaled_description: no {what} named {name!r} (known: {sorted(names)})")
        for it in items:
            if name is None or it["name"] == name:
                apply(it, float(factor))


def scaled_description(desc: dict, *, body_mass: dict | None = None, geom_friction: dict | None = None, actuator_kp: dict | None = None) -> dict:
    out = copy.deepcopy(desc)

    def mass(b: dict, f: float) -> None:
        b["mass"] = b["mass"] * f
        b["inertia"] = [v * f for v in b["inertia"]]

    def friction(g: dict, f: float) -> None:
        g["friction"] = [g["friction"][0] * f] + list(g["friction"][1:])

    def kp(a: dict, f: float) -> None:
        a["kp"] = a["kp"] * f

    _scale_named(out["bodies"], body_mass, "body", mass)
    _scale_named(out["geoms"], geom_friction, "geom", friction)
    _scale_named(out["actuators"], actuator_kp, "actuator", kp)
    return out


def image_sections(blob: bytes) -> tuple[bytes, bytes, bytes]:
    blob = bytes(blob)
    if len(blob) < 64:
        raise ValueError(f"image_sections: {len(blob)} bytes are no model image (the header alone has 64)")
    head = struct.unpack("<16I", blob[:64])
    if head[0] != BLOB_MAGIC:
        raise ValueError(f"image_sections: bad magic {head[0]:08x}")
    nf, ni = head[8], head[9]
    if len(blob) != 64 + 4 * (nf + ni):
        raise ValueError(f"image_sections: {len(blob)} bytes, the header announces {64 + 4 * (nf + ni)}")
    return blob[:64], blob[64 : 64 + 4 * nf], blob[64 + 4 * nf :]
```

Measured before the change: 1.248 million.

## Add precomputed joint-space pair tables to skip hand self-collision pair checks

Precomputes, at model pack time, per body-pair grids over one or two hinge joint angles that mark cells where the pair provably cannot collide, and stores them in the int section. The leap cube engine kernels receive the int section and can drop a body pair's narrow-phase work when the current joint angles fall in a safe cell. Model sets share the tables only when all members keep identical kinematics, otherwise they fall back to a table-free int copy. This adds host-side packing cost, validation and a per-pair lookup in the kernel, and it relies on the conservative margin being correct.

```diff
diff --git a/include/judo_amd.h b/include/judo_amd.h
--- a/include/judo_amd.h
+++ b/include/judo_amd.h
@@ -107,6 +107,9 @@
 int jh_model_set_update(jh_model_set* set, int b, const jh_model* model);
 int jh_model_set_info(const jh_model_set* set, int* out );
 void jh_model_set_destroy(jh_model_set* set);
+
+int jh_model_set_pair_tables(const jh_model_set* set);
+int jh_pair_tables_shared(const void* blob0, size_t nbytes0, const void* blob, size_t nbytes);
 int jh_plan_step_batch_models(const jh_model_set* set, void* blk_dev, const void* blk_host, size_t blk_bytes, size_t blk_stride_bytes, int o_nominal, int o_sigma, int o_tp, int o_lohi,
                               const float* noise, int ldn, size_t noise_stride_floats, const float* W, int N, int H, int K, float* costs, float* trace, int mode, float lambda, int k,
                               int tie_high, int E, int row_floats, int colmajor, float* scratch, float* out, size_t out_stride_floats, void* out_host_mark, void* const* timing,
diff --git a/judo_amd/_lib.py b/judo_amd/_lib.py
--- a/judo_amd/_lib.py
+++ b/judo_amd/_lib.py
@@ -74,6 +74,8 @@
     "jh_model_set_update": (C.c_int, [C.c_void_p, C.c_int, C.c_void_p]),
     "jh_model_set_info": (C.c_int, [C.c_void_p, C.POINTER(C.c_int)]),
     "jh_model_set_destroy": (None, [C.c_void_p]),
+    "jh_model_set_pair_tables": (C.c_int, [C.c_void_p]),
+    "jh_pair_tables_shared": (C.c_int, [C.c_void_p, C.c_size_t, C.c_void_p, C.c_size_t]),
     "jh_plan_step_batch_models": (C.c_int, [C.c_void_p, C.c_void_p, C.c_void_p, C.c_size_t, C.c_size_t, C.c_int, C.c_int, C.c_int, C.c_int, f32p, C.c_int, C.c_size_t, f32p, C.c_int, C.c_int, C.c_int,
                                             f32p, f32p, C.c_int, C.c_float, C.c_int, C.c_int, C.c_int, C.c_int, C.c_int, f32p, f32p, C.c_size_t, C.c_void_p, C.c_void_p, C.c_void_p]),
     "jh_update_fused_batch": (C.c_int, [C.c_int, f32p, f32p, C.c_size_t, C.c_int, C.c_int, C.c_int, f32p, C.c_int, C.c_size_t, C.c_int, C.c_int, C.c_int, C.c_int, C.c_float, C.c_int, C.c_int, C.c_int,
diff --git a/judo_amd/csrc/jh_api.hip b/judo_amd/csrc/jh_api.hip
--- a/judo_amd/csrc/jh_api.hip
+++ b/judo_amd/csrc/jh_api.hip
@@ -57,6 +57,60 @@
     n++;
   }
   return n;
+}
+
+static int image_pair_tables(const jh_blob_header& h, const int* I) {
+  constexpr int HEADER = 24, PT_SLOT = JH_PT_SLOT, PT_MAX = JH_PT_MAX, PT_I = JH_PT_I, LANES = 16;
+  if (h.nint < (uint32_t)HEADER || I[PT_SLOT] == 0) return 0;
+  const long o = I[PT_SLOT], len = JH_PT_LEN, nbp = I[17];
+  if (o < HEADER || o + len > (long)h.nint) { jh_set_error("model_create: the pair tables at int %ld (%ld ints) lie outside the int section of %u", o, len, h.nint); return -1; }
+  const int n = I[o];
+  if (n < 0 || n > PT_MAX) { jh_set_error("model_create: %d pair tables, at most %d", n, PT_MAX); return -1; }
+  for (int t = 0; t < PT_MAX; t++) {
+    const int* T = I + o + 1 + t * PT_I;
+    if (t >= n) { for (int k = 0; k < PT_I; k++) if (T[k] != 0) { jh_set_error("model_create: pair table %d is beyond the count of %d and not zero", t, n); return -1; } continue; }
+    float f[4]; memcpy(f, T + 3, sizeof(f));
+    if (T[0] < 0 || T[0] >= nbp || (t > 0 && T[0] <= T[-PT_I])) { jh_set_error("model_create: pair table %d names body pair %d of %ld (ascending, each once)", t, T[0], nbp); return -1; }
+    if (T[1] < 0 || T[1] >= LANES || T[2] < 0 || T[2] >= LANES) { jh_set_error("model_create: pair table %d names joints (%d, %d) of %d", t, T[1], T[2], LANES); return -1; }
+    if (!std::isfinite(f[0]) || !std::isfinite(f[2]) || !std::isfinite(f[1]) || !std::isfinite(f[3]) || !(f[1] > 0.f) || !(f[3] >= 0.f)) {
+      jh_set_error("model_create: pair table %d: grid origins (%g, %g) and inverse cell widths (%g, %g) must be finite, the first width positive", t, f[0], f[2], f[1], f[3]);
+      return -1;
+    }
+  }
+  return (int)len;
+}
+
+static bool pair_tables_shared(const std::vector<float>& F0, const std::vector<int>& I0, const std::vector<float>& F, const std::vector<int>& I) {
+  constexpr int HEADER = 24, PT_SLOT = JH_PT_SLOT, BODY_F = 32, DOF_F = 20, ACT_F = 8, GEOM_F = 20, NBC = 20;
+  if (I0.size() <= (size_t)PT_SLOT || I.size() != I0.size() || F.size() != F0.size() || I[PT_SLOT] != I0[PT_SLOT]) return false;
+  const long o = I0[PT_SLOT], len = JH_PT_LEN;
+  if (o == 0) return true;
+  if (o < HEADER || o + len > (long)I0.size() || memcmp(&I[o], &I0[o], 4 * len) != 0) return false;
+  const long NM = I0[0], nv = I0[2], nu = I0[4], NG = I0[5], oBS = I0[16];
+  const long oDof = HEADER + NM * BODY_F, oGeom = oDof + nv * DOF_F + nu * ACT_F;
+  if (NM < 1 || nv < 6 || nu < 0 || NG < 0 || oGeom + NG * GEOM_F > (long)F0.size() || oBS < 0 || oBS + NBC * 8 > (long)F0.size()) return false;
+  auto same = [&](long at, long n) { return memcmp(&F[at], &F0[at], 4 * n) == 0; };
+  for (long b = 1; b < NM; b++) if (!same(HEADER + b * BODY_F, 12) || !same(HEADER + b * BODY_F + 28, 3)) return false;
+  for (long d = 6; d < nv; d++) if (!same(oDof + d * DOF_F + 6, 3)) return false;
+  for (long g = 0; g < NG; g++) if (!same(oGeom + g * GEOM_F, 16)) return false;
+  return same(oBS, NBC * 8);
+}
+
+static bool blob_sections(const void* blob, size_t nbytes, std::vector<float>& F, std::vector<int>& I) {
+  jh_blob_header h;
+  if (!blob || nbytes < sizeof(h)) return false;
+  memcpy(&h, blob, sizeof(h));
+  if (h.magic != JH_BLOB_MAGIC || nbytes != sizeof(h) + 4 * ((size_t)h.nfloat + h.nint)) return false;
+  const char* q = (const char*)blob + sizeof(h);
+  F.assign((const float*)q, (const float*)q + h.nfloat);
+  I.assign((const int*)(q + 4 * (size_t)h.nfloat), (const int*)(q + 4 * (size_t)h.nfloat) + h.nint);
+  return true;
+}
+
+extern "C" int jh_pair_tables_shared(const void* blob0, size_t nbytes0, const void* blob, size_t nbytes) {
+  std::vector<float> F0, F; std::vector<int> I0, I;
+  JH_REQUIRE(blob_sections(blob0, nbytes0, F0, I0) && blob_sections(blob, nbytes, F, I), "pair_tables_shared: not a model blob");
+  return pair_tables_shared(F0, I0, F, I) ? 1 : 0;
 }
 
 extern "C" int jh_model_create(const void* blob, size_t nbytes, int device, jh_model** out) {
@@ -78,6 +132,7 @@
     std::vector<int> I((const int*)(q + 4 * (size_t)h.nfloat), (const int*)(q + 4 * (size_t)h.nfloat) + h.nint);
     cylinders = image_cylinders(h, F.data(), I.data());
     if (cylinders < 0) return JH_ERR_BLOB;
+    if (h.kind == JH_TASK_LEAP_CUBE && image_pair_tables(h, I.data()) < 0) return JH_ERR_BLOB;
     if (cylinders > 0 && h.kind != JH_TASK_LEAP_CUBE) { jh_set_error("model_create: %d cylinder geoms, and only the leap kernel has a cylinder build", cylinders); return JH_ERR_BLOB; }
     if (h.kind == JH_TASK_FR3_PICK) {
       arm_pairs = image_arm_pairs(h, I.data());
@@ -429,7 +484,7 @@
                    tie_high, E, row_floats, colmajor, scratch, out, flag, nullptr, timing, stream);
 }
 
-static int plan_step_batch(const char* who, const jh_model* m, const float* images, long long image_stride, int B, void* blk_dev, const void* blk_host, size_t blk_bytes, size_t blk_stride_bytes,
+static int plan_step_batch(const char* who, const jh_model* m, const float* images, long long image_stride, const int* ints, int B, void* blk_dev, const void* blk_host, size_t blk_bytes, size_t blk_stride_bytes,
                            int o_nominal, int o_sigma, int o_tp, int o_lohi, const float* noise, int ldn, size_t noise_stride_floats, const float* W, int N, int H, int K, float* costs,
                            float* trace, int mode, float lambda, int k, int tie_high, int E, int row_floats, int colmajor, float* scratch, float* out, size_t out_stride_floats,
                            void* out_host_mark, void* const* timing, void* stream) {
@@ -476,9 +531,9 @@
   else {
     if (closed) rc = jh_simple_rollout_cost_batch(m, images, b, b + o_tp, W, H, K, a, s, st);
     else
-      rc = m->cylinders > 0           ? jh_engine5_rollout_cost_batch_cyl(m, images, image_stride, B, b, b + o_nominal, b + o_sigma, b + o_lohi, b + o_tp, s.blk, noise, ldn, s.noise, W, N, H, K, costs, trace, st)
-           : m->contact_capacity > 48 ? jh_engine5_rollout_cost_batch_cap64(m, images, image_stride, B, b, b + o_nominal, b + o_sigma, b + o_lohi, b + o_tp, s.blk, noise, ldn, s.noise, W, N, H, K, costs, trace, st)
-                                      : jh_engine5_rollout_cost_batch(m, images, image_stride, B, b, b + o_nominal, b + o_sigma, b + o_lohi, b + o_tp, s.blk, noise, ldn, s.noise, W, N, H, K, costs, trace, st);
+      rc = m->cylinders > 0           ? jh_engine5_rollout_cost_batch_cyl(m, images, image_stride, ints, B, b, b + o_nominal, b + o_sigma, b + o_lohi, b + o_tp, s.blk, noise, ldn, s.noise, W, N, H, K, costs, trace, st)
+           : m->contact_capacity > 48 ? jh_engine5_rollout_cost_batch_cap64(m, images, image_stride, ints, B, b, b + o_nominal, b + o_sigma, b + o_lohi, b + o_tp, s.blk, noise, ldn, s.noise, W, N, H, K, costs, trace, st)
+                                      : jh_engine5_rollout_cost_batch(m, images, image_stride, ints, B, b, b + o_nominal, b + o_sigma, b + o_lohi, b + o_tp, s.blk, noise, ldn, s.noise, W, N, H, K, costs, trace, st);
     if (rc == JH_OK && timing) JH_HIP(hipEventRecord((hipEvent_t)timing[1], st));
     if (rc == JH_OK) rc = jh_update_tail_batch_launch(a, s, st);
   }
@@ -493,7 +548,7 @@
                                   int tie_high, int E, int row_floats, int colmajor, float* scratch, float* out, size_t out_stride_floats, void* out_host_mark, void* const* timing,
                                   void* stream) {
   JH_REQUIRE(m != nullptr, "plan_step_batch: null pointer");
-  return plan_step_batch("plan_step_batch", m, m->d_f, 0, B, blk_dev, blk_host, blk_bytes, blk_stride_bytes, o_nominal, o_sigma, o_tp, o_lohi, noise, ldn, noise_stride_floats, W, N, H, K, costs, trace,
+  return plan_step_batch("plan_step_batch", m, m->d_f, 0, m->d_i, B, blk_dev, blk_host, blk_bytes, blk_stride_bytes, o_nominal, o_sigma, o_tp, o_lohi, noise, ldn, noise_stride_floats, W, N, H, K, costs, trace,
                          mode, lambda, k, tie_high, E, row_floats, colmajor, scratch, out, out_stride_floats, out_host_mark, timing, stream);
 }
 
@@ -503,7 +558,28 @@
   float* d_images;
   const jh_model* m0;
   std::vector<std::vector<float>> hf;
+  std::vector<std::vector<int>> hi;
+  int* d_i_plain;
+  bool tables;
 };
+
+static long int_sections_differ(const std::vector<int>& a, const std::vector<int>& b) {
+  constexpr long PT_SLOT = JH_PT_SLOT, PT_LEN = JH_PT_LEN;
+  if (a.size() != b.size()) return 0;
+  const long o = a.size() > (size_t)PT_SLOT && a[PT_SLOT] == b[PT_SLOT] && a[PT_SLOT] > 0 ? a[PT_SLOT] : -1;
+  for (long w = 0; w < (long)a.size(); w++) if (a[w] != b[w] && !(o >= 0 && w >= o && w < o + PT_LEN)) return w;
+  return -1;
+}
+
+static int model_set_tables(jh_model_set* s, bool member0_changed) {
+  s->tables = true;
+  for (int b = 1; b < s->B && s->tables; b++) s->tables = pair_tables_shared(s->hf[0], s->hi[0], s->hf[b], s->hi[b]);
+  if (!member0_changed) return JH_OK;
+  std::vector<int> plain = s->hi[0];
+  if (plain.size() > (size_t)JH_PT_SLOT) plain[JH_PT_SLOT] = 0;
+  if (!plain.empty()) JH_HIP(hipMemcpy(s->d_i_plain, plain.data(), 4 * plain.size(), hipMemcpyHostToDevice));
+  return JH_OK;
+}
 
 static int model_set_member(const char* who, const jh_model* m0, const jh_model* m, int b) {
   JH_REQUIRE(m != nullptr, "%s: member %d is a null pointer", who, b);
@@ -515,10 +591,8 @@
   JH_REQUIRE(m->field == m0->field, "%s: member %d differs from the set's member 0 in " #field " (" fmt " against " fmt ")", who, b, m->field, m0->field)
     JH_SET_SAME(device, "%d"); JH_SET_SAME(kind, "%d"); JH_SET_SAME(nq, "%d"); JH_SET_SAME(nv, "%d"); JH_SET_SAME(nu, "%d"); JH_SET_SAME(ns, "%d"); JH_SET_SAME(ntaskparam, "%d");
     JH_SET_SAME(nf, "%zu"); JH_SET_SAME(ni, "%zu");
-    if (m->h_i != m0->h_i) {
-      size_t w = 0;
-      while (w < m->h_i.size() && m->h_i[w] == m0->h_i[w]) w++;
-      jh_set_error("%s: member %d differs from the set's member 0 in the int section h_i (word %zu: %d against %d): topology, pair lists and lane lists are one for the launch", who, b, w, m->h_i[w], m0->h_i[w]);
+    if (const long w = int_sections_differ(m->h_i, m0->h_i); w >= 0) {
+      jh_set_error("%s: member %d differs from the set's member 0 in the int section h_i (word %ld: %d against %d): topology, pair lists and lane lists are one for the launch", who, b, w, m->h_i[w], m0->h_i[w]);
       return JH_ERR_INVALID;
     }
     JH_SET_SAME(kernel_gen, "%d"); JH_SET_SAME(contact_capacity, "%d"); JH_SET_SAME(cylinders, "%d"); JH_SET_SAME(self_collision, "%d"); JH_SET_SAME(rollout_schedule, "%d");
@@ -538,7 +612,7 @@
 
 static int model_set_upload(jh_model_set* s, int b, const jh_model* m) {
   if (s->nf) JH_HIP(hipMemcpy(s->d_images + (size_t)b * s->stride, m->d_f, 4 * s->nf, hipMemcpyDeviceToDevice));
-  s->hf[b] = m->h_f;
+  s->hf[b] = m->h_f; s->hi[b] = m->h_i;
   return JH_OK;
 }
 
@@ -550,14 +624,16 @@
   const jh_model* m0 = models[0];
   JH_HIP(hipSetDevice(m0->device));
   jh_model_set* s = new jh_model_set();
-  s->B = B; s->nf = m0->nf; s->stride = (m0->nf + 63) / 64 * 64; s->d_images = nullptr; s->m0 = m0; s->hf.resize(B);
+  s->B = B; s->nf = m0->nf; s->stride = (m0->nf + 63) / 64 * 64; s->d_images = nullptr; s->m0 = m0; s->hf.resize(B); s->hi.resize(B); s->d_i_plain = nullptr; s->tables = false;
   if (s->stride == 0) s->stride = 64;
   hipError_t e = hipMalloc(&s->d_images, 4 * s->stride * (size_t)B);
   if (e == hipSuccess) e = hipMemset(s->d_images, 0, 4 * s->stride * (size_t)B);
   int rc = JH_OK;
   if (e != hipSuccess) { jh_set_error("model_set_create: device allocation failed: %s", hipGetErrorString(e)); rc = JH_ERR_HIP; }
+  if (rc == JH_OK && hipMalloc(&s->d_i_plain, 4 * (m0->ni ? m0->ni : 1)) != hipSuccess) { jh_set_error("model_set_create: device allocation failed"); rc = JH_ERR_HIP; }
   for (int b = 0; b < B && rc == JH_OK; b++) rc = model_set_upload(s, b, models[b]);
-  if (rc != JH_OK) { if (s->d_images) (void)hipFree(s->d_images); delete s; return rc; }
+  if (rc == JH_OK) rc = model_set_tables(s, true);
+  if (rc != JH_OK) { if (s->d_images) (void)hipFree(s->d_images); if (s->d_i_plain) (void)hipFree(s->d_i_plain); delete s; return rc; }
   *out = s;
   return JH_OK;
 }
@@ -569,7 +645,7 @@
   JH_HIP(hipSetDevice(s->m0->device));
   if (int rc = model_set_upload(s, b, model)) return rc;
   if (b == 0) s->m0 = model;
-  return JH_OK;
+  return model_set_tables(s, b == 0);
 }
 
 extern "C" int jh_model_set_info(const jh_model_set* s, int* out) {
@@ -583,7 +659,13 @@
 extern "C" void jh_model_set_destroy(jh_model_set* s) {
   if (!s) return;
   if (s->d_images) (void)hipFree(s->d_images);
+  if (s->d_i_plain) (void)hipFree(s->d_i_plain);
   delete s;
+}
+
+extern "C" int jh_model_set_pair_tables(const jh_model_set* s) {
+  JH_REQUIRE(s != nullptr, "model_set_pair_tables: null pointer");
+  return s->tables && s->hi[0].size() > (size_t)JH_PT_SLOT && s->hi[0][JH_PT_SLOT] > 0 ? 1 : 0;
 }
 
 extern "C" int jh_plan_step_batch_models(const jh_model_set* set, void* blk_dev, const void* blk_host, size_t blk_bytes, size_t blk_stride_bytes, int o_nominal, int o_sigma, int o_tp, int o_lohi,
@@ -591,7 +673,7 @@
                                          int k, int tie_high, int E, int row_floats, int colmajor, float* scratch, float* out, size_t out_stride_floats, void* out_host_mark,
                                          void* const* timing, void* stream) {
   JH_REQUIRE(set != nullptr, "plan_step_batch_models: null pointer");
-  return plan_step_batch("plan_step_batch_models", set->m0, set->d_images, (long long)set->stride, set->B, blk_dev, blk_host, blk_bytes, blk_stride_bytes, o_nominal, o_sigma, o_tp, o_lohi, noise, ldn,
+  return plan_step_batch("plan_step_batch_models", set->m0, set->d_images, (long long)set->stride, set->tables ? set->m0->d_i : set->d_i_plain, set->B, blk_dev, blk_host, blk_bytes, blk_stride_bytes, o_nominal, o_sigma, o_tp, o_lohi, noise, ldn,
                          noise_stride_floats, W, N, H, K, costs, trace, mode, lambda, k, tie_high, E, row_floats, colmajor, scratch, out, out_stride_floats, out_host_mark, timing, stream);
 }
 
diff --git a/judo_amd/csrc/jh_engine_v5.hip b/judo_amd/csrc/jh_engine_v5.hip
--- a/judo_amd/csrc/jh_engine_v5.hip
+++ b/judo_amd/csrc/jh_engine_v5.hip
@@ -50,6 +50,7 @@
 constexpr int HITPAIR = 1 << 15;
 static_assert(MAXG <= 128, "hand geom pairs are packed into 14 bits");
 constexpr int MAXBP = 128;
+constexpr int PT_SLOT = JH_PT_SLOT, PT_MAX = JH_PT_MAX, PT_I = JH_PT_I;
 constexpr int MAXBPL = 96;
 constexpr int NDH = 22 * 23 / 2;
 constexpr int NV = 22, NQ = 23, NU = 16, NS = 31, NS_CALTECH = 23, NX = 45, NMB = 17;
@@ -441,7 +442,7 @@
 #ifdef JH_V5_COUNT
   int cnt_dense = 0, cnt_it = 0, cnt_l2 = 0, cnt_bp = 0, cnt_hh = 0, cnt_cls[4] = {0, 0, 0, 0};
   enum { CB_SPH = 34, CB_SPHMAX, CB_BOXMAX, CB_L1PAIRPASS, CB_L1LISTPASS, CB_TRIPS, CB_BPAIRS, CB_T, CB_COMBOPASS, CB_CUBEBOX, CB_CUBEBOXLANES, CB_MSPH, CB_MBOX, CB_MT, CB_NOSPH, CB_ONEA, CB_ONEB,
-         CB_OWNTRIPS, CB_SPHOVER, CB_FEWSPH };
+         CB_OWNTRIPS, CB_SPHOVER, CB_FEWSPH, CB_TSAFE, CB_TDROP };
 #define V5_CADD(k, v) do { if (stats) atomicAdd(stats + (k), (int)(v)); } while (0)
 #define V5_CMAX(k, v) do { if (stats) atomicMax(stats + (k), (int)(v)); } while (0)
 #endif
@@ -669,6 +670,26 @@
           if (lane == 0) { V5_CADD(CB_SPHMAX, nsm); V5_CADD(CB_L1PAIRPASS, npass); V5_CADD(CB_L1LISTPASS, (nsm + G - 1) / G); }
         }
 #endif
+        int pt_slot = PT_SLOT; asm volatile("" : "+s"(pt_slot));
+        const int oPT = gI[pt_slot];
+#pragma unroll 1
+        for (int t = 0; oPT > 0 && t < PT_MAX; t++) {
+          const int* T = gI + oPT + 1 + t * PT_I;
+          const int qi = __float_as_int(q), ja = T[1], jb = T[2];
+          const int a0 = __builtin_amdgcn_readlane(qi, ja), a1 = __builtin_amdgcn_readlane(qi, 16 + ja), a2 = __builtin_amdgcn_readlane(qi, 32 + ja), a3 = __builtin_amdgcn_readlane(qi, 48 + ja);
+          const int b0 = __builtin_amdgcn_readlane(qi, jb), b1 = __builtin_amdgcn_readlane(qi, 16 + jb), b2 = __builtin_amdgcn_readlane(qi, 32 + jb), b3 = __builtin_amdgcn_readlane(qi, 48 + jb);
+          const float qa = __int_as_float(r == 0 ? a0 : (r == 1 ? a1 : (r == 2 ? a2 : a3))), qb = __int_as_float(r == 0 ? b0 : (r == 1 ? b1 : (r == 2 ? b2 : b3)));
+          const float fa = (qa - __int_as_float(T[3])) * __int_as_float(T[4]), fb = (qb - __int_as_float(T[5])) * __int_as_float(T[6]);
+          const bool in = fa >= 0.f && fa < 8.f && fb >= 0.f && fb < 8.f;
+          const unsigned long long w = (unsigned long long)(unsigned)T[7] | (unsigned long long)(unsigned)T[8] << 32;
+          const bool safe = in && ((w >> (((int)fa + 8 * (int)fb) & 63)) & 1ull);
+          const unsigned drop = (safe && l == (T[0] & (G - 1))) ? 1u << (T[0] / G) : 0u;
+#ifdef JH_V5_COUNT
+          if (live && l == 0 && safe) V5_CADD(CB_TSAFE, 1);
+          if (live && (sph & drop) != 0) V5_CADD(CB_TDROP, 1);
+#endif
+          sph &= ~drop;
+        }
         unsigned char* const tail = reinterpret_cast<unsigned char*>(&S.pool[0][0]);
         static_assert(sizeof(((RS*)nullptr)->pool) >= MAXBP - MAXBPL, "the tail of the sphere survivors fits the contact pool's storage");
         int nsl = 0;
@@ -1615,7 +1636,7 @@
   return jh_launch_done(ovf, st);
 }
 
-int JH_V5_NAME(jh_engine5_rollout_cost_batch)(const jh_model* m, const float* images, long long image_stride, int B, const float* x0, const float* nominal, const float* sigma, const float* lohi, const float* tp, long long blk_stride,
+int JH_V5_NAME(jh_engine5_rollout_cost_batch)(const jh_model* m, const float* images, long long image_stride, const int* ints, int B, const float* x0, const float* nominal, const float* sigma, const float* lohi, const float* tp, long long blk_stride,
                                   const float* noise, int ldn, long long noise_stride, const float* W, int N, int H, int K, float* costs, float* trace, hipStream_t st) {
   if (!model_is_leap(m)) { jh_set_error("plan_step_batch: the cooperative engine kernel is instantiated for leap_cube only"); return JH_ERR_UNSUPPORTED; }
   if ((m->cylinders > 0) != (JH_V5_CYL != 0)) { jh_set_error("plan_step_batch: an image with cylinder geoms runs on the cylinder build of the leap kernel and no other image does (%d cylinders)", m->cylinders); return JH_ERR_UNSUPPORTED; }
@@ -1625,7 +1646,7 @@
   const size_t ovf_bytes = NOVF > 0 ? (size_t)B * N * NOVF * POOL_F * sizeof(float) : 0;
   float* ovf = ovf_bytes > 0 ? jh_launch_scratch(m, ovf_bytes, st) : nullptr;
 #define JH_V5_LAUNCH_BATCH(SELF_)                                                                                                                                                  \
-  hipLaunchKernelGGL((k_leap_v5<false, WAVES_PER_BLOCK, SELF_, false, true>), dim3(grid, B), dim3(WAVE * WAVES_PER_BLOCK), 0, st, images, m->d_i, x0, 0, nominal, noise, ldn, sigma, W, \
+  hipLaunchKernelGGL((k_leap_v5<false, WAVES_PER_BLOCK, SELF_, false, true>), dim3(grid, B), dim3(WAVE * WAVES_PER_BLOCK), 0, st, images, ints, x0, 0, nominal, noise, ldn, sigma, W, \
                      lohi, tp, N, 0, H, K, costs, (float*)nullptr, (const float*)nullptr, (float*)nullptr, (float*)nullptr, m->d_stats, dshift, trace, ovf, (unsigned*)nullptr, blk_stride, noise_stride, image_stride)
   if (m->self_collision && m->h_i[17] > 0) JH_V5_LAUNCH_BATCH(true); else JH_V5_LAUNCH_BATCH(false);
 #undef JH_V5_LAUNCH_BATCH
diff --git a/judo_amd/csrc/jh_internal.h b/judo_amd/csrc/jh_internal.h
--- a/judo_amd/csrc/jh_internal.h
+++ b/judo_amd/csrc/jh_internal.h
@@ -13,6 +13,7 @@
 #define JH_BLOB_MAGIC 0x314D484Au
 #define JH_BLOB_VERSION 1u
 #define JH_NSTATS 512
+constexpr int JH_PT_SLOT = 19, JH_PT_MAX = 4, JH_PT_I = 9, JH_PT_LEN = 1 + JH_PT_MAX * JH_PT_I;
 
 struct jh_blob_header {
   uint32_t magic, version, kind, nq, nv, nu, ns, ntaskparam, nfloat, nint;
@@ -124,11 +125,11 @@
 int jh_engine5_materialize_cyl(const jh_model* m, const float* x0, int x0_batched, const float* controls, int N, int H, float* states, float* sensors,
                                hipStream_t st);
 
-int jh_engine5_rollout_cost_batch(const jh_model* m, const float* images, long long image_stride, int B, const float* x0, const float* nominal, const float* sigma, const float* lohi, const float* tp, long long blk_stride,
+int jh_engine5_rollout_cost_batch(const jh_model* m, const float* images, long long image_stride, const int* ints, int B, const float* x0, const float* nominal, const float* sigma, const float* lohi, const float* tp, long long blk_stride,
                                   const float* noise, int ldn, long long noise_stride, const float* W, int N, int H, int K, float* costs, float* trace, hipStream_t st);
-int jh_engine5_rollout_cost_batch_cap64(const jh_model* m, const float* images, long long image_stride, int B, const float* x0, const float* nominal, const float* sigma, const float* lohi, const float* tp, long long blk_stride,
+int jh_engine5_rollout_cost_batch_cap64(const jh_model* m, const float* images, long long image_stride, const int* ints, int B, const float* x0, const float* nominal, const float* sigma, const float* lohi, const float* tp, long long blk_stride,
                                         const float* noise, int ldn, long long noise_stride, const float* W, int N, int H, int K, float* costs, float* trace, hipStream_t st);
-int jh_engine5_rollout_cost_batch_cyl(const jh_model* m, const float* images, long long image_stride, int B, const float* x0, const float* nominal, const float* sigma, const float* lohi, const float* tp, long long blk_stride,
+int jh_engine5_rollout_cost_batch_cyl(const jh_model* m, const float* images, long long image_stride, const int* ints, int B, const float* x0, const float* nominal, const float* sigma, const float* lohi, const float* tp, long long blk_stride,
                                       const float* noise, int ldn, long long noise_stride, const float* W, int N, int H, int K, float* costs, float* trace, hipStream_t st);
 
 bool jh_engine5_accepts(const jh_model* m);
diff --git a/judo_amd/device.py b/judo_amd/device.py
--- a/judo_amd/device.py
+++ b/judo_amd/device.py
@@ -185,6 +185,9 @@
         _lib.check(_lib.lib().jh_model_set_info(self.handle, out), "jh_model_set_info")
         return {"B": int(out[0]), "image_floats": int(out[1]), "stride_floats": int(out[2]), "distinct_from_first": int(out[3])}
 
+    def pair_tables(self) -> bool:
+        return bool(_lib.lib().jh_model_set_pair_tables(self.handle))
+
     def update(self, b: int, model: GpuModel) -> None:
         _lib.check(_lib.lib().jh_model_set_update(self.handle, int(b), model.handle), "jh_model_set_update")
         self.models[int(b)] = model
diff --git a/judo_amd/engine_model.py b/judo_amd/engine_model.py
--- a/judo_amd/engine_model.py
+++ b/judo_amd/engine_model.py
@@ -1,5 +1,7 @@
 
 from __future__ import annotations
+
+import collections
 
 import numpy as np
 
@@ -249,7 +251,196 @@
     return np.array(g["size"][:3])
 
 
-def pack_engine_model(desc: dict, fingertips: str | None = None) -> bytes:
+PT_SLOT, PT_MAX, PT_I, PT_CELLS = 19, 4, 9, 8
+PT_SUB = 16
+PT_MARGIN = 0.2
+PT_SLACK = 1e-5
+PT_SUB_COARSE = (2, 4, 8)
+PT_CACHE = 8
+_pt_cache: collections.OrderedDict[bytes, list] = collections.OrderedDict()
+
+
+def _rot_axis(al: np.ndarray, q: np.ndarray) -> np.ndarray:
+    sn, cs = np.sin(q), np.cos(q)
+    t, (x, y, z) = 1.0 - cs, al
+    return np.stack([t * x * x + cs, t * x * y - sn * z, t * x * z + sn * y, t * x * y + sn * z, t * y * y + cs, t * y * z - sn * x,
+                     t * x * z - sn * y, t * y * z + sn * x, t * z * z + cs], -1).reshape(-1, 3, 3)
+
+
+def _obb_faces(ca, Ra, ha, cb, Rb, hb, infl):
+    d = cb - ca
+    C = np.abs(np.einsum("nki,nkj->nij", Ra, Rb))
+    da, db = np.abs(np.einsum("nki,nk->ni", Ra, d)), np.abs(np.einsum("nki,nk->ni", Rb, d))
+    return (da <= ha + C @ hb + infl).all(-1) & (db <= hb + np.einsum("nki,k->ni", C, ha) + infl).all(-1)
+
+
+def hand_pair_tables(F: list, I: list) -> list[dict]:
+    Ff = np.asarray(F, np.float32).astype(np.float64)
+    NM, NBLK, nv, nu, NG = I[0], I[1], I[2], I[4], I[5]
+    oDofF = HEADER_F + NM * BODY_F
+    oGeomF = oDofF + nv * DOF_F + nu * ACT_F
+    oGeomI = HEADER_I + NM * BODY_I + NBLK * BLOCK_I + nu * ACT_I
+    oBP, oBS, nBP = I[15], I[16], I[17]
+    oBG, NBC = oBP + 2 * nBP, 20
+    bodies = Ff[HEADER_F: HEADER_F + NM * BODY_F].reshape(NM, BODY_F)[1:]
+    geoms = Ff[oGeomF: oGeomF + NG * GEOM_F].reshape(NG, GEOM_F)
+    key = b"".join(np.ascontiguousarray(x).tobytes() for x in (
+        np.asarray(I[HEADER_I: HEADER_I + NM * BODY_I] + I[oGeomI: oGeomI + NG * GEOM_I] + I[oBP: oBG + 2 * NBC] + [NM, NBLK, nv, nu, NG], np.int64),
+        bodies[:, 0:12], bodies[:, 28:31], Ff[oDofF + 6 * DOF_F: oDofF + nv * DOF_F].reshape(-1, DOF_F)[:, 6:9], geoms[:, 0:16], Ff[oBS: oBS + 8 * NBC]))
+    if key in _pt_cache:
+        _pt_cache.move_to_end(key)
+        return _pt_cache[key]
+    assert all(I[oGeomI + g * GEOM_I + 1] in (GBOX, GSPHERE, GCYLINDER) for g in range(NG)), "pair tables: a geom kind the broad phase's restatement does not know"
+    static = lambda c: c == 0 or c >= NM
+    par = lambda c: I[HEADER_I + c * BODY_I]
+
+    def chain(c):
+        out = []
+        while not static(c) and c > 0:
+            out.append(c)
+            c = par(c)
+        return out[::-1]
+
+    def body_volumes(c):
+        g0, n = I[oBG + 2 * c], I[oBG + 2 * c + 1]
+        G = Ff[oGeomF + g0 * GEOM_F: oGeomF + (g0 + n) * GEOM_F].reshape(n, GEOM_F)
+        ty = [I[oGeomI + (g0 + k) * GEOM_I + 1] for k in range(n)]
+        half = np.array([[g[0]] * 3 if t == GSPHERE else ([g[0], g[0], g[1]] if t == GCYLINDER else list(g[0:3])) for g, t in zip(G, ty)])
+        bb = Ff[oBS + 8 * c: oBS + 8 * c + 8]
+        return dict(pos=G[:, 3:6], R=G[:, 6:15].reshape(n, 3, 3), half=half, rb=G[:, 15], ctr=bb[0:3], rad=bb[3], bhalf=bb[4:7])
+
+    cand = []
+    for pi in range(nBP):
+        ca, cb = I[oBP + 2 * pi], I[oBP + 2 * pi + 1]
+        la, lb = chain(ca), chain(cb)
+        while la and lb and la[0] == lb[0]:
+            la, lb = la[1:], lb[1:]
+        links = la + lb
+        if not 1 <= len(links) <= 2 or any(I[HEADER_I + k * BODY_I + 1] != JHINGE or Ff[oDofF + (5 + k) * DOF_F + 6] == 0 for k in links):
+            continue
+        lo = [Ff[oDofF + (5 + k) * DOF_F + 7] - PT_MARGIN for k in links]
+        w = [(Ff[oDofF + (5 + k) * DOF_F + 8] + PT_MARGIN - l0) / PT_CELLS for k, l0 in zip(links, lo)]
+        two = len(links) == 2
+        ncell = PT_CELLS * (PT_CELLS if two else 1)
+        A, B = body_volumes(ca), body_volumes(cb)
+
+        def evaluate(cells, sub):
+            k1, k2 = np.meshgrid(np.arange(sub), np.arange(sub if two else 1), indexing="ij")
+            qs = {links[0]: (lo[0] + ((cells % PT_CELLS)[:, None] + (k1.ravel() + 0.5) / sub) * w[0]).ravel()}
+            if two:
+                qs[links[1]] = (lo[1] + ((cells // PT_CELLS)[:, None] + (k2.ravel() + 0.5) / sub) * w[1]).ravel()
+            cell = np.repeat(np.arange(len(cells)), k1.size)
+            N = cell.size
+
+            def side(ls):
+                R, P, anchors = np.broadcast_to(np.eye(3), (N, 3, 3)), np.zeros((N, 3)), []
+                for k in ls:
+                    bf = Ff[HEADER_F + k * BODY_F: HEADER_F + (k + 1) * BODY_F]
+                    P = P + R @ bf[0:3]
+                    anchors.append(P)
+                    R = R @ bf[3:12].reshape(3, 3) @ _rot_axis(bf[28:31], qs[k])
+                return R, P, anchors
+
+            (RA, pA, anA), (RB, pB, anB) = side(la), side(lb)
+            cAw, cBw = pA + RA @ A["ctr"], pB + RB @ B["ctr"]
+            gA, gB = pA[:, None] + np.einsum("nij,gj->ngi", RA, A["pos"]), pB[:, None] + np.einsum("nij,gj->ngi", RB, B["pos"])
+            L = []
+            for an in anA + anB:
+                r = max(np.linalg.norm(cAw - an, axis=-1).max() + A["rad"], np.linalg.norm(cBw - an, axis=-1).max() + B["rad"])
+                for g, V in ((gA, A), (gB, B)):
+                    r = max(r, (np.linalg.norm(g - an[:, None], axis=-1) + np.linalg.norm(V["half"], axis=-1)).max())
+                L.append(r)
+            sp = [x / sub for x in w]
+            D = sum(0.5 * s_ * r for s_, r in zip(sp, L)) / (1.0 - sum(sp))
+
+            def level1(idx, infl):
+                d = cAw[idx] - cBw[idx]
+                idx = idx[(d * d).sum(-1) <= (A["rad"] + B["rad"] + infl) ** 2]
+                return idx[_obb_faces(cAw[idx], RA[idx], A["bhalf"], cBw[idx], RB[idx], B["bhalf"], infl)]
+
+            def candidate(idx, infl):
+                s1, out = level1(idx, infl), np.zeros(N, bool)
+                if not s1.size:
+                    return out
+
+                def near(g, V, co, Ro, ho):
+                    e = np.maximum(np.abs(np.einsum("nki,ngk->ngi", Ro, g - co[:, None])) - ho, 0.0)
+                    return (e * e).sum(-1) <= (V["rb"] + infl) ** 2
+                nA, nB = near(gA[s1], A, cBw[s1], RB[s1], B["bhalf"]), near(gB[s1], B, cAw[s1], RA[s1], A["bhalf"])
+                for a in range(nA.shape[1]):
+                    for b in range(nB.shape[1]):
+                        i = s1[nA[:, a] & nB[:, b] & ~out[s1]]
+                        if not i.size:
+                            continue
+                        e = gA[i, a] - gB[i, b]
+                        i = i[(e * e).sum(-1) <= (A["rb"][a] + B["rb"][b] + infl) ** 2]
+                        if i.size:
+                            out[i] = _obb_faces(gA[i, a], RA[i] @ A["R"][a], A["half"][a], gB[i, b], RB[i] @ B["R"][b], B["half"][b], infl)
+                return out
+
+            everything = np.arange(N)
+            l1_plain = np.zeros(N, bool)
+            l1_plain[level1(everything, 0.0)] = True
+            unsafe = candidate(everything, D + PT_SLACK)
+            certain = candidate(np.flatnonzero(unsafe), 0.0)
+            n = len(cells)
+            return np.bincount(cell, weights=unsafe, minlength=n) > 0, np.bincount(cell, weights=certain, minlength=n) > 0, np.bincount(cell, weights=l1_plain, minlength=n) > 0, D
+
+        cells = np.arange(ncell)
+        unsafe, certain, useful, D = evaluate(cells, PT_SUB_COARSE[0])
+        if not useful.any():
+            continue
+        for sub in PT_SUB_COARSE[1:] + (PT_SUB,):
+            again = np.flatnonzero(unsafe & ~certain)
+            if again.size:
+                u2, c2, f2, D = evaluate(again, sub)
+                unsafe[again], certain[again], useful[again] = u2, c2, useful[again] | f2
+        safe = ~unsafe
+        word = sum(1 << int(c) for c in np.flatnonzero(safe))
+        cand.append(dict(pair=pi, j1=links[0] - 1, j2=links[-1] - 1, o1=float(lo[0]), inv1=float(1.0 / w[0]), o2=float(lo[1]) if two else 0.0,
+                         inv2=float(1.0 / w[1]) if two else 0.0, word=word, score=int((safe & useful).sum()), D=float(D)))
+    best = sorted((t for t in cand if t["score"] > 0), key=lambda t: (-t["score"], t["pair"]))[:PT_MAX]
+    out = sorted(best, key=lambda t: t["pair"])
+    _pt_cache[key] = out
+    while len(_pt_cache) > PT_CACHE:
+        _pt_cache.popitem(last=False)
+    return out
+
+
+def pair_table_section(tables: list[dict]) -> list[int]:
+    bits = lambda x: int(np.float32(x).view(np.int32))
+    s32 = lambda u: u - (1 << 32) if u >= 1 << 31 else u
+    out = [len(tables)]
+    for t in tables:
+        out += [t["pair"], t["j1"], t["j2"], bits(t["o1"]), bits(t["inv1"]), bits(t["o2"]), bits(t["inv2"]), s32(t["word"] & 0xFFFFFFFF), s32(t["word"] >> 32)]
+    return out + [0] * (PT_I * (PT_MAX - len(tables)))
+
+
+def read_pair_tables(blob: bytes) -> list[dict]:
+    nf = int(np.frombuffer(blob[:64], np.uint32)[8])
+    Iv = np.frombuffer(blob[64 + 4 * nf:], np.int32)
+    o = int(Iv[PT_SLOT]) if Iv.size > PT_SLOT else 0
+    out = []
+    for t in range(int(Iv[o]) if o > 0 else 0):
+        r = Iv[o + 1 + t * PT_I: o + 1 + (t + 1) * PT_I]
+        f = r[3:7].view(np.float32)
+        out.append(dict(pair=int(r[0]), j1=int(r[1]), j2=int(r[2]), o1=float(f[0]), inv1=float(f[1]), o2=float(f[2]), inv2=float(f[3]),
+                        word=(int(r[7]) & 0xFFFFFFFF) | (int(r[8]) & 0xFFFFFFFF) << 32))
+    return out
+
+
+def pair_table_safe(t: dict, qa, qb) -> np.ndarray:
+    f32 = np.float32
+    with np.errstate(invalid="ignore"):
+        fa = (np.asarray(qa, f32) - f32(t["o1"])) * f32(t["inv1"])
+        fb = (np.asarray(qb, f32) - f32(t["o2"])) * f32(t["inv2"])
+        inside = (fa >= 0) & (fa < PT_CELLS) & (fb >= 0) & (fb < PT_CELLS)
+    bit = np.where(inside, fa, 0).astype(np.int64) + PT_CELLS * np.where(inside, fb, 0).astype(np.int64)
+    word = np.array([(t["word"] >> k) & 1 for k in range(64)], bool)
+    return inside & word[bit]
+
+
+def pack_engine_model(desc: dict, fingertips: str | None = None, pair_tables: bool = True) -> bytes:
     fingertips = desc.get("fingertips", "sphere") if fingertips is None else fingertips
     if fingertips not in ("sphere", "cylinder"):
         raise ValueError(f"fingertips must be 'sphere' or 'cylinder', got {fingertips!r}")
@@ -478,6 +669,9 @@
             lo, hi = corners.min(0), corners.max(0)
             ctr, half = 0.5 * (lo + hi), 0.5 * (hi - lo)
             F += [*ctr, float(np.linalg.norm(half)), *half, 0.0]
+        hand_tables = hand_pair_tables(F, I) if pair_tables else []
+    else:
+        hand_tables = []
     allg = [g for g in desc["geoms"] if g["type"] in kinds + ("capsule",)]
     gidx = {id(g): i for i, g in enumerate(allg)}
     pairs_all = generic_pairs(orig, dict(desc, geoms=allg), st)
@@ -555,6 +749,9 @@
     if ref_frames is not None:
         I[18] = len(F)
         F += ref_frames
+    if hand_tables:
+        I[PT_SLOT] = len(I)
+        I += pair_table_section(hand_tables)
     ntp = 9 if desc.get("family", desc["task"]) == "leap_cube" else 22
     return _pack(TASK_KIND[desc.get("family", desc["task"])], lay, ntp, F, I)
 
diff --git a/judo_amd/models.py b/judo_amd/models.py
--- a/judo_amd/models.py
+++ b/judo_amd/models.py
@@ -335,7 +335,7 @@
         return _pack_cylinder(desc)
     from judo_amd.engine_model import pack_engine_model
 
-    return pack_engine_model(desc)
+    return pack_engine_model(desc, pair_tables=bool(desc.get("pair_tables", True)))
 
 
 def _scale_named(items: list[dict], factors: dict | None, what: str, apply) -> None:
```

New measurement: 1.291 million (median of 6 runs). +3.4%, better.
